# allentran/golds-rl-gym

Measured on AMD Instinct MI355X. Metric: env-steps/sec (whole node), 32k parallel Swarm-v0 envs, 20-step PAAC rollout, higher is better.
Workload: dtype f32; 1 GPU; Swarm-v0 84x84, 32768 envs per GPU, T=20 PAAC update, conv policy of train_paac_conv.py (BASELINE configs[2]); envs_per_gpu=32768, envs_total=32768, rollout_steps=20, policy=conv, train=True, swarm_math=exact, env_state_dtype=f64, streams=4, gradient_exchange=none

## Files before the change

### golds-rl-gym_amd/csrc/net_conv.hip

```cpp
#include <rccl/rccl.h>
#include <stdlib.h>
#include <string.h>

#include <chrono>
#include <cmath>
#include <string>
#include <vector>

#include "../../include/goldsrl_net.h"
#include "common.h"
#include "net_gemm.h"
#include "net_reduce.inc"
#include "rng.h"

namespace grl {

enum : uint32_t { RS_ACTION = 16 };

struct ConvOffsets {
    static constexpr long c1w = 0, c1b = c1w + 8 * 8 * 3 * 32, c2w = c1b + 32, c2b = c2w + 4 * 4 * 32 * 64, c3w = c2b + 64,
                          c3b = c3w + 3 * 3 * 64 * 64, d1w = c3b + 64, d1b = d1w + 3136 * 512, d2w = d1b + 512,
                          d2b = d2w + 512 * 256, p1w = d2b + 256, p1b = p1w + 256 * 512, heads = p1b + 512;
};
constexpr int GRL_MAX_ACTIONS = 4;
// ... 17 lines not shown
using GatherT2 = ConvGather<10, 10, 1, 1, -1, -1, 2, 2, 64, 9, 9, true>;

}

constexpr int GRL_MAX_LANES = 8;
constexpr int kLossScaleAt = 8, kLossBoundAt = 10;
constexpr int kRangeLatchAt = 12;
struct NetLane {
    float *grads;
    float *a1, *a2, *a3, *d1, *d2, *p1, *v1, *v2;
    float *ga1, *ga2, *ga3, *gd1, *gd2, *gp1, *gv1, *gv2;
    float *sraw, *z2sh, *dz2, *gt;
    float *a2sh, *d2s, *gsl, *dza, *dz3sh, *tmpw3;
    unsigned long long *m2s;
    float *dl2, *tt2, *tmpw2;
    int2 *t2desc;
    float *z3sh;
    float *a3sh, *d3, *ysh;
    unsigned long long *m3;
    float *gd1sh, *gsh3, *g3p, *dz3p;
    int *perm, *goffp, *blkcnt, *blkoff, *sbeg, *send, *sgrp, *binbase;
    unsigned short *pkey, *prank;
    unsigned *smask, *tmask, *zmask, *wmask;
    int *slot_of;
    int2 *rowdesc;
    unsigned char *skey;
    unsigned short *srank, *stap;
    int *sblkcnt, *sblkoff, *sbinbase, *sperm;
    unsigned *tamask, *tbmask, *tcmask, *tnmask;
    int *trowlist, *tblklist, *tc3list, *trows_n, *twgcnt, *twgoff;
    unsigned *tumask;
    unsigned *obsrec;
    unsigned *tneed2;
    float *tubias;
    float *tug, *tuspix;
    float *tslab, *tsums;
    unsigned *stmask, *szmask;
    int *sbase, *rowagent, *sblk;
    signed char *tilegroup, *org;
    signed char *ulist;
    float *slab;
    float *slab1h;
    float *slabb;
    float *slab1b;
    float *cfold;
    float *carow;
    int *cperm, *cblkcnt, *cblkoff, *cgoff, *cslot, *cinv;
    signed char *ctilegroup;
    double *slab64;
    float *ro_mu;
    float *ws_a3, *ws_d1, *ws_d2, *ws_p1, *ws_v1, *ws_v2, *ws_a3sh, *ws_d3;
    unsigned long long *ws_m3;
    unsigned long long *mb_d2, *mb_v1, *ws_mb;
    float *ws_sraw, *ws_a2sh, *ws_d2s;
    unsigned long long *ws_m2s;
    signed char *ws_ulist;
    void *ws_idx[24];
    bool train_ready;
};

struct grl_net : NetLane {
    grl_handle *h;
    grl_net_config cfg;
    std::string err;
    int chunk;
    float *params, *adam_m, *adam_v;
    float *paramsT;
    long adam_t;
    float *w3t, *w2t;
    float *w3f;
    float *wpvT;
    int shared_trunk;
    double sfrac;
    double pfrac[3];
    float *tbgimg, *tbgz, *tbgimg3, *tbgz3, *tybg;
    int *tbglist;
    int obs_index;
    int trunk_skip;
    int patch_skip;
    int gemm_f32, range_fallback_on, range_fallbacks, range_bits_last, update_skipped_last;
    int f32_by_fallback, f32_clean_passes, range_return_k, range_returns;
    float absmax_last;
    int loss_scale_on;
    int acc1;
    int expand3_gather;
    int expand2_gemm, ctiles;
    float *w2corr;
    grl::HeadOff ho;
    int npad, ptiles, pslices, pslice_rows, pwgrad_xcd, pdgrad_xcd, pwgrad_pair, pdgrad_pair, swgrad_pair, swgrad_chunks, slots_xcd;
    int tn_wgs, tn_wgs_dense;
    size_t slab_floats, slab_used, slabb_floats, slabb_used;
    std::vector<grl::RJob> rq;
    std::vector<int> rq_dst;
    float *stats;
    int T, B;
    uint8_t *ro_lb, *ro_ab, *ro_pos, *ro_done;
    float *ro_act, *ro_envact, *ro_val, *ro_rew, *ro_y, *ro_adv, *ro_boot, *ro_pmu, *ro_psg;
    float *mu, *sigma, *vs;
    uint8_t *tmp_lb, *tmp_ab, *tmp_pos;
    int tmp_envs;
    unsigned long act_counter;
    std::vector<void *> allocs;
    bool prof_on;
    std::vector<hipEvent_t> prof_ev;
    std::vector<unsigned char> prof_tag;
    std::vector<double> prof_launch_flops;
    int prof_tag_cur;
    size_t prof_used;
    double prof_flops;
    int last_n;
    void *comm;
    int comm_world, comm_rank;
    hipEvent_t ar_ev0, ar_ev1;
    int ar_pending;
    long ar_calls;
    long ht_rollouts, ht_updates;
    double ht_rollout_ms, ht_train_enq_ms, ht_train_wait_ms;
    double ht_train_t0;
    double ar_ms_total;
    float ar_ms_last;
    int keep_level;
    float *keep;
    size_t keep_slots;
    long param_version, keep_version;
    int keep_max_level;
    bool keep_free_capped;
    size_t keep_free_cap, keep_headroom, keep_free_seen;
    int resident_last;
    float last_inv_total;
    NetLane lanes[GRL_MAX_LANES];
    hipStream_t lane_stream[GRL_MAX_LANES];
    hipEvent_t ev_fork, ev_join[GRL_MAX_LANES];
    hipStream_t side_stream[GRL_MAX_LANES];
    hipEvent_t ev_side0[GRL_MAX_LANES], ev_side1[GRL_MAX_LANES], ev_side2[GRL_MAX_LANES];
    int idx_side, side_now, pitem_on_side;
    int nlanes, cur_lane, last_lane;
};

namespace grl {

static int nfail(grl_net *n, int code, const std::string &msg) {
    if (n) n->err = msg;
    return code;
}
#define NET_HIP(n, call)                                                                                   \
    do {                                                                                                   \
        hipError_t _e = (call);                                                                            \
        if (_e != hipSuccess) return nfail(n, GRL_E_HIP, std::string(#call) + ": " + hipGetErrorString(_e)); \
    } while (0)

template <typename T>
static int nalloc(grl_net *n, T **p, size_t count) {
    NET_HIP(n, hipMalloc((void **)p, count * sizeof(T)));
    n->allocs.push_back(*p);
    NET_HIP(n, hipMemsetAsync(*p, 0, count * sizeof(T), n->h->stream));
    NET_HIP(n, hipStreamSynchronize(n->h->stream));
    return GRL_OK;
}

static void use_lane(grl_net *net, int k) {
    if (k == net->cur_lane) return;
    net->lanes[net->cur_lane] = static_cast<NetLane &>(*net);
    static_cast<NetLane &>(*net) = net->lanes[k];
    net->h->stream = net->lane_stream[k];
    net->cur_lane = k;
}
static int lanes_active(const grl_net *net) { return net->prof_on ? 1 : net->nlanes; }
static int lanes_fork(grl_net *net) {
    if (lanes_active(net) < 2) return GRL_OK;
    use_lane(net, 0);
    NET_HIP(net, hipEventRecord(net->ev_fork, net->lane_stream[0]));
    for (int k = 1; k < net->nlanes; ++k) NET_HIP(net, hipStreamWaitEvent(net->lane_stream[k], net->ev_fork, 0));
    return GRL_OK;
}
static int lanes_join(grl_net *net) {
    use_lane(net, 0);
    if (lanes_active(net) < 2) return GRL_OK;
    for (int k = 1; k < net->nlanes; ++k) {
        NET_HIP(net, hipEventRecord(net->ev_join[k], net->lane_stream[k]));
        NET_HIP(net, hipStreamWaitEvent(net->lane_stream[0], net->ev_join[k], 0));
    }
    return GRL_OK;
}

static double slot_rows_for_flops(grl_net *net, int n) {
    if (!net->prof_on) return 9.0 * n;
    int live = 9 * n;
    if (hipStreamSynchronize(net->h->stream) == hipSuccess) (void)hipMemcpy(&live, net->sbase + n, sizeof(int), hipMemcpyDeviceToHost);
    return (double)live;
}

enum {
    PT_OTHER = 0, PT_DENSE_FWD, PT_DENSE_DGRAD, PT_DENSE_WGRAD, PT_PATCH_FWD, PT_PATCH_DGRAD, PT_PATCH_WGRAD, PT_ENV_FWD, PT_ENV_DGRAD,
    PT_ENV_WGRAD, PT_SLOT_FWD, PT_SLOT_DGRAD, PT_SLOT_WGRAD, PT_CLASS_CORR, PT_PER_AGENT, PT_COUNT
};

template <int BM, int BN, int WGM, int WGN, class AG, class Epi, int XCD = 1, bool FENCE = true, int NBUF = 1, bool ACC1 = false>
static void launch_rowk(grl_net *net, dim3 grid, hipStream_t st, AG ag, const float *Bt, int ldb, int N, Epi epi) {
    constexpr bool kAcc1 = ACC1 && ((WGM * WGN == 8 && BM == 128 && BN == 128) || (WGM * WGN == 4 && BM * BN <= 128 * 64));
    if (net->gemm_f32)
        hipLaunchKernelGGL((gemm_rowk<BM, BN, WGM, WGN, AG, Epi, XCD, FENCE, true, NBUF, false>), grid, dim3(64 * WGM * WGN), 0, st, ag, Bt, ldb, N, epi);
    else if (kAcc1 && net->acc1)
        hipLaunchKernelGGL((gemm_rowk<BM, BN, WGM, WGN, AG, Epi, XCD, FENCE, false, NBUF, kAcc1>), grid, dim3(64 * WGM * WGN), 0, st, ag, Bt, ldb, N, epi);
    else
        hipLaunchKernelGGL((gemm_rowk<BM, BN, WGM, WGN, AG, Epi, XCD, FENCE, false, NBUF, false>), grid, dim3(64 * WGM * WGN), 0, st, ag, Bt, ldb, N, epi);
}
template <int BM, int BN, int WGM, int WGN, class AG, int XCD = 1>
static void launch_tn(grl_net *net, dim3 grid, hipStream_t st, AG ag, const float *dY, int J, int mc, float *slab) {
    if (net->gemm_f32) hipLaunchKernelGGL((gemm_tn<BM, BN, WGM, WGN, AG, XCD, true>), grid, dim3(64 * WGM * WGN), 0, st, ag, dY, J, mc, slab);
    else hipLaunchKernelGGL((gemm_tn<BM, BN, WGM, WGN, AG, XCD, false>), grid, dim3(64 * WGM * WGN), 0, st, ag, dY, J, mc, slab);
}

__global__ void evict_kernel(float4 *__restrict__ buf, size_t n4) {
    const size_t stride = (size_t)gridDim.x * blockDim.x;
    for (size_t i = (size_t)blockIdx.x * blockDim.x + threadIdx.x; i < n4; i += stride) buf[i] = make_float4(0.f, 0.f, 0.f, 0.f);
}
static void maybe_evict(grl_net *n) {
    static const bool on = getenv("GRL_NET_EVICT") && atoi(getenv("GRL_NET_EVICT")) != 0;
    if (!on) return;
    static float4 *buf = nullptr;
    constexpr size_t bytes = (size_t)512 << 20;
    if (!buf && hipMalloc((void **)&buf, bytes) != hipSuccess) { buf = nullptr; return; }
    hipLaunchKernelGGL(evict_kernel, dim3(2048), dim3(256), 0, n->h->stream, buf, bytes / 16);
}

struct GemmTimer {
    grl_net *n;
    GemmTimer(grl_net *net, double flops) : n(net) {
        maybe_evict(n);
        if (n->prof_on && n->prof_used + 2 <= n->prof_ev.size()) {
            (void)hipEventRecord(n->prof_ev[n->prof_used], n->h->stream);
            n->prof_flops += flops;
            n->prof_tag[n->prof_used / 2] = (unsigned char)n->prof_tag_cur;
            n->prof_launch_flops[n->prof_used / 2] = flops;
        }
    }
    ~GemmTimer() {
        if (n->prof_on && n->prof_used + 2 <= n->prof_ev.size()) {
            (void)hipEventRecord(n->prof_ev[n->prof_used + 1], n->h->stream);
            n->prof_used += 2;
        }
    }
};

__global__ void transpose_kernel(const float *__restrict__ src, int K, int N, float *__restrict__ dst) {
    __shared__ float tile[32][33];
    int k0 = blockIdx.y * 32, n0 = blockIdx.x * 32;
    for (int r = threadIdx.y; r < 32; r += blockDim.y)
        if (k0 + r < K && n0 + (int)threadIdx.x < N) tile[r][threadIdx.x] = src[(long)(k0 + r) * N + n0 + threadIdx.x];
    __syncthreads();
    for (int r = threadIdx.y; r < 32; r += blockDim.y)
        if (n0 + r < N && k0 + (int)threadIdx.x < K) dst[(long)(n0 + r) * K + k0 + threadIdx.x] = tile[threadIdx.x][r];
}

__global__ void conv2_corr_weights_kernel(const float *__restrict__ w2, float *__restrict__ bt);
static int trunk_background(grl_net *net);
static void refresh_transposes(grl_net *net) {
    const struct { long off; int K, N; } L[] = {
        {ConvOffsets::c2w, 512, 64}, {ConvOffsets::c3w, 576, 64}, {ConvOffsets::d1w, 3136, 512}, {ConvOffsets::d2w, 512, 256},
        {ConvOffsets::p1w, 256, 512}, {net->ho.v1w, 256, 512}, {net->ho.v2w, 512, 256}};
    for (const auto &l : L) {
        float *dst = l.off == ConvOffsets::p1w ? net->wpvT : l.off == net->ho.v1w ? net->wpvT + (size_t)512 * 256 : net->paramsT + l.off;
        hipLaunchKernelGGL(transpose_kernel, dim3((l.N + 31) / 32, (l.K + 31) / 32), dim3(32, 8), 0, net->h->stream, net->params + l.off,
                           l.K, l.N, dst);
    }
    hipLaunchKernelGGL(conv2_corr_weights_kernel, dim3((4 * 576 * 128 + 255) / 256), dim3(256), 0, net->h->stream, net->params + ConvOffsets::c2w,
                       net->w2corr);
    for (int tap = 0; tap < 9; ++tap)
        hipLaunchKernelGGL(transpose_kernel, dim3(2, 2), dim3(32, 8), 0, net->h->stream, net->params + ConvOffsets::c3w + tap * 4096, 64, 64,
                           net->w3f + tap * 4096);
    (void)trunk_background(net);
}

__global__ __launch_bounds__(256) void conv1_sparse_kernel(const uint8_t *__restrict__ lbins, const uint8_t *__restrict__ abins,
                                                           const uint8_t *__restrict__ pos, const float *__restrict__ w1,
                                                           const float *__restrict__ b1, float *__restrict__ a1, int G,
                                                           float *__restrict__ sraw) {
    __shared__ unsigned int cnt[2][7056 / 4 + 4];
    __shared__ float S[400 * 32];
    const int env = blockIdx.x, tid = threadIdx.x;
    for (int i = tid; i < 2 * (7056 / 4 + 4); i += 256) (&cnt[0][0])[i] = 0;
    __syncthreads();
    if (tid < 80) {
        int bx = lbins[((size_t)env * 80 + tid) * 2], by = lbins[((size_t)env * 80 + tid) * 2 + 1];
        if (bx != 255) { int idx = bx * G + by; atomicAdd(&cnt[0][idx >> 2], 1u << (8 * (idx & 3))); }
    } else if (tid < 90) {
        int a = tid - 80;
        int bx = abins[((size_t)env * 10 + a) * 2], by = abins[((size_t)env * 10 + a) * 2 + 1];
        if (bx != 255) { int idx = bx * G + by; atomicAdd(&cnt[1][idx >> 2], 1u << (8 * (idx & 3))); }
    }
    __syncthreads();
// ... 550 lines not shown
}

extern "C" {

int grl_net_config_default(int32_t kind, grl_net_config *cfg) {
    if (!cfg || kind != GRL_NET_CONV_SINGLE_AGENT) return GRL_E_INVALID;
    memset(cfg, 0, sizeof(*cfg));
    cfg->struct_size = (int32_t)sizeof(grl_net_config);
    cfg->kind = kind;
    cfg->max_chunk_samples = 40960;
    cfg->scale = 1000.f;
    cfg->entropy_beta = 0.02f;
    cfg->clip_norm = 40.f;
    cfg->gamma = 0.99f;
    cfg->num_actions = 2;
    return GRL_OK;
}

static int range_flag_init(grl_net *n);

int grl_net_create(grl_handle *h, const grl_net_config *cfg, grl_net **out) {
    if (!h || !cfg || !out) return GRL_E_INVALID;
    *out = nullptr;
    if (cfg->struct_size != (int32_t)sizeof(grl_net_config)) return fail(h, GRL_E_INVALID, "grl_net_create: grl_net_config size mismatch");
    if (cfg->kind != GRL_NET_CONV_SINGLE_AGENT) return fail(h, GRL_E_INVALID, "grl_net_create: unknown kind");
    if (h->cfg.env_kind != GRL_ENV_SWARM || h->cfg.grid_size != 84)
        return fail(h, GRL_E_INVALID, "grl_net_create: the conv net needs a Swarm handle with grid_size 84 (84x84x3 input)");
    if (cfg->max_chunk_samples < 10 || cfg->max_chunk_samples % 10 || cfg->max_chunk_samples > 131072)
        return fail(h, GRL_E_INVALID, "grl_net_create: max_chunk_samples must be a multiple of 10 in 10..131072");
    if (cfg->num_actions < 1 || cfg->num_actions > GRL_MAX_ACTIONS)
        return fail(h, GRL_E_INVALID, "grl_net_create: num_actions must be in 1..4");
    bool free_capped = false;
    unsigned long long free_mb = 0;
    if (const char *e = getenv("GRL_NET_KEEP_FREE_MB")) {
        char *end = nullptr;
        free_mb = strtoull(e, &end, 10);
        if (*e < '0' || *e > '9' || *end != 0 || free_mb >= (1ull << 44))
            return fail(h, GRL_E_INVALID, "grl_net_create: GRL_NET_KEEP_FREE_MB must be a number of MB (decimal digits)");
        free_capped = true;
    }
    hipSetDevice(h->cfg.device_id);
    grl_net *n = new grl_net();
    n->h = h; n->cfg = *cfg; n->chunk = cfg->max_chunk_samples; n->adam_t = 0;
    n->ho = head_offsets(cfg->num_actions);
    n->T = 0; n->B = 0; n->tmp_envs = 0; n->act_counter = 0; n->prof_on = false; n->prof_used = 0; n->prof_flops = 0; n->last_n = 0; n->prof_tag_cur = 0;
    n->ro_lb = nullptr; n->slab_floats = 0; n->slab_used = 0; n->slabb_floats = 0; n->slabb_used = 0; n->w3t = n->w2t = nullptr;
    n->mu = n->sigma = n->vs = nullptr;
    n->keep_level = 0;
    n->ar_ev0 = n->ar_ev1 = nullptr; n->ar_pending = 0; n->ar_calls = 0; n->ht_rollouts = n->ht_updates = 0; n->ht_rollout_ms = n->ht_train_enq_ms = n->ht_train_wait_ms = 0.0; n->ht_train_t0 = 0.0; n->ar_ms_total = 0.0; n->ar_ms_last = 0.f;
    n->keep = nullptr; n->keep_slots = 0; n->param_version = 0; n->keep_version = -1;
    n->keep_max_level = 3; n->keep_free_capped = false; n->keep_free_cap = 0; n->keep_headroom = 0; n->keep_free_seen = 0;
    n->resident_last = 0;
    if (const char *e = getenv("GRL_NET_KEEP_LEVEL")) n->keep_max_level = atoi(e);
    n->keep_free_capped = free_capped; n->keep_free_cap = (size_t)free_mb << 20;
    n->shared_trunk = (cfg->reserved & GRL_NET_F_PER_AGENT_TRUNK) ? 0 : 1;
    n->cur_lane = 0; n->last_lane = 0;
    for (int k = 0; k < GRL_MAX_LANES; ++k) { n->lane_stream[k] = nullptr; n->ev_join[k] = nullptr; n->side_stream[k] = nullptr; n->ev_side0[k] = n->ev_side1[k] = n->ev_side2[k] = nullptr; }
    n->idx_side = 0; n->side_now = 0; n->pitem_on_side = 0;
    n->lane_stream[0] = h->stream; n->ev_fork = nullptr; n->nlanes = 1;
    const size_t c = n->chunk;
    n->ptiles = (int)((c + 255) / 256) + 9;
    n->ctiles = (int)((c + 255) / 256) + 4;
    {
        const char *lsk = getenv("GRL_NET_LOSS_SCALE");
        n->loss_scale_on = (lsk && strcmp(lsk, "off") == 0) ? 0 : 1;
        const char *gm = getenv("GRL_NET_GEMM"), *rf = getenv("GRL_NET_RANGE_FALLBACK");
        n->gemm_f32 = (gm && strcmp(gm, "f32") == 0) ? 1 : 0;
        n->range_fallback_on = (rf && strcmp(rf, "off") == 0) ? 0 : 1;
        n->range_fallbacks = 0; n->range_bits_last = 0; n->update_skipped_last = 0;
        n->f32_by_fallback = 0; n->f32_clean_passes = 0; n->range_returns = 0; n->absmax_last = 0.f;
        n->range_return_k = 4;
        if (const char *rr = getenv("GRL_NET_RANGE_RETURN")) n->range_return_k = strcmp(rr, "off") == 0 ? 0 : std::max(0, atoi(rr));
        const char *psk = getenv("GRL_PATCH_SKIP");
        n->patch_skip = (psk && strcmp(psk, "off") == 0) ? 0 : 1;
        const char *oix = getenv("GRL_OBS_INDEX");
        n->obs_index = (oix && strcmp(oix, "off") == 0) ? 0 : 1;
        const char *tsk = getenv("GRL_TRUNK_SKIP");
        n->trunk_skip = (tsk && strcmp(tsk, "off") == 0) ? 0 : 1;
        n->pfrac[0] = n->pfrac[1] = n->pfrac[2] = 1.0; n->sfrac = 1.0;
        const char *e2 = getenv("GRL_NET_EXPAND2");
        n->expand2_gemm = (e2 && strcmp(e2, "lds") == 0) ? 0 : 1;
        { const char *e3 = getenv("GRL_NET_EXPAND3"); n->expand3_gather = (e3 && strcmp(e3, "prod") == 0) ? 0 : 1;
          const char *a1 = getenv("GRL_NET_ACC1"); n->acc1 = (a1 && strcmp(a1, "off") == 0) ? 0 : 1; }
    }
    n->pslice_rows = PATCH_SLICE_ROWS; n->pwgrad_xcd = 1;
    if (const char *e = getenv("GRL_PATCH_SLICE")) { const int v = atoi(e); if (v == 256 || v == 512 || v == 1024 || v == 2048 || v == 4096 || v == 8192) n->pslice_rows = v; }
    if (const char *e = getenv("GRL_PATCH_WGRAD_XCD")) n->pwgrad_xcd = atoi(e);
    n->pwgrad_pair = 1;
    if (const char *e = getenv("GRL_PATCH_WGRAD_PAIR")) n->pwgrad_pair = strcmp(e, "off") != 0 && strcmp(e, "0") != 0;
    n->pdgrad_pair = 1;
    if (const char *e = getenv("GRL_PATCH_DGRAD_PAIR")) n->pdgrad_pair = strcmp(e, "off") != 0 && strcmp(e, "0") != 0;
    n->swgrad_pair = 1;
    if (const char *e = getenv("GRL_SLOT_WGRAD_PAIR")) n->swgrad_pair = strcmp(e, "off") != 0 && strcmp(e, "0") != 0;
    n->slots_xcd = 1;
    if (const char *e = getenv("GRL_SLOTS_XCD")) n->slots_xcd = strcmp(e, "off") != 0 && strcmp(e, "0") != 0;
    n->swgrad_chunks = 0;
    if (const char *e = getenv("GRL_SLOT_WGRAD_CHUNKS")) n->swgrad_chunks = std::max(0, atoi(e));
    n->pdgrad_xcd = 1;
    n->tn_wgs = 1024; n->tn_wgs_dense = 512;
    if (const char *e = getenv("GRL_TN_WGS")) { const int v = atoi(e); if (v >= 256 && v <= 4096) n->tn_wgs = v; }
    if (const char *e = getenv("GRL_TN_WGS_DENSE")) { const int v = atoi(e); if (v >= 128 && v <= 4096) n->tn_wgs_dense = v; }
    if (const char *e = getenv("GRL_PATCH_DGRAD_XCD")) n->pdgrad_xcd = atoi(e) != 0;
    n->pslices = (int)((c + n->pslice_rows - 1) / n->pslice_rows) + 9;
    n->npad = (int)((c + 255) / 256 * 256);
    int rc = GRL_OK;
    auto A = [&](float **p, size_t cnt) { if (rc == GRL_OK) rc = nalloc(n, p, cnt); };
    A(&n->params, n->ho.total); A(&n->paramsT, n->ho.total); A(&n->adam_m, n->ho.total); A(&n->adam_v, n->ho.total);
    A(&n->w3f, 576 * 64); A(&n->stats, 16); A(&n->wpvT, (size_t)1024 * 256); A(&n->w2corr, 4 * 576 * 128);
    A(&n->tbgimg, 12800); A(&n->tbgz, 128); A(&n->tbgimg3, 5184); A(&n->tbgz3, 128); A(&n->tybg, 49 * 512);
    if (rc == GRL_OK) rc = nalloc(n, &n->tbglist, 4);
    int nlanes = (cfg->reserved & GRL_NET_F_SINGLE_STREAM) ? 1 : 4;
    if (const char *env = getenv("GRL_NET_LANES")) { int v = atoi(env); if (v >= 1 && v <= GRL_MAX_LANES) nlanes = v; }
    for (int k = 0; k < nlanes && rc == GRL_OK; ++k) {
        static_cast<NetLane &>(*n) = NetLane{};
        rc = alloc_lane_forward(n);
        n->lanes[k] = static_cast<NetLane &>(*n);
    }
    static_cast<NetLane &>(*n) = n->lanes[0];
    if (rc == GRL_OK && nlanes > 1) {
        bool ok = hipEventCreateWithFlags(&n->ev_fork, hipEventDisableTiming) == hipSuccess;
        for (int k = 1; k < nlanes && ok; ++k)
            ok = hipStreamCreateWithFlags(&n->lane_stream[k], hipStreamNonBlocking) == hipSuccess &&
                 hipEventCreateWithFlags(&n->ev_join[k], hipEventDisableTiming) == hipSuccess;
        if (!ok) rc = nfail(n, GRL_E_HIP, "creating the lane streams/events failed");
    }
    if (rc == GRL_OK) n->nlanes = nlanes;
    {
        const char *e = getenv("GRL_NET_IDX_SIDE");
        const bool want = !(cfg->reserved & GRL_NET_F_SINGLE_STREAM) && !(e && (!strcmp(e, "off") || !strcmp(e, "0"))) && rc == GRL_OK;
        if (want && side_stream_pick(n) == GRL_OK && n->side_stream[0]) {
            const bool ok = hipEventCreateWithFlags(&n->ev_side0[0], hipEventDisableTiming) == hipSuccess &&
                            hipEventCreateWithFlags(&n->ev_side1[0], hipEventDisableTiming) == hipSuccess &&
                            hipEventCreateWithFlags(&n->ev_side2[0], hipEventDisableTiming) == hipSuccess;
            n->idx_side = ok ? 1 : 0;
        }
        (void)hipGetLastError();
    }
    if (rc == GRL_OK && hipFuncSetAttribute((const void *)expand_conv2_kernel, hipFuncAttributeMaxDynamicSharedMemorySize,
                                            (int)EXP2_LDS_BYTES) != hipSuccess)
        rc = nfail(n, GRL_E_HIP, "hipFuncSetAttribute(expand_conv2_kernel)");
    if (rc == GRL_OK) rc = ensure_tmp_obs(n, h->E);
    if (rc == GRL_OK) rc = range_flag_init(n);
    if (rc != GRL_OK) {
        fail(h, rc, "grl_net_create: " + n->err);
        grl_net_destroy(n);
        return rc;
    }
    hipStreamSynchronize(h->stream);
    *out = n;
    return GRL_OK;
}

int grl_net_destroy(grl_net *n) {
    if (!n) return GRL_OK;
    const bool alive = grl_handle_alive(n->h);
    grl_sync_for_destroy(n->h);
    if (n->comm) {
        ncclCommDestroy((ncclComm_t)n->comm);
        (void)hipGetLastError();
    }
    if (alive) use_lane(n, 0);
    for (int k = 1; k < GRL_MAX_LANES; ++k) {
        if (n->lane_stream[k]) { hipStreamSynchronize(n->lane_stream[k]); hipStreamDestroy(n->lane_stream[k]); }
        if (n->ev_join[k]) hipEventDestroy(n->ev_join[k]);
    }
    for (int k = 0; k < GRL_MAX_LANES; ++k) {
// ... 357 lines not shown
```

### golds-rl-gym_amd/csrc/net_gemm.h

```cpp
#pragma once
#include <hip/hip_runtime.h>
#include <stdint.h>

#include <type_traits>
#include <utility>

namespace grl {

template <class E, class = void>
struct epi_row_bits : std::false_type {};
template <class E>
struct epi_row_bits<E, std::void_t<decltype(E::kRowBits)>> : std::bool_constant<E::kRowBits> {};

template <class E, class = void>
struct epi_row_auxn : std::false_type {};
template <class E>
struct epi_row_auxn<E, std::void_t<decltype(E::kRowAuxN)>> : std::bool_constant<E::kRowAuxN> {};
template <class E, class = void>
struct epi_add_aux : std::false_type {};
template <class E>
struct epi_add_aux<E, std::void_t<decltype(E::kAddAux)>> : std::bool_constant<E::kAddAux> {};

typedef float f32x16 __attribute__((ext_vector_type(16)));
typedef float f32x4 __attribute__((ext_vector_type(4)));
// ... 839 lines not shown
        s += (row[0] + row[32]) + (row[64] + row[96]);
    }
    red[threadIdx.x] = s;
    __syncthreads();
    if (threadIdx.x < 32) {
        float t = 0.f;
#pragma unroll
        for (int j = 0; j < 8; ++j) t += red[j * 32 + threadIdx.x];
        partial[blockIdx.x * 32 + threadIdx.x] = t;
    }
}

constexpr float kLowScale = 2048.f;
__device__ __forceinline__ void split2(float x, float y, unsigned &h, unsigned &l) {
    const f32x2 xy = {x, y};
    const f16x2 hv = __builtin_convertvector(xy, f16x2);
    const f32x2 r = {(x - (float)hv[0]) * kLowScale, (y - (float)hv[1]) * kLowScale};
    const f16x2 lv = __builtin_convertvector(r, f16x2);
    h = __builtin_bit_cast(unsigned, hv);
    l = __builtin_bit_cast(unsigned, lv);
}
__device__ __forceinline__ void split4(float x0, float x1, float x2, float x3, uint2 &h, uint2 &l) {
    split2(x0, x1, h.x, l.x);
    split2(x2, x3, h.y, l.y);
}
__device__ __forceinline__ void mfma_x3(f32x4 &acc, f32x4 &acl, const f16x8 (&a)[2], const f16x8 (&b)[2]) {
    acl = __builtin_amdgcn_mfma_f32_16x16x32_f16(a[1], b[0], acl, 0, 0, 0);
    acl = __builtin_amdgcn_mfma_f32_16x16x32_f16(a[0], b[1], acl, 0, 0, 0);
    acc = __builtin_amdgcn_mfma_f32_16x16x32_f16(a[0], b[0], acc, 0, 0, 0);
}
constexpr int kLdh = 32;
__device__ int *g_gemm_range_flag;
__device__ unsigned *g_gemm_absmax;
constexpr float kF16Max = 65504.f;
constexpr int kW128M = 4, kW128N = 2, kW256M = 8, kW256N = 1;
__device__ __forceinline__ int swz(int row) { return (0x78 >> (((row >> 2) & 3) * 2)) & 3; }

__device__ __forceinline__ int f32_off(int row, int k) { return row * 32 + ((((k >> 2) ^ (row & 7)) << 2) | (k & 3)); }
template <int TM, int TN>
__device__ __forceinline__ void mfma_f32_step(const float *__restrict__ Af, const float *__restrict__ Bf, int arow, int brow, int kg,
                                              f32x4 (&acc)[TM][TN]) {
    float4 a0[TM], a1[TM], b0[TN], b1[TN];
#pragma unroll
    for (int a = 0; a < TM; ++a) {
        a0[a] = *reinterpret_cast<const float4 *>(Af + f32_off(arow + a * 16, 8 * kg));
        a1[a] = *reinterpret_cast<const float4 *>(Af + f32_off(arow + a * 16, 8 * kg + 4));
    }
#pragma unroll
    for (int b = 0; b < TN; ++b) {
        b0[b] = *reinterpret_cast<const float4 *>(Bf + f32_off(brow + b * 16, 8 * kg));
        b1[b] = *reinterpret_cast<const float4 *>(Bf + f32_off(brow + b * 16, 8 * kg + 4));
    }
#define GRL_F32_STEP(AV, BV)                                                                                          \
    _Pragma("unroll") for (int a = 0; a < TM; ++a)                                                                    \
        _Pragma("unroll") for (int b = 0; b < TN; ++b) acc[a][b] = __builtin_amdgcn_mfma_f32_16x16x4f32(AV, BV, acc[a][b], 0, 0, 0);
    GRL_F32_STEP(a0[a].x, b0[b].x) GRL_F32_STEP(a0[a].y, b0[b].y) GRL_F32_STEP(a0[a].z, b0[b].z) GRL_F32_STEP(a0[a].w, b0[b].w)
    GRL_F32_STEP(a1[a].x, b1[b].x) GRL_F32_STEP(a1[a].y, b1[b].y) GRL_F32_STEP(a1[a].z, b1[b].z) GRL_F32_STEP(a1[a].w, b1[b].w)
#undef GRL_F32_STEP
}

template <class T, class = void> struct ag_has_ctx : std::false_type {};
template <class T> struct ag_has_ctx<T, std::void_t<decltype(std::declval<const T &>().wg_ctx(0))>> : std::true_type {};
template <class AG> __device__ __forceinline__ auto ag_ctx(const AG &ag, int m0) {
    if constexpr (ag_has_ctx<AG>::value) return ag.wg_ctx(m0);
    else return m0;
}
template <class AG, class C> __device__ __forceinline__ bool ag_tile_ok(const AG &ag, const C &c, int m0, int k0) {
    if constexpr (ag_has_ctx<AG>::value) return ag.tile_ok_c(c, k0);
    else return ag.tile_ok(m0, k0);
}
template <class AG, class C> __device__ __forceinline__ int ag_bk(const AG &ag, const C &c, int m0, int k0) {
    if constexpr (ag_has_ctx<AG>::value) return ag.bk_c(c, k0);
    else return ag.bk(k0, m0);
}
template <class T, class = void> struct ag_has_n_ok : std::false_type {};
template <class T> struct ag_has_n_ok<T, std::void_t<decltype(std::declval<const T &>().n_ok(0, 0))>> : std::true_type {};
template <class T, class = void> struct ag_has_i_ok : std::false_type {};
template <class T> struct ag_has_i_ok<T, std::void_t<decltype(std::declval<const T &>().i_ok(0, 0))>> : std::true_type {};
template <class T, class = void> struct ag_pair_n : std::false_type {};
template <class T> struct ag_pair_n<T, std::void_t<decltype(T::kPairN)>> : std::bool_constant<T::kPairN> {};
template <class T, class = void> struct ag_pair_i : std::false_type {};
template <class T> struct ag_pair_i<T, std::void_t<decltype(T::kPairI)>> : std::bool_constant<T::kPairI> {};

template <int BM, int BN, int WGM, int WGN, class AG, class Epi, int XCD_ORDER = 1, bool FENCE = true, bool F32 = false, int NBUF = 1, bool ACC1 = false>
__global__ __launch_bounds__(64 * WGM * WGN, ACC1 ? (WGM * WGN == 8 ? 6 : 4) : WGM * WGN / 2) void gemm_rowk(AG ag, const float *__restrict__ Bt, int ldb, int N, Epi epi) {
    constexpr int BK = 32, LDH = kLdh, NT = 64 * WGM * WGN, RPP = NT / 8;
    constexpr int WM = BM / WGM, WN = BN / WGN, TM = WM / 16, TN = WN / 16;
    constexpr int NA = BM / RPP;
    constexpr int NB = BN / RPP;
    static_assert((WGM * WGN == 4 || WGM * WGN == 8) && TM >= 1 && TN >= 1 && NA >= 1 && BN % RPP == 0, "4 or 8 waves");
    static_assert(NBUF == 1 || NBUF == 2, "one or two LDS buffers");
    __shared__ __attribute__((aligned(16))) unsigned short As[NBUF][2][BM * LDH];
    static_assert(!(ACC1 && F32), "the fp32 form has one accumulator set anyway");
    __shared__ __attribute__((aligned(16))) unsigned short Bs[NBUF][ACC1 ? 3 : 2][BN * LDH];

    const int tid = threadIdx.x, lane = tid & 63, wave = tid >> 6;
    const int wm = wave / WGN, wn = wave - wm * WGN;
    int bx = blockIdx.x, by = blockIdx.y;
    if constexpr (XCD_ORDER == 2) {
        const int nt = (ag.live_rows() + BM - 1) / BM, tpx = (nt + 7) >> 3, w = blockIdx.y;
        if ((w >> 3) >= tpx) return;
        by = (w & 7) * tpx + (w >> 3);
        if (by >= nt) return;
    }
    if (XCD_ORDER == 1) {
        const int nx = gridDim.x, L = by * nx + bx, g = L / (8 * nx);
        if ((g + 1) * 8 <= (int)gridDim.y) {
            const int l = L - g * 8 * nx;
            by = g * 8 + (l & 7);
            bx = l >> 3;
        }
    }
    const int m0 = by * BM, n0 = bx * BN;
    if (!ag.tile_active(m0)) return;
    constexpr bool PAIRN = ag_pair_n<AG>::value;
    int2 pp = make_int2(0, 0);
    if constexpr (PAIRN) {
        static_assert(!PAIRN || (BM == 128 && BN == 128 && WGN == 2 && 64 * WGM * WGN == 512), "128 x 128 on eight waves: a wave column per pixel");
        pp = ag.npair(m0, bx);
        if (pp.x < 0) return;
    } else if constexpr (ag_has_n_ok<AG>::value) {
        if (!ag.n_ok(m0, n0)) return;
    }
    const int M = ag.rows, K = ag.K();
    const auto wctx = ag_ctx(ag, m0);
    const int trow = tid >> 3, tk4 = (tid & 7) * 4;
    const int wo = (((tk4 >> 3) ^ swz(trow)) << 3) + (tk4 & 4);

    long aoff[NA];
    int ayx[NA];
    bool arow_ok[NA];
#pragma unroll
    for (int i = 0; i < NA; ++i) {
        int r = m0 + trow + RPP * i;
        arow_ok[i] = r < M;
        int iy0, ix0;
        ag.row(arow_ok[i] ? r : 0, aoff[i], iy0, ix0);
        ayx[i] = (iy0 << 16) | (ix0 & 0xFFFF);
    }
    static_assert(NB == 1 || NB == 2 || NB == 4, "B tile of 1, 2 or 4 passes");
    const float *brow0 = Bt + (long)(ag.bn(PAIRN ? pp.x * 64 : n0, m0) + trow) * ldb + tk4;
    const float *brow1 = PAIRN ? Bt + (long)(ag.bn(max(pp.y, pp.x) * 64, m0) + trow) * ldb + tk4 : brow0 + (long)RPP * ldb;

    float4 ra[NA];
    float4 rb0 = make_float4(0.f, 0.f, 0.f, 0.f), rb1 = rb0, rb2 = rb0, rb3 = rb0;
    unsigned vmask = 0;
#define GRL_LOAD_TILE(kt_)                                                                                 \
    {                                                                                                      \
        int toff, ty, tx;                                                                                  \
        ag.tap((kt_) * BK, toff, ty, tx);                                                                  \
        _Pragma("unroll") for (int i = 0; i < NA; ++i) {                                                   \
            int iy0 = ayx[i] >> 16, ix0 = (int)(int16_t)(ayx[i] & 0xFFFF);                                 \
            bool v = arow_ok[i] && ag.ok(iy0, ix0, ty, tx);                                                \
             \
              \
            ra[i] = *reinterpret_cast<const float4 *>(ag.base + (v ? aoff[i] + toff : 0L) + tk4);          \
            vmask = v ? (vmask | (1u << i)) : (vmask & ~(1u << i));    \
        }                                                                                                  \
                     \
        const int bko = ag_bk(ag, wctx, m0, (kt_) * BK);                                                             \
        rb0 = *reinterpret_cast<const float4 *>(brow0 + bko);                                              \
        if (NB > 1) rb1 = *reinterpret_cast<const float4 *>(brow1 + bko);                                  \
        if (NB > 2) rb2 = *reinterpret_cast<const float4 *>(brow0 + (long)2 * RPP * ldb + bko);            \
        if (NB > 2) rb3 = *reinterpret_cast<const float4 *>(brow0 + (long)3 * RPP * ldb + bko);            \
    }
#define GRL_STORE_PLANES(S_, row_, v4_)                                                                    \
    {                                                                                                      \
        if constexpr (F32) {                                                                               \
            *reinterpret_cast<float4 *>(reinterpret_cast<float *>(&S_[0][0]) + f32_off(row_, tk4)) = (v4_); \
        } else {                                                                                           \
            uint2 h_, l_;                                                                                  \
            split4((v4_).x, (v4_).y, (v4_).z, (v4_).w, h_, l_);                                            \
            *reinterpret_cast<uint2 *>(&S_[0][(row_) * LDH + wo]) = h_;                                    \
            *reinterpret_cast<uint2 *>(&S_[1][(row_) * LDH + wo]) = l_;                                    \
        }                                                                                                  \
    }
#define GRL_STORE_PLANES_B(S_, row_, v4_)                                                                  \
    {                                                                                                      \
        GRL_STORE_PLANES(S_, row_, v4_)                                                                    \
        if constexpr (ACC1) {                                                                              \
            uint2 h_, l_;                                                                                  \
            split4((v4_).x, (v4_).y, (v4_).z, (v4_).w, h_, l_);       \
            const f16x2 k_ = {(_Float16)kLowScale, (_Float16)kLowScale};                                   \
            const f16x2 s0_ = __builtin_bit_cast(f16x2, h_.x) * k_, s1_ = __builtin_bit_cast(f16x2, h_.y) * k_; \
            *reinterpret_cast<uint2 *>(&S_[2][(row_) * LDH + wo]) = make_uint2(__builtin_bit_cast(unsigned, s0_), __builtin_bit_cast(unsigned, s1_)); \
        }                                                                                                  \
    }
#define GRL_STORE_TILE(buf_)                                                                               \
    {                                                                                                      \
        _Pragma("unroll") for (int i = 0; i < NA; ++i) {                                                   \
            const bool v = (vmask >> i) & 1u;                                                              \
            float4 t4 = ra[i];                                                                             \
            t4.x = v ? t4.x : 0.f; t4.y = v ? t4.y : 0.f; t4.z = v ? t4.z : 0.f; t4.w = v ? t4.w : 0.f;    \
            if (AG::kRelu) { t4.x = fmaxf(t4.x, 0.f); t4.y = fmaxf(t4.y, 0.f); t4.z = fmaxf(t4.z, 0.f); t4.w = fmaxf(t4.w, 0.f); } \
            GRL_STORE_PLANES(As[buf_], trow + RPP * i, t4)                                                 \
        }                                                                                                  \
        GRL_STORE_PLANES_B(Bs[buf_], trow, rb0)                                                            \
        if (NB > 1) GRL_STORE_PLANES_B(Bs[buf_], trow + RPP, rb1)                                          \
        if (NB > 2) GRL_STORE_PLANES_B(Bs[buf_], trow + 2 * RPP, rb2)                                      \
        if (NB > 2) GRL_STORE_PLANES_B(Bs[buf_], trow + 3 * RPP, rb3)                                      \
    }

    f32x4 acc[TM][TN], acl[ACC1 ? 1 : TM][ACC1 ? 1 : TN];
#pragma unroll
    for (int a = 0; a < TM; ++a)
#pragma unroll
        for (int b = 0; b < TN; ++b)
#pragma unroll
            for (int r = 0; r < 4; ++r) {
                acc[a][b][r] = 0.f;
                if constexpr (!ACC1) acl[a][b][r] = 0.f;
            }

    const int nk = K / BK;
    int kt = 0;
    while (kt < nk && !ag_tile_ok(ag, wctx, m0, kt * BK)) ++kt;
    GRL_LOAD_TILE(kt < nk ? kt : 0)
    const int l16 = lane & 15, kg = lane >> 4;
    const int ro = (kg ^ swz(l16)) << 3;
    const int aro = (wm * WM + l16) * LDH + ro;
    const int bro = (wn * WN + l16) * LDH + ro;
#define GRL_MFMA_TILE(cb_)                                                                                                             \
    {                                                                                                                                  \
        if constexpr (F32) {                                                                                                           \
            mfma_f32_step<TM, TN>(reinterpret_cast<const float *>(&As[cb_][0][0]), reinterpret_cast<const float *>(&Bs[cb_][0][0]),    \
                                  wm * WM + l16, wn * WN + l16, kg, acc);                                                              \
        } else if constexpr (ACC1) {                                                                                                   \
            f16x8 af[TM][2];                                                                                                           \
            _Pragma("unroll") for (int a = 0; a < TM; ++a)                                                                             \
                _Pragma("unroll") for (int p = 0; p < 2; ++p) af[a][p] = *reinterpret_cast<const f16x8 *>(&As[cb_][p][aro + a * 16 * LDH]); \
            _Pragma("unroll") for (int b = 0; b < TN; ++b) {                                                                           \
                f16x8 bf[3];                                                                                                           \
                _Pragma("unroll") for (int p = 0; p < 3; ++p) bf[p] = *reinterpret_cast<const f16x8 *>(&Bs[cb_][p][bro + b * 16 * LDH]); \
                _Pragma("unroll") for (int a = 0; a < TM; ++a) {                                                                       \
                    acc[a][b] = __builtin_amdgcn_mfma_f32_16x16x32_f16(af[a][1], bf[0], acc[a][b], 0, 0, 0);                           \
                    acc[a][b] = __builtin_amdgcn_mfma_f32_16x16x32_f16(af[a][0], bf[1], acc[a][b], 0, 0, 0);                           \
                    acc[a][b] = __builtin_amdgcn_mfma_f32_16x16x32_f16(af[a][0], bf[2], acc[a][b], 0, 0, 0);                           \
                }                                                                                                                      \
            }                                                                                                                          \
        } else if constexpr (TM < TN) {         \
            f16x8 af[TM][2];                                                                                                           \
            _Pragma("unroll") for (int a = 0; a < TM; ++a)                                                                             \
                _Pragma("unroll") for (int p = 0; p < 2; ++p) af[a][p] = *reinterpret_cast<const f16x8 *>(&As[cb_][p][aro + a * 16 * LDH]); \
            _Pragma("unroll") for (int b = 0; b < TN; ++b) {                                                                           \
                f16x8 bf[2];                                                                                                           \
                _Pragma("unroll") for (int p = 0; p < 2; ++p) bf[p] = *reinterpret_cast<const f16x8 *>(&Bs[cb_][p][bro + b * 16 * LDH]); \
                _Pragma("unroll") for (int a = 0; a < TM; ++a) mfma_x3(acc[a][b], acl[a][b], af[a], bf);                               \
            }                                                                                                                          \
        } else {                                                                                                                       \
            f16x8 bf[TN][2];                                                                                                           \
            _Pragma("unroll") for (int b = 0; b < TN; ++b)                                                                             \
                _Pragma("unroll") for (int p = 0; p < 2; ++p) bf[b][p] = *reinterpret_cast<const f16x8 *>(&Bs[cb_][p][bro + b * 16 * LDH]); \
            _Pragma("unroll") for (int a = 0; a < TM; ++a) {                                                                           \
                f16x8 af[2];                                                                                                           \
                _Pragma("unroll") for (int p = 0; p < 2; ++p) af[p] = *reinterpret_cast<const f16x8 *>(&As[cb_][p][aro + a * 16 * LDH]); \
                _Pragma("unroll") for (int b = 0; b < TN; ++b) mfma_x3(acc[a][b], acl[a][b], af, bf[b]);                               \
            }                                                                                                                          \
        }                                                                                                                              \
    }
    if constexpr (NBUF == 1) {
        while (kt < nk) {
            GRL_STORE_TILE(0)
            __syncthreads();
            int ktn = kt + 1;
            while (ktn < nk && !ag_tile_ok(ag, wctx, m0, ktn * BK)) ++ktn;
            {
                const int ktl = ktn < nk ? ktn : kt;
                GRL_LOAD_TILE(ktl)
            }
            if constexpr (FENCE) { GRL_SCHED_FENCE }
            GRL_MFMA_TILE(0)
            if constexpr (FENCE) { GRL_SCHED_FENCE }
            __syncthreads();
            kt = ktn;
        }
    } else {
        int ktn = nk;
        if (kt < nk) {
            GRL_STORE_TILE(0)
            ktn = kt + 1;
            while (ktn < nk && !ag_tile_ok(ag, wctx, m0, ktn * BK)) ++ktn;
            GRL_LOAD_TILE(ktn < nk ? ktn : kt)
            __syncthreads();
        }
        int cb = 0;
        while (kt < nk) {
            int ktnn = ktn;
            if (ktn < nk) {
                GRL_STORE_TILE(cb ^ 1)
                ktnn = ktn + 1;
                while (ktnn < nk && !ag_tile_ok(ag, wctx, m0, ktnn * BK)) ++ktnn;
                GRL_LOAD_TILE(ktnn < nk ? ktnn : ktn)
            }
            if constexpr (FENCE) { GRL_SCHED_FENCE }
            GRL_MFMA_TILE(cb)
            if constexpr (FENCE) { GRL_SCHED_FENCE }
            __syncthreads();
            kt = ktn;
            ktn = ktnn;
            cb ^= 1;
        }
    }
#undef GRL_MFMA_TILE
    if constexpr (!F32) {
#pragma unroll
        for (int a = 0; a < TM; ++a)
#pragma unroll
            for (int b = 0; b < TN; ++b)
#pragma unroll
                for (int r = 0; r < 4; ++r) {
                    if constexpr (ACC1) acc[a][b][r] *= 1.0f / kLowScale;
                    else acc[a][b][r] = __builtin_fmaf(acl[a][b][r], 1.0f / kLowScale, acc[a][b][r]);
                }
    }
    const int ecolbase = PAIRN ? ((wn == 0 ? pp.x : pp.y) < 0 ? N : (wn == 0 ? pp.x : pp.y) * 64) : n0 + wn * WN;
    const int erow = m0 + wm * WM + 4 * kg, ecol = ecolbase + l16;
    int rax[TM][4];
    float eax[TM][TN][4];
    bool out_of_range = false;
    float amax = 0.f;
#pragma unroll
    for (int a = 0; a < TM; ++a)
#pragma unroll
        for (int r = 0; r < 4; ++r) {
            if constexpr (epi_row_bits<Epi>::value || epi_row_auxn<Epi>::value) rax[a][r] = epi.row_aux_n(min(erow + a * 16 + r, M - 1), ecolbase);
            else rax[a][r] = epi.row_aux(min(erow + a * 16 + r, M - 1));
        }
#pragma unroll
    for (int a = 0; a < TM; ++a)
#pragma unroll
        for (int b = 0; b < TN; ++b)
#pragma unroll
            for (int r = 0; r < 4; ++r)
                eax[a][b][r] = epi.elem_aux(min(erow + a * 16 + r, M - 1), min(ecol + b * 16, N - 1), rax[a][r]);
#pragma unroll
    for (int a = 0; a < TM; ++a)
#pragma unroll
        for (int b = 0; b < TN; ++b)
#pragma unroll
            for (int r = 0; r < 4; ++r) {
                const int row = erow + a * 16 + r, col = ecol + b * 16;
                if (row < M && col < N) epi.store(row, col, acc[a][b][r], rax[a][r], eax[a][b][r]);
                const float gv = epi_add_aux<Epi>::value ? acc[a][b][r] + eax[a][b][r] : acc[a][b][r];
                out_of_range |= !(fabsf(gv) <= kF16Max);
                if constexpr (F32) amax = fmaxf(amax, fabsf(gv));
            }
    if (!F32 && out_of_range) atomicOr(g_gemm_range_flag, 1);
    if constexpr (F32) {
#pragma unroll
        for (int o = 32; o > 0; o >>= 1) amax = fmaxf(amax, __shfl_xor(amax, o, 64));
        if (lane == 0) atomicMax(g_gemm_absmax, __float_as_uint(amax));
    }
    if constexpr (Epi::kColSum) {
#pragma unroll
        for (int b = 0; b < TN; ++b) {
            float sum = 0.f;
#pragma unroll
            for (int a = 0; a < TM; ++a)
#pragma unroll
                for (int r = 0; r < 4; ++r)
                    if (erow + a * 16 + r < M) sum += epi.value(acc[a][b][r], eax[a][b][r]);
            sum += __shfl_xor(sum, 16);
            sum += __shfl_xor(sum, 32);
            const int col = ecol + b * 16;
            if (kg == 0 && col < N) epi.csum[(long)(by * WGM + wm) * N + col] = sum;
        }
    }
    if constexpr (epi_row_bits<Epi>::value) {
        static_assert(WN == 64, "a wave covers exactly one 64-column block");
#pragma unroll
        for (int a = 0; a < TM; ++a)
#pragma unroll
            for (int r = 0; r < 4; ++r) {
                unsigned long long w = 0ull;
#pragma unroll
                for (int b = 0; b < TN; ++b) {
                    const unsigned long long bal = __ballot(epi.bit(acc[a][b][r], eax[a][b][r]));
                    w |= ((bal >> (16 * kg)) & 0xFFFFull) << (16 * b);
                }
                const int row = erow + a * 16 + r;
                if (l16 == 0 && row < M) epi.store_bits(row, ecolbase, w, rax[a][r]);
            }
    }
#undef GRL_LOAD_TILE
#undef GRL_STORE_TILE
#undef GRL_STORE_PLANES
#undef GRL_STORE_PLANES_B
}

template <int BM, int BN, int WGM, int WGN, class AG, int XCD_ORDER = 1, bool F32 = false>
__global__ __launch_bounds__(64 * WGM * WGN, WGM * WGN / 2) void gemm_tn(AG ag, const float *__restrict__ dY, int J, int mc, float *__restrict__ slab) {
    constexpr int BK = 32, LDH = kLdh, NT = 64 * WGM * WGN;
    constexpr int WM = BM / WGM, WN = BN / WGN, TM = WM / 16, TN = WN / 16;
    constexpr int A4 = BM / 4, B4 = BN / 4;
    constexpr int NA = BK * A4 / NT, NB = BK * B4 / NT;
    static_assert((WGM * WGN == 4 || WGM * WGN == 8) && NA >= 1 && NB >= 1 && NA <= 4 && NB <= 4 && (NA != 3) && (NB != 3), "tile size");
    __shared__ __attribute__((aligned(16))) unsigned short As[2][BM * LDH];
    __shared__ __attribute__((aligned(16))) unsigned short Bs[2][BN * LDH];
    const int tid = threadIdx.x, lane = tid & 63, wave = tid >> 6;
    const int wm = wave / WGN, wn = wave - wm * WGN;
    int bx = blockIdx.x, by = blockIdx.y, bz = blockIdx.z;
    if (XCD_ORDER == 2) {
        const int nx = gridDim.x, ny = gridDim.y, l = by * nx + bx, g = l / (8 * ny);
        if ((g + 1) * 8 <= nx) {
            const int r = l - g * 8 * ny;
            bx = g * 8 + (r & 7);
            by = r >> 3;
        } else {
            const int r = l - g * 8 * ny, w = nx - g * 8;
            by = r / w;
            bx = g * 8 + (r - by * w);
        }
    }
    if (XCD_ORDER == 1) {
        const int nx = gridDim.x, T = nx * gridDim.y, L = bz * T + by * nx + bx, g = L / (8 * T);
        if ((g + 1) * 8 <= (int)gridDim.z) {
            const int l = L - g * 8 * T, t = l >> 3;
            bz = g * 8 + (l & 7);
            by = t / nx;
            bx = t - by * nx;
        }
    }
    constexpr bool PAIR = ag_pair_i<AG>::value;
    const int i0 = bx * BM, j0 = by * BN;
    const int I = ag.K();
    int mbeg, mend;
    ag.mrange(bz, mc, mbeg, mend);
    int2 pp = make_int2(0, 0);
    if constexpr (PAIR) {
        static_assert(!PAIR || BM == 128, "two 64-column halves");
        pp = ag.pair(bz, bx);
        if (pp.x < 0) return;
    } else if constexpr (ag_has_i_ok<AG>::value) {
        if (!ag.i_ok(bz, i0)) return;
    }

    int toff, ty, tx;
    ag.tap(PAIR ? (((int)(threadIdx.x % (BM / 4)) < 16 ? pp.x : max(pp.y, 0)) * 64) : i0, toff, ty, tx);

    const int ca = tid % A4, cb = tid % B4;
    int ga = tid / A4, gb = tid / B4;
    if (NA == 4) ga ^= (ca >> 1) & 1;
    if (NA == 2) ga ^= ((ca >> 1) & 1) << 1;
    if (NB == 4) gb ^= (cb >> 1) & 1;
    if (NB == 2) gb ^= ((cb >> 1) & 1) << 1;
    if (NB == 1) gb ^= ((cb >> 1) & 1) << 2;
    const int ma = NA * ga, mb = NB * gb;
    const int acol = PAIR ? toff + (ca & 15) * 4 : toff + ca * 4;
    const bool ahalf_ok = !PAIR || ca < 16 || pp.y >= 0;
    float4 ra[NA], rb[NB];
    unsigned vma = 0, vmb = 0;
    int2 ia[NA];
    int ib[NB];
    unsigned iva = 0;
#define GRL_LOAD_IDX(mt_)                                                                                          \
    {                                                                                                              \
        _Pragma("unroll") for (int i = 0; i < NA; ++i) {                                                           \
            const int m = (mt_) + ma + i;                                                                          \
            ia[i] = ag.ahandle(m < mend ? m : mbeg);                                                               \
            iva = (m < mend && ag.hvalid(ia[i])) ? (iva | (1u << i)) : (iva & ~(1u << i));                         \
        }                                                                                                          \
        _Pragma("unroll") for (int i = 0; i < NB; ++i) {                                                           \
            const int m = (mt_) + mb + i;                                                                          \
            ib[i] = ag.bhandle(m < mend ? m : mbeg);                                                               \
            if (m >= mend) ib[i] = -1;                                                                             \
        }                                                                                                          \
    }
#define GRL_LOAD_TILE()                                                                                            \
    {                                                                                                              \
        _Pragma("unroll") for (int i = 0; i < NA; ++i) {                                                           \
            const bool inr = (iva >> i) & 1u;                                                                      \
            long off; int iy0, ix0;                                                                                \
            ag.rowh(ia[i], off, iy0, ix0);                                                                         \
            const bool v = inr && ahalf_ok && ag.ok(iy0, ix0, ty, tx);                                             \
            ra[i] = *reinterpret_cast<const float4 *>(ag.base + (v ? off + acol : (long)(ca * 4)));                \
            vma = v ? (vma | (1u << i)) : (vma & ~(1u << i));                                                      \
        }                                                                                                          \
        _Pragma("unroll") for (int i = 0; i < NB; ++i) {                                                           \
            const bool v = ib[i] >= 0;                                                                             \
            rb[i] = *reinterpret_cast<const float4 *>(dY + (long)(v ? ib[i] : 0) * J + j0 + cb * 4);               \
            vmb = v ? (vmb | (1u << i)) : (vmb & ~(1u << i));                                                      \
        }                                                                                                          \
    }
#define GRL_TN_OFF(rho_, m_) ((rho_) * LDH + ((((m_) >> 3) ^ swz(rho_)) << 3) + ((m_) & 7))
#define GRL_STORE_RUN(S_, NV_, rho_, m_, r_, comp_)                                                                \
    {                                                                                                              \
        if constexpr (F32) {                                                                                       \
            float *f_ = reinterpret_cast<float *>(&S_[0][0]) + f32_off(rho_, m_);                                  \
            if (NV_ == 4) *reinterpret_cast<float4 *>(f_) = make_float4(r_[0].comp_, r_[1 % NV_].comp_, r_[2 % NV_].comp_, r_[3 % NV_].comp_); \
            else if (NV_ == 2) *reinterpret_cast<float2 *>(f_) = make_float2(r_[0].comp_, r_[1 % NV_].comp_);      \
            else *f_ = r_[0].comp_;                                                                                \
        } else {                                                                                                   \
        const int o_ = GRL_TN_OFF(rho_, m_);                                                                       \
        if (NV_ == 4) {                                                                                            \
            uint2 h_, l_;                                                                                          \
            split4(r_[0].comp_, r_[1 % NV_].comp_, r_[2 % NV_].comp_, r_[3 % NV_].comp_, h_, l_);                  \
            *reinterpret_cast<uint2 *>(&S_[0][o_]) = h_;                                                           \
            *reinterpret_cast<uint2 *>(&S_[1][o_]) = l_;                                                           \
        } else {                                                                                                   \
            unsigned h_, l_;                                                                                       \
            split2(r_[0].comp_, r_[1 % NV_].comp_, h_, l_);                                                        \
            if (NV_ == 2) {                                                                                        \
                *reinterpret_cast<unsigned *>(&S_[0][o_]) = h_;                                                    \
                *reinterpret_cast<unsigned *>(&S_[1][o_]) = l_;                                                    \
            } else {                                                                                               \
                S_[0][o_] = (unsigned short)(h_ & 0xFFFFu);                                                        \
                S_[1][o_] = (unsigned short)(l_ & 0xFFFFu);                                                        \
            }                                                                                                      \
        }                                                                                                          \
        }                                                                                                          \
    }
#define GRL_STORE_TILE()                                                                                           \
    {                                                                                                              \
        _Pragma("unroll") for (int i = 0; i < NA; ++i) {                                                           \
            const bool v = (vma >> i) & 1u;                                                                        \
            float4 t4 = ra[i];                                                                                     \
            t4.x = v ? t4.x : 0.f; t4.y = v ? t4.y : 0.f; t4.z = v ? t4.z : 0.f; t4.w = v ? t4.w : 0.f;            \
            if (AG::kRelu) { t4.x = fmaxf(t4.x, 0.f); t4.y = fmaxf(t4.y, 0.f); t4.z = fmaxf(t4.z, 0.f); t4.w = fmaxf(t4.w, 0.f); } \
            ra[i] = t4;                                                                                            \
        }                                                                                                          \
        GRL_STORE_RUN(As, NA, 0 * A4 + ca, ma, ra, x)                                                  \
        GRL_STORE_RUN(As, NA, 1 * A4 + ca, ma, ra, y)                                                  \
        GRL_STORE_RUN(As, NA, 2 * A4 + ca, ma, ra, z)                                                  \
        GRL_STORE_RUN(As, NA, 3 * A4 + ca, ma, ra, w)                                                  \
        _Pragma("unroll") for (int i = 0; i < NB; ++i) {                                                           \
            const bool v = (vmb >> i) & 1u;                                                                        \
            float4 t4 = rb[i];                                                                                     \
            t4.x = v ? t4.x : 0.f; t4.y = v ? t4.y : 0.f; t4.z = v ? t4.z : 0.f; t4.w = v ? t4.w : 0.f;            \
            rb[i] = t4;                                                                                            \
        }                                                                                                          \
        if (NB == 1 && !F32) {       \
            const bool odd = gb & 1;                                                                               \
            const float4 t4 = rb[0];                                                                               \
            const float o0 = __shfl_xor(odd ? t4.x : t4.z, B4), o1 = __shfl_xor(odd ? t4.y : t4.w, B4);            \
            unsigned h0, l0, h1, l1;                                                                               \
            split2(odd ? o1 : t4.x, odd ? t4.w : o0, h0, l0);       \
            split2(odd ? o0 : t4.y, odd ? t4.z : o1, h1, l1);                  \
            const int q0 = GRL_TN_OFF((odd ? 3 : 0) * B4 + cb, mb & ~1), q1 = GRL_TN_OFF((odd ? 2 : 1) * B4 + cb, mb & ~1); \
            *reinterpret_cast<unsigned *>(&Bs[0][q0]) = h0;                                                        \
            *reinterpret_cast<unsigned *>(&Bs[1][q0]) = l0;                                                        \
            *reinterpret_cast<unsigned *>(&Bs[0][q1]) = h1;                                                        \
            *reinterpret_cast<unsigned *>(&Bs[1][q1]) = l1;                                                        \
        } else {                                                                                                   \
        GRL_STORE_RUN(Bs, NB, 0 * B4 + cb, mb, rb, x)                                                  \
        GRL_STORE_RUN(Bs, NB, 1 * B4 + cb, mb, rb, y)                                                  \
        GRL_STORE_RUN(Bs, NB, 2 * B4 + cb, mb, rb, z)                                                  \
        GRL_STORE_RUN(Bs, NB, 3 * B4 + cb, mb, rb, w)                                                  \
        }                                                                                                          \
    }
    f32x4 acc[TM][TN], acl[TM][TN];
#pragma unroll
    for (int a = 0; a < TM; ++a)
#pragma unroll
        for (int b = 0; b < TN; ++b)
#pragma unroll
            for (int r = 0; r < 4; ++r) acc[a][b][r] = acl[a][b][r] = 0.f;
    const int l16 = lane & 15, kg = lane >> 4;
    const int ro = (kg ^ swz(l16)) << 3;
    const int aro = (wm * WM + l16) * LDH + ro;
    const int bro = (wn * WN + l16) * LDH + ro;
    if (mbeg < mend) {
        GRL_LOAD_IDX(mbeg)
        GRL_LOAD_TILE()
        GRL_LOAD_IDX(mbeg + BK)
        for (int mt = mbeg; mt < mend; mt += BK) {
            GRL_STORE_TILE()
            __syncthreads();
            GRL_LOAD_TILE()
            GRL_LOAD_IDX(mt + 2 * BK)
            {
                if constexpr (F32) {
                    mfma_f32_step<TM, TN>(reinterpret_cast<const float *>(&As[0][0]), reinterpret_cast<const float *>(&Bs[0][0]),
                                          wm * WM + l16, wn * WN + l16, kg, acc);
                } else if constexpr (TM < TN) {
                    f16x8 af[TM][2];
#pragma unroll
                    for (int a = 0; a < TM; ++a)
#pragma unroll
                        for (int p = 0; p < 2; ++p) af[a][p] = *reinterpret_cast<const f16x8 *>(&As[p][aro + a * 16 * LDH]);
#pragma unroll
                    for (int b = 0; b < TN; ++b) {
                        f16x8 bf[2];
#pragma unroll
                        for (int p = 0; p < 2; ++p) bf[p] = *reinterpret_cast<const f16x8 *>(&Bs[p][bro + b * 16 * LDH]);
#pragma unroll
                        for (int a = 0; a < TM; ++a) mfma_x3(acc[a][b], acl[a][b], af[a], bf);
                    }
                } else {
                    f16x8 bf[TN][2];
#pragma unroll
                    for (int b = 0; b < TN; ++b)
#pragma unroll
                        for (int p = 0; p < 2; ++p) bf[b][p] = *reinterpret_cast<const f16x8 *>(&Bs[p][bro + b * 16 * LDH]);
#pragma unroll
                    for (int a = 0; a < TM; ++a) {
                        f16x8 af[2];
#pragma unroll
                        for (int p = 0; p < 2; ++p) af[p] = *reinterpret_cast<const f16x8 *>(&As[p][aro + a * 16 * LDH]);
#pragma unroll
                        for (int b = 0; b < TN; ++b) mfma_x3(acc[a][b], acl[a][b], af, bf[b]);
                    }
                }
            }
            __syncthreads();
        }
    }
    if constexpr (!F32) {
#pragma unroll
        for (int a = 0; a < TM; ++a)
#pragma unroll
            for (int b = 0; b < TN; ++b)
#pragma unroll
                for (int r = 0; r < 4; ++r) acc[a][b][r] = __builtin_fmaf(acl[a][b][r], 1.0f / kLowScale, acc[a][b][r]);
    }
    float *out = slab + (long)bz * I * J;
#pragma unroll
    for (int a = 0; a < TM; ++a)
#pragma unroll
        for (int b = 0; b < TN; ++b)
#pragma unroll
            for (int r = 0; r < 4; ++r) {
                const int pa = wm * WM + a * 16 + 4 * kg + r;
                const int pb = wn * WN + b * 16 + l16;
                int row = i0 + 4 * (pa % A4) + pa / A4;
                const int col = j0 + 4 * (pb % B4) + pb / B4;
                if constexpr (PAIR) {
                    const int c = row - i0, px = c < 64 ? pp.x : pp.y;
                    row = px < 0 ? I : px * 64 + (c & 63);
                }
                if (row < I && col < J) out[(long)row * J + col] = acc[a][b][r];
            }
#undef GRL_LOAD_TILE
#undef GRL_LOAD_IDX
#undef GRL_STORE_TILE
#undef GRL_STORE_RUN
#undef GRL_TN_OFF
}



constexpr int kNarrowCols = 4;
__global__ __launch_bounds__(256) void slab_reduce_narrow_kernel(const float *__restrict__ slab, int chunks, int n, float *__restrict__ dst,
                                                                 int accumulate) {
    const int lane = threadIdx.x & 63, i = blockIdx.x * kNarrowCols + (threadIdx.x >> 6);
    float s0 = 0.f, s1 = 0.f, s2 = 0.f, s3 = 0.f;
    if (i < n) {
        int c = lane;
        for (; c + 192 < chunks; c += 256) {
            s0 += slab[(long)c * n + i];
            s1 += slab[(long)(c + 64) * n + i];
            s2 += slab[(long)(c + 128) * n + i];
            s3 += slab[(long)(c + 192) * n + i];
        }
        for (; c < chunks; c += 64) s0 += slab[(long)c * n + i];
    }
    float s = (s0 + s1) + (s2 + s3);
#pragma unroll
    for (int o = 32; o > 0; o >>= 1) s += __shfl_xor(s, o, 64);
    if (lane == 0 && i < n) dst[i] = accumulate ? dst[i] + s : s;
}

__global__ __launch_bounds__(256) void colsum_kernel(const float *__restrict__ dY, int M, int J, int mc, float *__restrict__ slab) {
    __shared__ float4 red[256];
    const int jv = J >> 2;
    const int rl = 256 / jv;
    const int jl = threadIdx.x % jv, rsub = threadIdx.x / jv;
    const int mbeg = blockIdx.y * mc, mend = min(M, mbeg + mc);
    const float4 *__restrict__ p = reinterpret_cast<const float4 *>(dY) + jl;
    float4 s0 = make_float4(0.f, 0.f, 0.f, 0.f), s1 = s0, s2 = s0, s3 = s0;
    int m = mbeg + rsub;
    for (; m + 3 * rl < mend; m += 4 * rl) {
        const float4 v0 = p[(long)m * jv], v1 = p[(long)(m + rl) * jv], v2 = p[(long)(m + 2 * rl) * jv], v3 = p[(long)(m + 3 * rl) * jv];
        s0.x += v0.x; s0.y += v0.y; s0.z += v0.z; s0.w += v0.w;
        s1.x += v1.x; s1.y += v1.y; s1.z += v1.z; s1.w += v1.w;
        s2.x += v2.x; s2.y += v2.y; s2.z += v2.z; s2.w += v2.w;
        s3.x += v3.x; s3.y += v3.y; s3.z += v3.z; s3.w += v3.w;
    }
    for (; m < mend; m += rl) {
        const float4 v0 = p[(long)m * jv];
        s0.x += v0.x; s0.y += v0.y; s0.z += v0.z; s0.w += v0.w;
    }
    float4 s = make_float4((s0.x + s1.x) + (s2.x + s3.x), (s0.y + s1.y) + (s2.y + s3.y), (s0.z + s1.z) + (s2.z + s3.z),
                           (s0.w + s1.w) + (s2.w + s3.w));
    red[threadIdx.x] = s;
    __syncthreads();
    if (rsub == 0) {
        for (int r = 1; r < rl; ++r) {
            const float4 v = red[r * jv + jl];
            s.x += v.x; s.y += v.y; s.z += v.z; s.w += v.w;
// ... 7 lines not shown
```

### golds-rl-gym_amd/csrc/net_patch.inc

```

struct PatchShape { int g, ry0, ry1, rx0, rx1; };
__device__ __forceinline__ PatchShape patch_shape(const signed char *__restrict__ ul, int cnt) {
    int uy0 = 9, ux0 = 9, uy1 = -1, ux1 = -1;
    for (int j = 0; j < cnt; ++j) {
        const int u = ul[j], y = u / 9, x = u - y * 9;
        uy0 = min(uy0, y); ux0 = min(ux0, x); uy1 = max(uy1, y); ux1 = max(ux1, x);
    }
    if (uy0 > 8) return PatchShape{0, 0, 4, 0, 4};
    const int oy = min(max(uy0 - 2, 0), 2), ox = min(max(ux0 - 2, 0), 2);
    PatchShape p{oy * 3 + ox, max(uy0 - 2, 0) - oy, min(uy1, 6) - oy, max(ux0 - 2, 0) - ox, min(ux1, 6) - ox};
    if (p.ry0 < 0 || p.ry1 > 4 || p.ry0 > p.ry1) { p.ry0 = 0; p.ry1 = 4; }
    if (p.rx0 < 0 || p.rx1 > 4 || p.rx0 > p.rx1) { p.rx0 = 0; p.rx1 = 4; }
    return p;
}
__device__ __forceinline__ int span_code(int &r0, int &r1) {
    if (r0 == 0) return r1;
    if (r1 == 4) return 4 + r0;
    r0 = 0;
    return r1;
}

constexpr int PATCH_KEYS = 9 * 81;
constexpr int PATCH_SORT_BLOCK = 1024;
__global__ __launch_bounds__(PATCH_SORT_BLOCK) void patch_group_kernel(const signed char *__restrict__ ulist, const int *__restrict__ sbase, int n,
// ... 473 lines not shown
    __syncthreads();
    if (threadIdx.x == 0) tmask[blockIdx.x] = (unsigned short)(part[0] | part[1]);
}

struct PItemBufs { float *d2c; int4 *desc; unsigned short *tapm, *tmask9; int *icnt, *ioff, *irows; };
static PItemBufs pitem_bufs(grl_net *net) {
    const size_t c = net->chunk, nbmax = (c + 255) / 256;
    PItemBufs b;
    b.d2c = net->a2;
    b.desc = reinterpret_cast<int4 *>(net->a2 + (size_t)net->ctiles * 256 * 576);
    b.tapm = reinterpret_cast<unsigned short *>(b.desc + c * 25 + 256);
    b.tmask9 = b.tapm + c * 25 + 256;
    b.icnt = reinterpret_cast<int *>(b.tmask9 + ((c * 25 + 127) / 128 + 8) / 2 * 2 + 2);
    b.ioff = b.icnt + nbmax * PITEM_KEYS;
    b.irows = b.ioff + nbmax * PITEM_KEYS;
    return b;
}
static bool pitem_gather_on(const grl_net *net) { return net->expand3_gather && net->expand2_gemm && net->chunk <= (1u << 17); }
static int pitem_index(grl_net *net, int n, const uint8_t *pos) {
    hipStream_t st = net->h->stream;
    const PItemBufs b = pitem_bufs(net);
    const bool trunk3f = net->trunk_skip && net->expand2_gemm;
    const unsigned *wm = net->patch_skip ? net->wmask : nullptr, *smk = net->patch_skip ? net->smask : nullptr;
    const int nb = (n + 255) / 256;
    if ((nb + PITEM_SB - 1) / PITEM_SB > 256) return nfail(net, GRL_E_INVALID, "pitem_index: chunk too large for the item scan");
    hipLaunchKernelGGL(pitem_count_kernel, dim3(nb), dim3(256), 0, st, wm, smk, n, (const signed char *)net->org, pos, (const int *)net->cslot, b.icnt);
    hipLaunchKernelGGL(pitem_scan_kernel, dim3(1), dim3(1024), 0, st, (const int *)b.icnt, nb, b.ioff, b.irows);
    hipLaunchKernelGGL(pitem_place_kernel, dim3(nb), dim3(256), 0, st, wm, smk, n, (const signed char *)net->org, pos, (const int *)net->cslot,
                       (const int *)net->cinv, trunk3f ? (const unsigned *)net->tcmask : (const unsigned *)nullptr, (const int *)b.ioff, b.desc, b.tapm);
    const int tiles = (n * 25 + 127) / 128;
    hipLaunchKernelGGL(pitem_masks_kernel, dim3(tiles), dim3(128), 0, st, b.desc, (const unsigned short *)b.tapm, (const int *)b.irows, b.tmask9);
    NET_HIP(net, hipGetLastError());
    return GRL_OK;
}

static int forward_conv3_dense1_shared(grl_net *net, int nenv, const uint8_t *pos) {
    hipStream_t st = net->h->stream;
    const float *P = net->params, *PT = net->paramsT;
    const int n = nenv * 10;
    const bool trunk3f = net->trunk_skip && net->expand2_gemm;
    if (trunk3f) {
        GatherConv3Rows g{net->a2sh, net->tc3list, net->trows_n + 2, net->tbgimg3, nenv * 49, 1};
        EpiBiasDualRows e{net->z3sh, nullptr, 64, P + ConvOffsets::c3b, net->tc3list, net->trows_n + 2, nullptr, nullptr};
        net->prof_tag_cur = PT_ENV_FWD;
        {
            GemmTimer t(net, 2.0 * trunk_live(net, 2, (double)nenv * 49) * 576 * 64);
            launch_rowk<256, 64, kW256M, kW256N, GatherConv3Rows, EpiBiasDualRows>(net, dim3(1, (nenv * 49 + 255) / 256), st, g, PT + ConvOffsets::c3w, 576, 64, e);
        }
    } else {
        GatherConv3 g{net->a2sh, nenv * 49};
        EpiBiasAct e{net->z3sh, 64, P + ConvOffsets::c3b, ACT_NONE};
        net->prof_tag_cur = PT_ENV_FWD;
        GemmTimer t(net, 2.0 * nenv * 49 * 576 * 64);
        launch_rowk<256, 64, kW256M, kW256N, GatherConv3, EpiBiasAct>(net, dim3(1, (nenv * 49 + 255) / 256), st, g, PT + ConvOffsets::c3w, 576, 64, e);
    }
    if (pitem_gather_on(net)) {
        const PItemBufs pb = pitem_bufs(net);
        float *d2c = pb.d2c;
        int4 *desc = pb.desc;
        unsigned short *tmask9 = pb.tmask9;
        int *irows = pb.irows;
        hipLaunchKernelGGL(a3sh_relu_kernel, dim3(nenv), dim3(256), 0, st, (const float *)net->z3sh,
                           trunk3f ? (const unsigned *)net->tcmask : (const unsigned *)nullptr, (const float *)net->tbgz3,
                           trunk3f ? (const unsigned *)net->tumask : (const unsigned *)nullptr, net->a3sh);
        if (net->pitem_on_side) net->pitem_on_side = 0;
        else if (int rc = pitem_index(net, n, pos)) return rc;
        const int maxrows = n * 25, tiles = (maxrows + 127) / 128;
        double live_pairs = (double)maxrows * 9;
        if (net->prof_on) {
            int nlive = 0;
            NET_HIP(net, hipStreamSynchronize(st));
            NET_HIP(net, hipMemcpy(&nlive, irows, sizeof(int), hipMemcpyDeviceToHost));
            const int nt = (nlive + 127) / 128;
            std::vector<unsigned short> tm(nt > 0 ? nt : 1);
            if (nt > 0) NET_HIP(net, hipMemcpy(tm.data(), tmask9, (size_t)nt * 2, hipMemcpyDeviceToHost));
            live_pairs = 0;
            for (int t = 0; t < nt; ++t) live_pairs += 128.0 * __builtin_popcount(tm[t] & 0x1FFu);
        }
        SlotsToPatch g{d2c, desc, maxrows, irows, tmask9};
        EpiPatchExpand e{desc, net->z3sh, (const float *)net->tbgz3, net->d3, net->m3};
        net->prof_tag_cur = PT_SLOT_FWD;
        GemmTimer t(net, 2.0 * live_pairs * 64 * 64);
        if (net->slots_xcd)
            launch_rowk<128, 64, 4, 1, SlotsToPatch, EpiPatchExpand, 2, true, 1, true>(net, dim3(1, tiles + 8), st, g, PT + ConvOffsets::c3w, 576, 64, e);
        else
            launch_rowk<128, 64, 4, 1, SlotsToPatch, EpiPatchExpand, 1, true, 1, true>(net, dim3(1, tiles), st, g, PT + ConvOffsets::c3w, 576, 64, e);
    } else {
    {
        SlotRowsP g{net->d2s, net->sperm, n * 9, 64, 64, net->sbase + n, net->patch_skip ? net->stmask : nullptr};
        EpiPermStore e{net->a2, net->sperm, 576};
        net->prof_tag_cur = PT_SLOT_FWD;
        GemmTimer t(net, 2.0 * slot_rows_for_flops(net, n) * 64 * 576 * net->sfrac);
        launch_rowk<256, 64, kW256M, kW256N, SlotRowsP, EpiPermStore>(net, dim3(576 / 64, (n * 9 + 255) / 256), st, g, net->w3f, 64, 576, e);
    }
    maybe_evict(net);
    hipLaunchKernelGGL(expand_conv3_patch_kernel, dim3(nenv), dim3(256), 0, st, net->z3sh, net->a2, net->ulist, net->sbase, net->org,
                       net->patch_skip ? net->smask : nullptr, net->patch_skip ? net->wmask : nullptr, net->a3sh, net->d3, net->m3,
                       trunk3f ? (const unsigned *)net->tcmask : (const unsigned *)nullptr, (const float *)net->tbgz3,
                       trunk3f ? (const unsigned *)net->tumask : (const unsigned *)nullptr);
    }
    if (trunk3f) {
        static_assert(3136 <= DenseRowsKU::kMaxK, "the union mask's 64 bits cover K");
        DenseRowsKU g{{net->a3sh, nenv, 3136, 3136}, net->tumask};
        EpiBiasAct e{net->ysh, 512, net->tubias, ACT_NONE};
        net->prof_tag_cur = PT_ENV_FWD;
        GemmTimer t(net, 2.0 * nenv * 64.0 * trunk_union_pixels(net) * 512);
        launch_rowk<128, 64, 4, 1, DenseRowsKU, EpiBiasAct, true, true, 2>(net, dim3(512 / 64, (nenv + 127) / 128), st, g, PT + ConvOffsets::d1w, 3136, 512, e);
    } else {
        DenseRows g{net->a3sh, nenv, 3136, 3136};
        EpiBiasAct e{net->ysh, 512, P + ConvOffsets::d1b, ACT_NONE};
        net->prof_tag_cur = PT_ENV_FWD;
        GemmTimer t(net, 2.0 * nenv * 3136 * 512);
        launch_rowk<128, 64, 4, 1, DenseRows, EpiBiasAct>(net, dim3(512 / 64, (nenv + 127) / 128), st, g, PT + ConvOffsets::d1w, 3136, 512, e);
    }
    {
        static_assert(1600 <= PatchRows::kMaxK0, "the support word's 32 bits cover the patch");
        PatchRows g{net->d3, net->perm, net->tilegroup, net->ptiles * 256, 1600, 1600, 0, nullptr, nullptr, net->patch_skip ? net->tmask : nullptr, nullptr};
        EpiPatchFwd e{net->d1, net->ysh, net->perm, 512};
        net->prof_tag_cur = PT_PATCH_FWD;
        GemmTimer t(net, 2.0 * n * 1600 * 512 * net->pfrac[0]);
        launch_rowk<128, 128, kW128M, kW128N, PatchRows, EpiPatchFwd, true, false, 2>(net, dim3(512 / 128, net->ptiles * 2), st, g, PT + ConvOffsets::d1w, 3136, 512, e);
    }
    NET_HIP(net, hipGetLastError());
    return GRL_OK;
}

__global__ __launch_bounds__(256, 6) void agent_dz3_kernel(const float *__restrict__ gsh3, const float *__restrict__ g3p,
                                                        const float *__restrict__ a3sh, const unsigned long long *__restrict__ m3,
                                                        const signed char *__restrict__ org, const unsigned *__restrict__ smask, int nenv,
                                                        float *__restrict__ dz3sh, float *__restrict__ dz3p, float *__restrict__ bsum,
                                                        const unsigned *__restrict__ cmask, float *__restrict__ bgsum,
                                                        const float *__restrict__ a3bg, const unsigned *__restrict__ umask) {
    __shared__ __attribute__((aligned(16))) float acc[49 * 64];
    __shared__ unsigned cm[2];
    const unsigned um0 = umask ? umask[0] : 0xFFFFFFFFu, um1 = umask ? umask[1] : 0xFFFFFFFFu;
    const float4 zero4 = make_float4(0.f, 0.f, 0.f, 0.f);
    float4 cs = zero4;
    float4 cb = zero4;
    __shared__ unsigned char mskn[49 * 16];
    __shared__ int og[10], pcnt[10];
    __shared__ unsigned char plist[10][28];
    const int tid = threadIdx.x, l16 = tid & 15, c4 = l16 * 4;
    float4 bg4 = zero4;
    if (a3bg) bg4 = *reinterpret_cast<const float4 *>(a3bg + c4);
    for (int env = blockIdx.x; env < nenv; env += gridDim.x) {
        __syncthreads();
        if (tid >= 64 && tid < 66) cm[tid - 64] = cmask ? cmask[(size_t)env * 2 + tid - 64] : 0xFFFFFFFFu;
        if (tid < 10) {
            og[tid] = org[(size_t)env * 10 + tid];
            const unsigned sm = smask ? smask[(size_t)env * 10 + tid] : 0x1FFFFFFu;
            int c = 0;
            for (int q = 0; q < 25; ++q)
                if ((sm >> q) & 1u) plist[tid][c++] = (unsigned char)q;
            pcnt[tid] = c;
        }
        __syncthreads();
        {
            float4 sv[4], gv[4];
#pragma unroll
            for (int k = 0; k < 4; ++k) {
                const int i = tid + 256 * k, p = i >> 4;
                sv[k] = bg4;
                gv[k] = zero4;
                if (i < 49 * 16 && ((p < 32 ? um0 >> p : um1 >> (p - 32)) & 1u)) {
                    if (!a3bg || ((cm[p >> 5] >> (p & 31)) & 1u)) sv[k] = reinterpret_cast<const float4 *>(a3sh + (size_t)env * 3136)[i];
                    gv[k] = reinterpret_cast<const float4 *>(gsh3 + (size_t)env * 3136)[i];
                }
            }
#pragma unroll
            for (int k = 0; k < 4; ++k) {
                const int i = tid + 256 * k;
                if (i < 49 * 16) {
                    const float4 s = sv[k], g = gv[k];
                    mskn[i] = (unsigned char)((s.x > 0.f ? 1 : 0) | (s.y > 0.f ? 2 : 0) | (s.z > 0.f ? 4 : 0) | (s.w > 0.f ? 8 : 0));
                    reinterpret_cast<float4 *>(acc)[i] = make_float4(s.x > 0.f ? g.x : 0.f, s.y > 0.f ? g.y : 0.f, s.z > 0.f ? g.z : 0.f, s.w > 0.f ? g.w : 0.f);
                }
            }
        }
        int qn = -1;
        float4 gn = zero4;
        unsigned bn = 0;
#define GRL_DZ3_FETCH(a_, r_)                                                                                             \
        {                                                                                                                  \
            const int e_ = tid + 256 * (r_);                                                                               \
            qn = e_ < pcnt[a_] * 16 ? (int)plist[a_][e_ >> 4] : -1;                                                        \
            if (qn >= 0) {                                                                                                 \
                const size_t m_ = (size_t)env * 10 + (a_);                                                                \
                gn = *reinterpret_cast<const float4 *>(g3p + m_ * 1600 + qn * 64 + c4);                                    \
                bn = reinterpret_cast<const unsigned *>(m3)[(m_ * 25 + qn) * 2 + (c4 >> 5)];                               \
            }                                                                                                              \
// ... 55 lines not shown
```

### golds-rl-gym_amd/csrc/net_shared.inc

```

__device__ __forceinline__ bool conv1_cover(int ph, int pw, int c, int &oy1, int &ox1, int &tap1) {
    oy1 = (ph >> 2) - (c >> 1);
    ox1 = (pw >> 2) - (c & 1);
    const int ky = ph - 4 * oy1, kx = pw - 4 * ox1;
    tap1 = ky * 8 + kx;
    return oy1 >= 0 && oy1 < 20 && ox1 >= 0 && ox1 < 20;
}
__device__ __forceinline__ bool conv2_cover(int oy1, int ox1, int q, int &o2, int &tap2) {
    const int oy2 = (oy1 >> 1) - (q >> 1), ox2 = (ox1 >> 1) - (q & 1);
    tap2 = (oy1 - 2 * oy2) * 4 + (ox1 - 2 * ox2);
    o2 = oy2 * 9 + ox2;
    return oy2 >= 0 && oy2 < 9 && ox2 >= 0 && ox2 < 9;
}

__device__ __forceinline__ void agent_setup(const float *__restrict__ sraw_env, const float *__restrict__ w1, int ph, int pw, int tid,
                                            float *dlt, int *pairs, int *pix) {
    if (tid < 128) {
        const int c = tid >> 5, ci = tid & 31;
        int oy1, ox1, tap1;
        float d = 0.f;
        if (conv1_cover(ph, pw, c, oy1, ox1, tap1)) {
            const float s = sraw_env[(oy1 * 20 + ox1) * 32 + ci];
            d = fmaxf(s + w1[(tap1 * 3 + 2) * 32 + ci], 0.f) - fmaxf(s, 0.f);
        }
// ... 956 lines not shown
    hipLaunchKernelGGL(trunk_scan_kernel, dim3(1), dim3(1024), 0, st, net->twgcnt, nwg, net->twgoff, net->trows_n, net->tumask);
    hipLaunchKernelGGL(trunk_emit_kernel, dim3(nwg), dim3(256), 0, st, net->tamask, net->tbmask, net->tcmask, net->twgoff, nenv, net->trowlist,
                       net->tblklist, net->tc3list, net->tumask);
    hipLaunchKernelGGL(trunk_ubias_kernel, dim3(2), dim3(256), 0, st, net->params + ConvOffsets::d1b, (const float *)net->tybg, (const unsigned *)net->tumask,
                       net->tubias, net->tneed2);
    NET_HIP(net, hipGetLastError());
    return GRL_OK;
}
static double trunk_live(grl_net *net, int which, double upper) {
    if (!net->prof_on) return upper;
    int cnt = 0;
    if (hipStreamSynchronize(net->h->stream) != hipSuccess || hipMemcpy(&cnt, net->trows_n + which, sizeof(int), hipMemcpyDeviceToHost) != hipSuccess)
        return upper;
    return (double)cnt;
}

static int trunk_background(grl_net *net) {
    if (!net->shared_trunk || !net->tbgimg) return GRL_OK;
    hipStream_t st = net->h->stream;
    const float *P = net->params, *PT = net->paramsT;
    hipLaunchKernelGGL(trunk_bg_kernel, dim3(12800 / 256), dim3(256), 0, st, P + ConvOffsets::c1b, net->tbgimg, net->tbglist);
    {
        GatherConv2ReluRows g{net->tbgimg, net->tbglist, net->tbglist + 1, net->tbgimg, 1, 1};
        EpiBiasDualRows e{nullptr, nullptr, 64, P + ConvOffsets::c2b, net->tbglist, net->tbglist + 1, net->tbgz, net->tbgz + 64};
        launch_rowk<128, 64, 4, 1, GatherConv2ReluRows, EpiBiasDualRows>(net, dim3(1, 1), st, g, PT + ConvOffsets::c2w, 512, 64, e);
    }
    hipLaunchKernelGGL(trunk_fill_kernel, dim3((81 * 16 + 255) / 256), dim3(256), 0, st, (const unsigned *)nullptr, 0, 1, (const float *)nullptr, 0,
                       (float *)nullptr, (const float *)(net->tbgz + 64), net->tbgimg3, 81, (const unsigned *)nullptr);
    {
        GatherConv3Rows g{net->tbgimg3, net->tbglist, net->tbglist + 1, net->tbgimg3, 1, 1};
        EpiBiasDualRows e{nullptr, nullptr, 64, P + ConvOffsets::c3b, net->tbglist, net->tbglist + 1, net->tbgz3, net->tbgz3 + 64};
        launch_rowk<256, 64, kW256M, kW256N, GatherConv3Rows, EpiBiasDualRows>(net, dim3(1, 1), st, g, PT + ConvOffsets::c3w, 576, 64, e);
    }
    hipLaunchKernelGGL(trunk_ybg_kernel, dim3(98), dim3(256), 0, st, (const float *)(net->tbgz3 + 64), P + ConvOffsets::d1w, net->tybg);
    NET_HIP(net, hipGetLastError());
    return GRL_OK;
}

static int conv1_sparse_grid() {
    int per_cu = 0, dev = 0;
    hipDeviceProp_t prop;
    if (hipOccupancyMaxActiveBlocksPerMultiprocessor(&per_cu, (const void *)conv1_sparse_shared_kernel, 256, 0) != hipSuccess || hipGetDevice(&dev) != hipSuccess ||
        hipGetDeviceProperties(&prop, dev) != hipSuccess || per_cu < 1) {
        (void)hipGetLastError();
        return 1024;
    }
    return per_cu * prop.multiProcessorCount;
}
static double trunk_union_pixels(grl_net *net) {
    if (!net->prof_on) return 49.0;
    unsigned u[2] = {0xFFFFFFFFu, 0x1FFFFu};
    if (hipStreamSynchronize(net->h->stream) == hipSuccess) (void)hipMemcpy(u, net->tumask, sizeof(u), hipMemcpyDeviceToHost);
    return (double)(__builtin_popcount(u[0]) + __builtin_popcount(u[1] & 0x1FFFFu));
}
static int patch_sort(grl_net *net, int n);
static bool pitem_gather_on(const grl_net *net);
static int pitem_index(grl_net *net, int n, const uint8_t *pos);
static int forward_conv12_shared(grl_net *net, const uint8_t *lb, const uint8_t *ab, const uint8_t *pos, int nenv, bool tail) {
    hipStream_t st = net->h->stream;
    net->pitem_on_side = 0;
    const float *P = net->params, *PT = net->paramsT;
    const int n = nenv * 10;
    const bool trunk = net->expand2_gemm && net->trunk_skip;
    const bool side = net->idx_side && net->side_now && net->cur_lane == 0 && net->expand2_gemm && !net->prof_on && net->side_stream[0];
    if (side) NET_HIP(net, hipEventRecord(net->ev_side0[net->cur_lane], st));
    if (trunk)
        if (int rc = trunk_index(net, lb, ab, pos, nenv)) return rc;
    if (side) NET_HIP(net, hipEventRecord(net->ev_side2[net->cur_lane], st));
    static const int hgc1 = conv1_sparse_grid();
    if (net->obs_index) {
        static const int hgc1i = conv1_sparse_indexed_grid();
        if (int rc = obs_index(net, lb, ab, pos, nenv, net->obsrec, st, 1)) return rc;
        hipLaunchKernelGGL(conv1_sparse_indexed_kernel, dim3(nenv < hgc1i ? nenv : hgc1i), dim3(256), 0, st, (const unsigned *)net->obsrec, P + ConvOffsets::c1w,
                           P + ConvOffsets::c1b, net->sraw, trunk ? (const unsigned *)net->tnmask : (const unsigned *)nullptr, nenv);
    } else
    hipLaunchKernelGGL(conv1_sparse_shared_kernel, dim3(nenv < hgc1 ? nenv : hgc1), dim3(256), 0, st, lb, ab, P + ConvOffsets::c1w, P + ConvOffsets::c1b,
                       net->h->cfg.grid_size, net->sraw, trunk ? (const unsigned *)net->tnmask : (const unsigned *)nullptr, nenv);
    if (trunk) {
        GatherConv2ReluRows gr{net->sraw, net->trowlist, net->trows_n, net->tbgimg, nenv * 81, 1};
        EpiBiasDualRows e{net->z2sh, net->a2sh, 64, P + ConvOffsets::c2b, net->trowlist, net->trows_n, nullptr, nullptr};
        net->prof_tag_cur = PT_ENV_FWD;
        {
            GemmTimer t(net, 2.0 * trunk_live(net, 0, (double)nenv * 81) * 512 * 64);
            launch_rowk<128, 64, 4, 1, GatherConv2ReluRows, EpiBiasDualRows>(net, dim3(1, (nenv * 81 + 127) / 128), st, gr,
                                                                                      PT + ConvOffsets::c2w, 512, 64, e);
        }
        hipLaunchKernelGGL(trunk_fill_kernel, dim3((nenv * 81 * 16 + 255) / 256), dim3(256), 0, st, (const unsigned *)net->tamask, 3, 81,
                           (const float *)(net->tbgz + 64), nenv * 81, net->a2sh, (const float *)nullptr, (float *)nullptr, 0,
                           (const unsigned *)net->tneed2);
    } else {
        GatherConv2Relu g{net->sraw, nenv * 81};
        net->prof_tag_cur = PT_ENV_FWD;
        GemmTimer t(net, 2.0 * nenv * 81 * 512 * 64);
        if (net->expand2_gemm) {
            EpiBiasDual e{net->z2sh, net->a2sh, 64, P + ConvOffsets::c2b};
            launch_rowk<256, 64, kW256M, kW256N, GatherConv2Relu, EpiBiasDual>(net, dim3(1, (nenv * 81 + 255) / 256), st, g, PT + ConvOffsets::c2w, 512, 64, e);
        } else {
            EpiBiasAct e{net->z2sh, 64, P + ConvOffsets::c2b, ACT_NONE};
            launch_rowk<256, 64, kW256M, kW256N, GatherConv2Relu, EpiBiasAct>(net, dim3(1, (nenv * 81 + 255) / 256), st, g, PT + ConvOffsets::c2w, 512, 64, e);
        }
    }
    if (side) {
        hipStream_t ss = net->side_stream[net->cur_lane];
        NET_HIP(net, hipStreamWaitEvent(ss, net->ev_side0[net->cur_lane], 0));
        net->h->stream = ss;
        int rc = slot_index(net, pos, n);
        if (rc == GRL_OK) {
            const int nb = (n + 255) / 256;
            hipLaunchKernelGGL(conv2_prep_kernel, dim3((n + 3) / 4), dim3(256), 0, ss, net->sraw, pos, P + ConvOffsets::c1w, net->sbase, n, net->z2sh,
                               net->carow, net->ulist, net->cslot, net->d2s, 1);
            hipLaunchKernelGGL(corr_count_kernel, dim3(nb), dim3(256), 0, ss, pos, n, net->cblkcnt);
            hipLaunchKernelGGL(corr_offsets_kernel, dim3(1), dim3(256), 0, ss, net->cblkcnt, nb, net->ctiles, net->cblkoff, net->cgoff, net->ctilegroup,
                               net->cperm);
            hipLaunchKernelGGL(corr_place_kernel, dim3(nb), dim3(256), 0, ss, pos, n, net->cblkoff, net->cgoff, net->cperm, net->cinv);
            rc = patch_sort(net, n);
            if (rc == GRL_OK && tail && pitem_gather_on(net)) {
                NET_HIP(net, hipStreamWaitEvent(ss, net->ev_side2[net->cur_lane], 0));
                rc = pitem_index(net, n, pos);
                net->pitem_on_side = rc == GRL_OK;
            }
        }
        net->h->stream = st;
        if (rc) return rc;
    }
    if (side) {
        NET_HIP(net, hipEventRecord(net->ev_side1[net->cur_lane], net->side_stream[net->cur_lane]));
        NET_HIP(net, hipStreamWaitEvent(st, net->ev_side1[net->cur_lane], 0));
    } else if (int rc = slot_index(net, pos, n)) return rc;
    if (net->expand2_gemm) {
        const int nb = (n + 255) / 256;
        hipLaunchKernelGGL(conv2_prep_kernel, dim3((n + 3) / 4), dim3(256), 0, st, net->sraw, pos, P + ConvOffsets::c1w, net->sbase, n, net->z2sh,
                           net->carow, net->ulist, net->cslot, net->d2s, side ? 2 : 3);
        if (!side) {
        hipLaunchKernelGGL(corr_count_kernel, dim3(nb), dim3(256), 0, st, pos, n, net->cblkcnt);
        hipLaunchKernelGGL(corr_offsets_kernel, dim3(1), dim3(256), 0, st, net->cblkcnt, nb, net->ctiles, net->cblkoff, net->cgoff, net->ctilegroup,
                           net->cperm);
        hipLaunchKernelGGL(corr_place_kernel, dim3(nb), dim3(256), 0, st, pos, n, net->cblkoff, net->cgoff, net->cperm, net->cinv);
        }
        CorrRows g{net->carow, net->cperm, net->ctilegroup, net->ctiles * 256};
        EpiConv2Corr e{net->d2s, net->m2s, net->cperm, net->cslot, net->expand3_gather && net->chunk <= (1u << 17) ? net->a2 : nullptr};
        net->prof_tag_cur = PT_CLASS_CORR;
        GemmTimer t(net, 2.0 * n * 128 * 576 * (6.25 / 9.0));
        launch_rowk<128, 64, 4, 1, CorrRows, EpiConv2Corr, true, true, 1, true>(net, dim3(576 / 64, net->ctiles * 2), st, g, net->w2corr, 128, 576, e);
    } else {
        hipLaunchKernelGGL(expand_conv2_kernel, dim3(nenv < 256 ? nenv : 256), dim3(1024), EXP2_LDS_BYTES, st, net->sraw, net->z2sh, pos,
                           P + ConvOffsets::c1w, P + ConvOffsets::c2w, nenv, net->a2sh, net->d2s, net->m2s, net->ulist, net->sbase);
    }
    NET_HIP(net, hipGetLastError());
    return side ? GRL_OK : patch_sort(net, n);
}

__global__ void reduce_agents_kernel(const float *__restrict__ src, int nenv, int per4, float *__restrict__ dst) {
    const size_t i = (size_t)blockIdx.x * blockDim.x + threadIdx.x;
    if (i >= (size_t)nenv * per4) return;
    const size_t e = i / per4, r = i - e * per4;
    float4 v[10];
#pragma unroll
    for (int a = 0; a < 10; ++a) v[a] = reinterpret_cast<const float4 *>(src)[(e * 10 + a) * per4 + r];
    float4 s = v[0];
#pragma unroll
    for (int a = 1; a < 10; ++a) { s.x += v[a].x; s.y += v[a].y; s.z += v[a].z; s.w += v[a].w; }
    reinterpret_cast<float4 *>(dst)[i] = s;
}

__global__ __launch_bounds__(256) void agent_dz2_kernel(const float *__restrict__ gsl, const unsigned long long *__restrict__ m2,
                                                        const float *__restrict__ a2sh, const signed char *__restrict__ ulist,
                                                        const int *__restrict__ sbase, int nenv, float *__restrict__ dz2, float *__restrict__ dza,
                                                        float *__restrict__ bsum, const unsigned *__restrict__ amask, int bgsum) {
    __shared__ __attribute__((aligned(16))) float corr[81 * 64];
    float4 cs = make_float4(0.f, 0.f, 0.f, 0.f);
    __shared__ int ul[90], sb[11], u0[10];
    __shared__ unsigned long long mw[90];
    __shared__ unsigned am[3];
    const int tid = threadIdx.x, sl = tid >> 4, c4 = (tid & 15) * 4;
    const float4 zero4 = make_float4(0.f, 0.f, 0.f, 0.f);
    for (int env = blockIdx.x; env < nenv; env += gridDim.x) {
        __syncthreads();
        for (int i = tid; i < 81 * 16; i += 256) reinterpret_cast<float4 *>(corr)[i] = zero4;
        if (tid < 11) sb[tid] = sbase[(size_t)env * 10 + tid];
        if (tid >= 64 && tid < 67) am[tid - 64] = amask ? amask[(size_t)env * 3 + tid - 64] : 0xFFFFFFFFu;
        __syncthreads();
        if (tid < 90) {
            const int a = tid / 9, j = tid - a * 9;
            const bool has = j < sb[a + 1] - sb[a];
            ul[tid] = has ? ulist[sb[a] + j] : -1;
            mw[tid] = has ? m2[(size_t)sb[a] + j] : 0ull;
        }
        float *dz = dz2 + (size_t)env * 5184;
        float4 dzv[6];
        unsigned okm = 0;
#pragma unroll
        for (int k = 0; k < 6; ++k) {
            const int i = tid + 256 * k, o = i >> 4;
            const bool ok = i < 81 * 16 && (!bgsum || ((am[o >> 5] >> (o & 31)) & 1u));
            dzv[k] = zero4;
            if (ok) dzv[k] = reinterpret_cast<const float4 *>(dz)[i];
            okm |= ok ? 1u << k : 0u;
        }
        __syncthreads();
        if (tid < 10) {
            int y0 = 99, x0 = 99;
            for (int j = 0; j < 9; ++j) {
                const int u = ul[tid * 9 + j];
                if (u < 0) continue;
                y0 = min(y0, u / 9); x0 = min(x0, u % 9);
            }
            u0[tid] = y0 > 8 ? 0 : y0 * 9 + x0;
        }
        const float *ash = a2sh + (size_t)env * 5184;
        int u = sl < sb[1] - sb[0] ? ul[sl] : -1;
        float4 g = zero4, sv = zero4;
        if (u >= 0) {
            g = *reinterpret_cast<const float4 *>(gsl + ((size_t)sb[0] + sl) * 64 + c4);
            sv = *reinterpret_cast<const float4 *>(ash + u * 64 + c4);
        }
        __syncthreads();
#pragma unroll
        for (int a = 0; a < 10; ++a) {
            int un = -1;
            float4 gn = zero4, svn = zero4;
            if (a < 9) {
                un = sl < sb[a + 2] - sb[a + 1] ? ul[(a + 1) * 9 + sl] : -1;
                if (un >= 0) {
                    gn = *reinterpret_cast<const float4 *>(gsl + ((size_t)sb[a + 1] + sl) * 64 + c4);
                    svn = *reinterpret_cast<const float4 *>(ash + un * 64 + c4);
                }
// ... 284 lines not shown
```

### golds-rl-gym_amd/csrc/net_train.inc

```

namespace grl {

static inline double host_now_ms() {
    return std::chrono::duration<double, std::milli>(std::chrono::steady_clock::now().time_since_epoch()).count();
}

static int rq_flush(grl_net *net) {
    const int nj = (int)net->rq.size();
    if (!nj) { net->slab_used = 0; net->slabb_used = 0; return GRL_OK; }
    std::vector<int> phase(nj, 0);
    int maxph = 0;
    for (int k = 0; k < nj; ++k) {
        for (int i = 0; i < k; ++i) phase[k] += net->rq_dst[i] == net->rq_dst[k];
        maxph = std::max(maxph, phase[k]);
    }
    for (int ph = 0; ph <= maxph; ++ph) {
        int k = 0;
        while (k < nj) {
            RBatch B;
            B.njobs = 0;
            int blocks = 0;
            for (; k < nj && B.njobs < kRJobs; ++k) {
                if (phase[k] != ph) continue;
                B.bstart[B.njobs] = blocks;
// ... 599 lines not shown
    if (rc == GRL_OK) rc = nalloc(net, &net->t2desc, (size_t)4 * net->npad);
    A(&net->dl2, (size_t)4 * net->npad * 32); A(&net->tt2, (size_t)4 * net->npad * 32);
    A(&net->tmpw2, 4 * 256 * 32);
    A(&net->gd1sh, (c / 10) * 512); A(&net->gsh3, (c / 10) * 3136); A(&net->g3p, c * 1600); A(&net->dz3p, c * 1600);
    net->slab_floats = ((size_t)112 << 20) + (size_t)net->pslices * 1600 * 512;
    A(&net->slab, net->slab_floats);
    net->slab_used = 0;
    A(&net->slab1h, (size_t)2048 * 2048);
    {
        size_t sb = ((size_t)c / 128 + 2) * kW128M * 512;
        sb = std::max(sb, ((size_t)(c / 10) * 100 / 128 + 2) * kW128M * 128);
        sb = std::max(sb, ((size_t)(c / 10) * 81 / 128 + 2) * 4 * 64);
        net->slabb_floats = 5 * sb + 4096;
        A(&net->slabb, net->slabb_floats);
        net->slabb_used = 0;
    }
    A(&net->slab1b, (size_t)3 * 2048 * 64);
    A(&net->cfold, (size_t)kFoldParts * 32);
    if (rc == GRL_OK) rc = nalloc(net, &net->slab64, kSlab64Doubles + 4096);
    A(&net->ro_mu, c * (3 * (size_t)net->ho.A + net->ho.dz + 3));
    if (rc == GRL_OK) net->train_ready = true;
    return rc;
}

template <int BM, int BN, int WGM, int WGN, class AG>
static int tn_launch(grl_net *net, int rd, AG ag, int I, const float *dY, int J, float *gdst, int accumulate = 1, double flop_rows = 0.0,
                     int min_chunks = 0, int wgs = 0) {
    const int M = ag.rows;
    const int tiles = (I / BM) * (J / BN);
    int chunks = ((wgs > 0 ? wgs : net->tn_wgs) + tiles - 1) / tiles;
    if (min_chunks > chunks) chunks = min_chunks;
    if (chunks > 1024) chunks = 1024;
    if ((size_t)chunks * I * J > slab_left(net)) chunks = (int)(slab_left(net) / ((size_t)I * J));
    if (chunks < 1) return nfail(net, GRL_E_INVALID, "tn_launch: slab too small");
    int mc = ((M + chunks - 1) / chunks + 31) / 32 * 32;
    chunks = (M + mc - 1) / mc;
    const long n = (long)I * J;
    float *slab = slab_take(net, (size_t)chunks * n);
    if (!slab) return nfail(net, GRL_E_INVALID, "tn_launch: slab too small");
    {
        GemmTimer t(net, 2.0 * (flop_rows > 0.0 ? flop_rows : (double)M) * (double)I * J);
        launch_tn<BM, BN, WGM, WGN, AG>(net, dim3(I / BM, J / BN, chunks), net->h->stream, ag, dY, J, mc, slab);
    }
    RJob j{};
    j.kind = RJ_SLAB; j.blocks = (int)((n + 255) / 256); j.i0 = chunks; j.i1 = accumulate; j.n = n; j.p0 = slab; j.d0 = gdst;
    rq_push(net, rd, j);
    NET_HIP(net, hipGetLastError());
    return GRL_OK;
}

__global__ __launch_bounds__(256) void slot_range_masks_kernel(const int *__restrict__ sperm, const unsigned short *__restrict__ stap,
                                                               const int *__restrict__ live, int mc, unsigned *__restrict__ zmask) {
    __shared__ unsigned part[4];
    const int beg = blockIdx.x * mc, end = min(*live, beg + mc);
    unsigned v = 0;
    for (int s = beg + threadIdx.x; s < end; s += 256) v |= stap[sperm[s]];
#pragma unroll
    for (int o = 32; o > 0; o >>= 1) v |= __shfl_xor(v, o, 64);
    if ((threadIdx.x & 63) == 0) part[threadIdx.x >> 6] = v;
    __syncthreads();
    if (threadIdx.x == 0) zmask[blockIdx.x] = part[0] | part[1] | part[2] | part[3];
}
static int slot_wgrad_launch(grl_net *net, int n, float *gw3, double flop_rows, int min_chunks) {
    constexpr int BM = 64, BN = 64, I = 576, J = 64;
    const int M = n * 9, tiles = (I / BM) * (J / BN);
    int chunks = (net->tn_wgs + tiles - 1) / tiles;
    if (net->swgrad_chunks > 0) min_chunks = net->swgrad_chunks;
    if (min_chunks > chunks) chunks = min_chunks;
    if (chunks > 1024) chunks = 1024;
    if ((size_t)chunks * I * J > slab_left(net)) chunks = (int)(slab_left(net) / ((size_t)I * J));
    if (chunks < 1) return nfail(net, GRL_E_INVALID, "slot_wgrad_launch: slab too small");
    const int mc = ((M + chunks - 1) / chunks + 31) / 32 * 32;
    chunks = (M + mc - 1) / mc;
    float *slab = slab_take(net, (size_t)chunks * I * J);
    if (!slab) return nfail(net, GRL_E_INVALID, "slot_wgrad_launch: slab too small");
    hipStream_t st = net->h->stream;
    const bool skip = net->patch_skip != 0;
    if (skip) hipLaunchKernelGGL(slot_range_masks_kernel, dim3(chunks), dim3(256), 0, st, net->sperm, net->stap, net->sbase + n, mc, net->szmask);
    SlotGatherT3P ag{net->dz3p, net->rowdesc, M, net->sbase + n, net->sperm, nullptr, skip ? net->szmask : nullptr};
    {
        GemmTimer t(net, 2.0 * flop_rows * (double)I * J * net->sfrac);
        if (net->swgrad_pair) {
            SlotGatherT3PPair gp{ag};
            launch_tn<128, BN, 2, 2, SlotGatherT3PPair>(net, dim3(5, J / BN, chunks), st, gp, net->d2s, J, mc, slab);
        } else
            launch_tn<BM, BN, 2, 2, SlotGatherT3P>(net, dim3(I / BM, J / BN, chunks), st, ag, net->d2s, J, mc, slab);
    }
    RJob j{};
    j.kind = RJ_TAPS_C3; j.blocks = I * J / 32; j.i0 = chunks; j.p0 = slab; j.p1 = skip ? net->szmask : nullptr; j.d0 = gw3;
    rq_push(net, RD_C3W, j);
    NET_HIP(net, hipGetLastError());
    return GRL_OK;
}

static int colsum_launch(grl_net *net, int rd, const float *dY, int M, int J, float *gdst) {
    if (J < 32 || J > 1024 || (J & (J - 1))) return nfail(net, GRL_E_INVALID, "colsum_launch: J must be a power of two in 32..1024");
    int chunks = (M + 31) / 32;
    if (chunks > 2048) chunks = 2048;
    int mc = (M + chunks - 1) / chunks;
    chunks = (M + mc - 1) / mc;
    float *slab = slab_take(net, (size_t)chunks * J);
    if (!slab) return nfail(net, GRL_E_INVALID, "colsum_launch: slab too small");
    hipLaunchKernelGGL(colsum_kernel, dim3(1, chunks), dim3(256), 0, net->h->stream, dY, M, J, mc, slab);
    RJob j{};
    j.kind = RJ_NARROW; j.blocks = (J + kNarrowCols - 1) / kNarrowCols; j.i0 = chunks; j.i1 = 1; j.n = J; j.p0 = slab; j.d0 = gdst;
    rq_push(net, rd, j);
    NET_HIP(net, hipGetLastError());
    return GRL_OK;
}

static void csum_reduce(grl_net *net, int rd, const float *csum, int rows, int J, float *bias_dst) {
    const int parts = (rows + 127) / 128 * kW128M;
    RJob j{};
    j.kind = RJ_NARROW; j.blocks = (J + kNarrowCols - 1) / kNarrowCols; j.i0 = parts; j.i1 = 1; j.n = J; j.p0 = csum; j.d0 = bias_dst;
    rq_push(net, rd, j);
}

template <int BM, int BN, int WGM, int WGN, bool FENCE = true, int NBUF = 1, bool ACC1 = false, class AG, class Epi>
static void rowk_launch(grl_net *net, AG ag, const float *W, int ldb, int N, Epi epi, double flops) {
    GemmTimer t(net, flops);
    launch_rowk<BM, BN, WGM, WGN, AG, Epi, true, FENCE, NBUF, ACC1>(net, dim3(N / BN, (ag.rows + BM - 1) / BM), net->h->stream, ag, W, ldb, N, epi);
}

static int resident_grid(const void *kernel, int cap) {
    int per_cu = 0, dev = 0;
    hipDeviceProp_t prop;
    if (hipOccupancyMaxActiveBlocksPerMultiprocessor(&per_cu, kernel, 256, 0) != hipSuccess || hipGetDevice(&dev) != hipSuccess ||
        hipGetDeviceProperties(&prop, dev) != hipSuccess || per_cu < 1) {
        (void)hipGetLastError();
        return cap;
    }
    const long g = (long)per_cu * prop.multiProcessorCount;
    return g < cap ? (int)g : cap;
}

static int backward_chunk_body(grl_net *net, const TrainBufs &tb, const uint8_t *lb, const uint8_t *ab, const uint8_t *pos, int nenv,
                               const float *actions, const float *adv, const float *y, float inv_total, long slot,
                               const float *pmu, const float *psg, const float *pval);
static void rq_reset(grl_net *net) {
    net->rq.clear(); net->rq_dst.clear();
    net->slab_used = 0; net->slabb_used = 0;
}
static int backward_chunk(grl_net *net, const TrainBufs &tb, const uint8_t *lb, const uint8_t *ab, const uint8_t *pos, int nenv,
                          const float *actions, const float *adv, const float *y, float inv_total, long slot = -1,
                          const float *pmu = nullptr, const float *psg = nullptr, const float *pval = nullptr) {
    if (!net->rq.empty() || net->slab_used || net->slabb_used) {
        rq_reset(net);
        return nfail(net, GRL_E_INVALID, "backward_chunk: reductions of an earlier chunk were still queued");
    }
    const int rc = backward_chunk_body(net, tb, lb, ab, pos, nenv, actions, adv, y, inv_total, slot, pmu, psg, pval);
    if (rc != GRL_OK) rq_reset(net);
    return rc;
}
static int backward_chunk_body(grl_net *net, const TrainBufs &tb, const uint8_t *lb, const uint8_t *ab, const uint8_t *pos, int nenv,
                               const float *actions, const float *adv, const float *y, float inv_total, long slot,
                               const float *pmu, const float *psg, const float *pval) {
    hipStream_t st = net->h->stream;
    const float *P = net->params;
    float *Gr = net->grads;
    const int n = nenv * 10;
    bind_activations(net, slot);
    const bool have_heads = slot >= 0 && pmu && psg && pval;
    int rc = forward_chunk(net, lb, ab, pos, nenv, tb.cmu, tb.csigma, tb.cvs, slot >= 0, have_heads);
    if (rc) return rc;
    if (net->shared_trunk && net->obs_index && (rc = obs_index(net, lb, ab, pos, nenv, net->obsrec, st, 2))) return rc;
    const float *hmu = have_heads ? pmu : tb.cmu, *hsg = have_heads ? psg : tb.csigma, *hvs = have_heads ? pval : tb.cvs;
    const HeadOff &ho = net->ho;
    const int HS = heads_slab(ho.A), NW = 1024 * ho.A + 2 * ho.A;
    int chunks = (n + 4 * kHeadRows - 1) / (4 * kHeadRows);
    if (chunks > 1024) chunks = 1024;
    const int HS2 = HS + 768;
    float *hslab = slab_take(net, (size_t)chunks * HS2);
    if (!hslab) return nfail(net, GRL_E_INVALID, "backward_chunk: slab too small for the heads");
    GRL_HEADS_DISPATCH(ho.A, hipLaunchKernelGGL(heads_backward_kernel<kA>, dim3(chunks), dim3(256), 0, st, net->p1, net->v2,
                                                hmu, hsg, hvs, actions, adv, y, P, ho, n, net->cfg.scale, net->cfg.entropy_beta, inv_total,
                                                (const float *)(net->stats + kLossScaleAt), net->gp1, net->gv2, tb.dzh, tb.stats64, hslab));
    {
        RJob j{};
        j.kind = RJ_HEADS; j.blocks = (HS2 + kNarrowCols - 1) / kNarrowCols; j.i0 = chunks; j.i1 = NW; j.i2 = HS; j.i3 = HS2; j.p0 = hslab;
        j.d0 = Gr + ho.muw; j.p1 = Gr + ho.v3w; j.p2 = Gr + ConvOffsets::p1b; j.p3 = Gr + net->ho.v2b; j.d1 = tb.stats64;
        rq_push(net, RD_HEADS, j);
    }
    net->prof_tag_cur = net->shared_trunk ? PT_DENSE_DGRAD : PT_PER_AGENT;
    const size_t csum_floats = ((size_t)n / 128 + 2) * kW128M * 512;
    float *cs1 = slabb_take(net, csum_floats), *cs2 = slabb_take(net, csum_floats), *cs3 = slabb_take(net, csum_floats);
    if (!cs1 || !cs2 || !cs3) return nfail(net, GRL_E_INVALID, "backward_chunk: column-sum buffer too small");
    rowk_launch<128, 128, kW128M, kW128N>(net, DenseRows{net->gv2, n, 256, 256}, P + ho.v2w, 256, 512,
                                      EpiGradSumBits{net->gv1, 512, net->mb_v1, cs1}, 2.0 * n * 256 * 512);
    csum_reduce(net, RD_V1B, cs1, n, 512, Gr + ho.v1b);
    rowk_launch<128, 128, kW128M, kW128N, true, 2>(net, DenseRowsPair{net->gp1, n, 512, 512, (int)(net->gv1 - net->gp1), (int)(ho.v1w - ConvOffsets::p1w)},
                                P + ConvOffsets::p1w, 512, 256, EpiGradSumBits{net->gd2, 256, net->mb_d2, cs2}, 2.0 * n * 1024 * 256);
    csum_reduce(net, RD_D2B, cs2, n, 256, Gr + ConvOffsets::d2b);
    rowk_launch<128, 128, kW128M, kW128N>(net, DenseRows{net->gd2, n, 256, 256}, P + ConvOffsets::d2w, 256, 512,
                                      EpiGradSum{net->gd1, 512, net->d1, cs3}, 2.0 * n * 256 * 512);
    csum_reduce(net, RD_D1B, cs3, n, 512, Gr + ConvOffsets::d1b);
    if (!net->shared_trunk)
        rowk_launch<256, 64, kW256M, kW256N>(net, DenseRows{net->gd1, n, 512, 512}, P + ConvOffsets::d1w, 512, 3136,
                                   EpiGrad{net->ga3, 3136, net->a3}, 2.0 * n * 512 * 3136);
    if (net->shared_trunk) {
        hipLaunchKernelGGL(reduce_agents_kernel, dim3((unsigned)(((size_t)nenv * 128 + 255) / 256)), dim3(256), 0, st, net->gd1, nenv, 128,
                           net->gd1sh);
        net->prof_tag_cur = PT_ENV_DGRAD;
        const bool trunk3 = net->trunk_skip && net->expand2_gemm;
        if (trunk3) {
            int cch = (nenv + 31) / 32;
            if (cch > 2048) cch = 2048;
            const int cmc = (nenv + cch - 1) / cch;
            cch = (nenv + cmc - 1) / cmc;
            float *gslab = slab_take(net, (size_t)cch * 512);
            if (!gslab) return nfail(net, GRL_E_INVALID, "backward_chunk: slab too small");
            hipLaunchKernelGGL(colsum_kernel, dim3(1, cch), dim3(256), 0, st, (const float *)net->gd1sh, nenv, 512, cmc, gslab);
            hipLaunchKernelGGL(slab_reduce_narrow_kernel, dim3((512 + kNarrowCols - 1) / kNarrowCols), dim3(256), 0, st, gslab, cch, 512, net->tug, 0);
            rowk_launch<256, 64, kW256M, kW256N>(net, DenseRowsNU{{net->gd1sh, nenv, 512, 512}, net->tumask}, P + ConvOffsets::d1w, 512, 3136,
                                       EpiStore{net->gsh3, 3136}, 2.0 * nenv * 512 * 64.0 * trunk_union_pixels(net));
        } else {
            rowk_launch<256, 64, kW256M, kW256N>(net, DenseRows{net->gd1sh, nenv, 512, 512}, P + ConvOffsets::d1w, 512, 3136,
                                       EpiStore{net->gsh3, 3136}, 2.0 * nenv * 512 * 3136);
        }
        {
            PatchRows g{net->gd1, net->perm, net->tilegroup, net->ptiles * 256, 512, 512, 1, nullptr, nullptr, net->patch_skip ? net->tmask : nullptr, nullptr};
            net->prof_tag_cur = PT_PATCH_DGRAD;
            GemmTimer t(net, 2.0 * n * 512 * 1600 * net->pfrac[1]);
            if (net->pdgrad_pair) {
                PatchRowsPairN gp{g};
                launch_rowk<128, 128, kW128M, kW128N, PatchRowsPairN, EpiPermStore, true>(net, dim3(13, net->ptiles * 2), st, gp, P + ConvOffsets::d1w, 512, 1600,
                                                                                          EpiPermStore{net->g3p, net->perm, 1600});
            } else if (net->pdgrad_xcd)
                launch_rowk<256, 64, kW256M, kW256N, PatchRows, EpiPermStore, true>(net, dim3(1600 / 64, net->ptiles), st, g, P + ConvOffsets::d1w, 512, 1600, EpiPermStore{net->g3p, net->perm, 1600});
            else
                launch_rowk<256, 64, kW256M, kW256N, PatchRows, EpiPermStore, false>(net, dim3(1600 / 64, net->ptiles), st, g, P + ConvOffsets::d1w, 512, 1600, EpiPermStore{net->g3p, net->perm, 1600});
        }
        static const int hg3 = resident_grid((const void *)agent_dz3_kernel, 2048);
        maybe_evict(net);
        hipLaunchKernelGGL(agent_dz3_kernel, dim3(nenv < hg3 ? nenv : hg3), dim3(256), 0, st, net->gsh3, net->g3p, net->a3sh, net->m3,
                           net->org, net->patch_skip ? net->smask : nullptr, nenv, net->dz3sh, net->dz3p, net->slab1b,
                           trunk3 ? (const unsigned *)net->tcmask : (const unsigned *)nullptr, trunk3 ? net->tslab + 2048 * 64 : (float *)nullptr,
                           trunk3 ? (const float *)(net->tbgz3 + 64) : (const float *)nullptr,
                           trunk3 ? (const unsigned *)net->tumask : (const unsigned *)nullptr);
        if (trunk3) {
            RJob two[2] = {};
            two[0].kind = RJ_NARROW; two[0].blocks = (64 + kNarrowCols - 1) / kNarrowCols; two[0].i0 = nenv < hg3 ? nenv : hg3; two[0].i1 = 0; two[0].n = 64;
            two[0].p0 = net->tslab + 2048 * 64; two[0].d0 = net->tsums + 128;
            two[1] = two[0]; two[1].p0 = net->slab1b; two[1].d0 = net->tsums + 192;
            rb_launch(net, two, 2);
            hipLaunchKernelGGL(trunk_upix_kernel, dim3(49), dim3(256), 0, st, P + ConvOffsets::d1w, (const float *)net->tug, (const unsigned *)net->tumask,
                               net->tuspix);
            hipLaunchKernelGGL(trunk_uadd_kernel, dim3(1), dim3(64), 0, st, (const float *)net->tuspix, (const float *)(net->tbgz3 + 64), net->tsums);
        } else {
            RJob j{};
            j.kind = RJ_NARROW; j.blocks = (64 + kNarrowCols - 1) / kNarrowCols; j.i0 = nenv < hg3 ? nenv : hg3; j.i1 = 1; j.n = 64; j.p0 = net->slab1b; j.d0 = Gr + ConvOffsets::c3b;
            rq_push(net, RD_C3B, j);
        }
        net->prof_tag_cur = PT_ENV_DGRAD;
        if (trunk3) {
            float *cs4 = slabb_take(net, ((size_t)nenv * 81 / 128 + 2) * 4 * 64);
            if (!cs4) return nfail(net, GRL_E_INVALID, "backward_chunk: column-sum buffer too small");
            rowk_launch<128, 64, 4, 1, false, 1, true>(net, GatherT3Rows{net->dz3sh, net->trowlist, net->trows_n, nenv * 81}, net->w3t, 576, 64,
                                       EpiGradRowsSum{net->dz2, 64, net->a2sh, cs4, net->trowlist, net->trows_n},
                                       2.0 * trunk_live(net, 0, (double)nenv * 81) * 576 * 64);
            hipLaunchKernelGGL(colsum_live_kernel, dim3(kLiveParts), dim3(256), 0, st, (const float *)cs4, (const int *)net->trows_n, 128, 4, 64,
                               net->cfold);
        } else if (nenv % 256 == 0)
            rowk_launch<256, 64, 4, 1, false>(net, GatherT3PM{net->dz3sh, nenv * 81, nenv}, net->w3t, 576, 64,
                                       EpiGradPM{net->dz2, net->a2sh, nenv, 81, 64}, 2.0 * nenv * 441 * 64 * 64);
        else
            rowk_launch<256, 64, 4, 1, false>(net, GatherT3{net->dz3sh, nenv * 81}, net->w3t, 576, 64, EpiGrad{net->dz2, 64, net->a2sh},
                                       2.0 * nenv * 81 * 576 * 64);
        net->prof_tag_cur = PT_SLOT_DGRAD;
        hipLaunchKernelGGL(slot_rowdesc_kernel, dim3((n * 9 + 255) / 256), dim3(256), 0, st, net->rowagent, net->ulist, net->org, net->sbase + n,
                           net->sperm, n * 9, net->rowdesc);
        {
            SlotGatherT3P g3{net->dz3p, net->rowdesc, n * 9, net->sbase + n, net->sperm, net->patch_skip ? net->stmask : nullptr, nullptr};
            GemmTimer t(net, 2.0 * slot_rows_for_flops(net, n) * 576 * 64 * net->sfrac);
            launch_rowk<128, 64, 4, 1, SlotGatherT3P, EpiPermStore, true, true, 1, true>(net, dim3(1, (n * 9 + 127) / 128), st, g3, net->w3t, 576, 64,
                                                                                         EpiPermStore{net->gsl, net->sperm, 64});
        }
        static const int hg2 = resident_grid((const void *)agent_dz2_kernel, 2048);
        maybe_evict(net);
        const bool trunk = net->trunk_skip && net->expand2_gemm;
        float *slab1b_dz2 = net->slab1b + (size_t)2048 * 64;
        hipLaunchKernelGGL(agent_dz2_kernel, dim3(nenv < hg2 ? nenv : hg2), dim3(256), 0, st, net->gsl, net->m2s, net->a2sh, net->ulist,
                           net->sbase, nenv, net->dz2, net->dza, slab1b_dz2, trunk ? (const unsigned *)net->tamask : (const unsigned *)nullptr,
                           trunk ? 1 : 0);
        if (trunk) {
            hipLaunchKernelGGL(slab_reduce_narrow_kernel, dim3((64 + kNarrowCols - 1) / kNarrowCols), dim3(256), 0, st, slab1b_dz2, nenv < hg2 ? nenv : hg2, 64, net->tsums, 0);
            hipLaunchKernelGGL(trunk_closed3_kernel, dim3(1), dim3(256), 0, st, P + ConvOffsets::c3w, (const float *)(net->tbgz + 64),
                               (const float *)net->cfold, net->tsums, Gr + ConvOffsets::c3b);
        } else {
            RJob j{};
            j.kind = RJ_NARROW; j.blocks = (64 + kNarrowCols - 1) / kNarrowCols; j.i0 = nenv < hg2 ? nenv : hg2; j.i1 = 1; j.n = 64; j.p0 = slab1b_dz2; j.d0 = Gr + ConvOffsets::c2b;
            rq_push(net, RD_C2B, j);
        }
        net->prof_tag_cur = PT_ENV_DGRAD;
        float *cs5 = slabb_take(net, ((size_t)nenv * 100 / 128 + 2) * kW128M * 128);
        if (!cs5) return nfail(net, GRL_E_INVALID, "backward_chunk: column-sum buffer too small");
        if (trunk) {
            rowk_launch<128, 128, 2, 2, false>(net, GatherT2Rows{net->dz2, net->tblklist, net->trows_n + 1, nenv * 100}, net->w2t, 256, 128,
                                        EpiGradStride2Rows{net->gt, net->sraw, cs5, P + ConvOffsets::c1b, net->tblklist, net->trows_n + 1},
                                        2.0 * trunk_live(net, 1, (double)nenv * 100) * 256 * 128);
            hipLaunchKernelGGL(fold_class_sums_kernel, dim3(kFoldParts), dim3(256), 0, st, cs5, (nenv * 100 + 127) / 128 * 2, net->cfold,
                               (const int *)(net->trows_n + 1));
        } else {
            rowk_launch<128, 128, 2, 2, false>(net, GatherT2{net->dz2, nenv * 100}, net->w2t, 256, 128,
                                        EpiGradStride2<true, true>{net->gt, net->sraw, cs5}, 2.0 * nenv * 100 * 256 * 128);
            hipLaunchKernelGGL(fold_class_sums_kernel, dim3(kFoldParts), dim3(256), 0, st, cs5, (nenv * 100 + 127) / 128 * 2, net->cfold,
                               (const int *)nullptr);
        }
        {
            RJob j{};
            j.kind = RJ_FOLDFINAL; j.blocks = 1; j.p0 = net->cfold; j.d0 = Gr + ConvOffsets::c1b;
            rq_push(net, RD_C1B, j);
        }
    } else {
    if (n % 256 == 0)
        rowk_launch<256, 64, 4, 1, false>(net, GatherT3PM{net->ga3, n * 81, n}, net->w3t, 576, 64, EpiGradPM{net->ga2, net->a2, n, 81, 64},
                                   2.0 * n * 441 * 64 * 64);
    else
        rowk_launch<256, 64, 4, 1, false>(net, GatherT3{net->ga3, n * 81}, net->w3t, 576, 64, EpiGrad{net->ga2, 64, net->a2},
                                   2.0 * n * 81 * 576 * 64);
    rowk_launch<128, 128, 2, 2, false>(net, GatherT2{net->ga2, n * 100}, net->w2t, 256, 128, EpiGradStride2<true>{net->ga1, net->a1, nullptr},
                                2.0 * n * 100 * 256 * 128);
    }
    NET_HIP(net, hipGetLastError());
    net->prof_tag_cur = net->shared_trunk ? PT_DENSE_WGRAD : PT_PER_AGENT;
    if ((rc = tn_launch<128, 128, 2, 2>(net, RD_V2W, DenseRows{net->v1, n, 512, 512}, 512, net->gv2, 256, Gr + net->ho.v2w, 1, 0.0, 0, net->tn_wgs_dense))) return rc;
    if ((rc = tn_launch<128, 128, 2, 2>(net, RD_V1W, DenseRows{net->d2, n, 256, 256}, 256, net->gv1, 512, Gr + net->ho.v1w, 1, 0.0, 0, net->tn_wgs_dense))) return rc;
    if ((rc = tn_launch<128, 128, 2, 2>(net, RD_P1W, DenseRows{net->d2, n, 256, 256}, 256, net->gp1, 512, Gr + ConvOffsets::p1w, 1, 0.0, 0, net->tn_wgs_dense))) return rc;
    if ((rc = tn_launch<128, 128, 2, 2>(net, RD_D2W, DenseRows{net->d1, n, 512, 512}, 512, net->gd2, 256, Gr + ConvOffsets::d2w, 1, 0.0, 0, net->tn_wgs_dense))) return rc;
    if (net->shared_trunk) {
        net->prof_tag_cur = PT_ENV_WGRAD;
        if (net->trunk_skip && net->expand2_gemm) {
            constexpr int I = 3136, J = 512, tiles = (I / 64) * (J / 128);
            int chunks = (net->tn_wgs + tiles - 1) / tiles;
            if ((size_t)chunks * I * J > slab_left(net)) chunks = (int)(slab_left(net) / ((size_t)I * J));
            if (chunks < 1) return nfail(net, GRL_E_INVALID, "dense1 per-env weight gradient: slab too small");
            const int mc = ((nenv + chunks - 1) / chunks + 31) / 32 * 32;
            chunks = (nenv + mc - 1) / mc;
            float *slab = slab_take(net, (size_t)chunks * I * J);
            if (!slab) return nfail(net, GRL_E_INVALID, "dense1 per-env weight gradient: slab too small");
            {
                GemmTimer t(net, 2.0 * nenv * 64.0 * trunk_union_pixels(net) * J);
                launch_tn<64, 128, 2, 2, DenseRowsIU>(net, dim3(I / 64, J / 128, chunks), st, DenseRowsIU{{net->a3sh, nenv, 3136, 3136}, net->tumask},
                                                      net->gd1sh, J, mc, slab);
            }
            RJob j{};
            j.kind = RJ_UMASK; j.blocks = (int)(((long)I * J + 255) / 256); j.i0 = chunks; j.n = (long)I * J; j.p0 = slab; j.p1 = net->tumask;
            j.p2 = net->tbgz3 + 64; j.p3 = net->tug; j.d0 = Gr + ConvOffsets::d1w;
            rq_push(net, RD_D1W, j);
        } else if ((rc = tn_launch<64, 128, 2, 2>(net, RD_D1W, DenseRows{net->a3sh, nenv, 3136, 3136}, 3136, net->gd1sh, 512, Gr + ConvOffsets::d1w))) return rc;
        {
            float *pslab = slab_take(net, (size_t)net->pslices * 1600 * 512);
            if (!pslab) return nfail(net, GRL_E_INVALID, "backward_chunk: slab too small for the patch slices");
            PatchRows g{net->d3, net->perm, net->tilegroup, net->ptiles * 256, 1600, 1600, 0, net->sbeg, net->send, net->patch_skip ? net->tmask : nullptr,
                        net->patch_skip ? net->zmask : nullptr};
            {
                net->prof_tag_cur = PT_PATCH_WGRAD;
                GemmTimer t(net, 2.0 * n * 1600 * 512 * net->pfrac[2]);
                if (net->pwgrad_pair) {
                    PatchRowsPair gp{g};
                    if (net->pwgrad_xcd == 1)
                        launch_tn<128, 128, 2, 2, PatchRowsPair, 1>(net, dim3(13, 512 / 128, net->pslices), st, gp, net->gd1, 512, 0, pslab);
                    else
                        launch_tn<128, 128, 2, 2, PatchRowsPair, 0>(net, dim3(13, 512 / 128, net->pslices), st, gp, net->gd1, 512, 0, pslab);
                } else if (net->pwgrad_xcd == 1)
                    launch_tn<64, 128, 2, 2, PatchRows, 1>(net, dim3(1600 / 64, 512 / 128, net->pslices), st, g, net->gd1, 512, 0, pslab);
                else if (net->pwgrad_xcd == 2)
                    launch_tn<64, 128, 2, 2, PatchRows, 2>(net, dim3(1600 / 64, 512 / 128, net->pslices), st, g, net->gd1, 512, 0, pslab);
                else
                    launch_tn<64, 128, 2, 2, PatchRows, 0>(net, dim3(1600 / 64, 512 / 128, net->pslices), st, g, net->gd1, 512, 0, pslab);
            }
            RJob j{};
            j.kind = RJ_PATCH; j.blocks = 3136 * 128 / 256; j.i0 = net->pslices; j.p0 = pslab; j.p1 = net->sgrp; j.p2 = net->patch_skip ? net->zmask : nullptr;
            j.d0 = Gr + ConvOffsets::d1w;
            rq_push(net, RD_D1W, j);
        }
    } else {
        if ((rc = tn_launch<64, 128, 2, 2>(net, RD_D1W, DenseRows{net->a3, n, 3136, 3136}, 3136, net->gd1, 512, Gr + ConvOffsets::d1w))) return rc;
    }
    if (net->shared_trunk) {
        net->prof_tag_cur = PT_ENV_WGRAD;
        if (net->trunk_skip && net->expand2_gemm) {
            constexpr int I = 576, J = 64, tiles = (I / 64) * (J / 64);
            int chunks = (net->tn_wgs + tiles - 1) / tiles;
            if ((size_t)chunks * I * J > slab_left(net)) chunks = (int)(slab_left(net) / ((size_t)I * J));
            if (chunks < 1) return nfail(net, GRL_E_INVALID, "conv3 weight gradient: slab too small");
            float *slab = slab_take(net, (size_t)chunks * I * J);
            if (!slab) return nfail(net, GRL_E_INVALID, "conv3 weight gradient: slab too small");
            GatherConv3Rows ag{net->a2sh, net->tc3list, net->trows_n + 2, net->tbgimg3, nenv * 49, chunks};
            {
                GemmTimer t(net, 2.0 * trunk_live(net, 2, (double)nenv * 49) * I * J);
                launch_tn<64, 64, 2, 2, GatherConv3Rows>(net, dim3(I / 64, J / 64, chunks), st, ag, net->dz3sh, J, 0, slab);
            }
            RJob j{};
            j.kind = RJ_SLAB; j.blocks = (I * J + 255) / 256; j.i0 = chunks; j.i1 = 1; j.n = (long)I * J; j.p0 = slab; j.d0 = Gr + ConvOffsets::c3w;
            rq_push(net, RD_C3W, j);
            RJob r{};
            r.kind = RJ_RANK1; r.blocks = I * J / 256; r.i0 = 63; r.p0 = net->tbgz + 64; r.p1 = net->tsums + 128; r.d0 = Gr + ConvOffsets::c3w;
            rq_push(net, RD_C3W, r);
        } else if ((rc = tn_launch<64, 64, 2, 2>(net, RD_C3W, GatherConv3{net->a2sh, nenv * 49}, 576, net->dz3sh, 64, Gr + ConvOffsets::c3w))) return rc;
        net->prof_tag_cur = PT_SLOT_WGRAD;
        if ((rc = slot_wgrad_launch(net, n, Gr + ConvOffsets::c3w, slot_rows_for_flops(net, n), 684))) return rc;
        net->prof_tag_cur = PT_ENV_WGRAD;
        if (net->trunk_skip && net->expand2_gemm) {
            constexpr int I = 512, J = 64, tiles = (I / 128) * (J / 64);
            int chunks = (net->tn_wgs + tiles - 1) / tiles;
            if ((size_t)chunks * I * J > slab_left(net)) chunks = (int)(slab_left(net) / ((size_t)I * J));
            if (chunks < 1) return nfail(net, GRL_E_INVALID, "conv2 weight gradient: slab too small");
            float *slab = slab_take(net, (size_t)chunks * I * J);
            if (!slab) return nfail(net, GRL_E_INVALID, "conv2 weight gradient: slab too small");
            GatherConv2ReluRows ag{net->sraw, net->trowlist, net->trows_n, net->tbgimg, nenv * 81, chunks};
            {
                GemmTimer t(net, 2.0 * trunk_live(net, 0, (double)nenv * 81) * I * J);
                launch_tn<128, 64, 2, 2, GatherConv2ReluRows>(net, dim3(I / 128, J / 64, chunks), st, ag, net->dz2, J, 0, slab);
            }
            RJob j{};
            j.kind = RJ_SLAB; j.blocks = (I * J + 255) / 256; j.i0 = chunks; j.i1 = 1; j.n = (long)I * J; j.p0 = slab; j.d0 = Gr + ConvOffsets::c2w;
            rq_push(net, RD_C2W, j);
            RJob w{};
            w.kind = RJ_CLOSED_W; w.blocks = 128; w.p0 = P + ConvOffsets::c1b; w.p1 = net->tsums + 64; w.d0 = Gr + ConvOffsets::c2w;
            rq_push(net, RD_C2W, w);
            RJob b1{};
            b1.kind = RJ_CLOSED_B1; b1.blocks = 1; b1.p0 = P + ConvOffsets::c1b; b1.p1 = P + ConvOffsets::c2w; b1.p2 = net->tsums; b1.d0 = Gr + ConvOffsets::c1b;
            rq_push(net, RD_C1B, b1);
            RJob b2{};
            b2.kind = RJ_CLOSED_B2; b2.blocks = 1; b2.p0 = net->tsums; b2.d0 = Gr + ConvOffsets::c2b;
            rq_push(net, RD_C2B, b2);
        } else if ((rc = tn_launch<128, 64, 2, 2>(net, RD_C2W, GatherConv2Relu{net->sraw, nenv * 81}, 512, net->dz2, 64, Gr + ConvOffsets::c2w))) return rc;
    } else {
        if ((rc = tn_launch<64, 64, 2, 2>(net, RD_C3W, GatherConv3{net->a2, n * 49}, 576, net->ga3, 64, Gr + ConvOffsets::c3w))) return rc;
        if ((rc = tn_launch<128, 64, 2, 2>(net, RD_C2W, GatherConv2{net->a1, n * 81}, 512, net->ga2, 64, Gr + ConvOffsets::c2w))) return rc;
    }
    if (!net->shared_trunk && (rc = colsum_launch(net, RD_C3B, net->ga3, n * 49, 64, Gr + ConvOffsets::c3b))) return rc;
    int blocks = nenv < 512 ? nenv : 512;
    if (net->shared_trunk) {
        static const int hgs = resident_grid((const void *)agent_ds_kernel, 2048);
        const int dblocks = nenv < hgs ? nenv : hgs, npad = net->npad;
        maybe_evict(net);
        const int t2rows = (n + 127) / 128 * 128;
        hipLaunchKernelGGL(gather_t2_kernel, dim3((t2rows + kT2Agents - 1) / kT2Agents), dim3(256), 0, st, net->sraw, pos, net->ulist, net->sbase,
                           P + ConvOffsets::c1w, n, npad, t2rows, net->t2desc, net->dl2);
        net->prof_tag_cur = PT_CLASS_CORR;
        {
            const int cpc = 64;
            const int mc = ((n + cpc - 1) / cpc + 31) / 32 * 32;
            T2SlotGather g{net->dza, net->t2desc, 4 * npad, npad, n, 32, cpc};
            {
                GemmTimer t(net, 4 * 2.0 * n * 256 * 32);
                launch_rowk<128, 32, 4, 1, T2SlotGather, EpiStore>(net, dim3(1, 4 * npad / 128), st, g, net->w2t, 256, 32, EpiStore{net->tt2, 32});
            }
            float *cslab = slab_take(net, (size_t)4 * cpc * 8192);
            if (!cslab) return nfail(net, GRL_E_INVALID, "class corrections: slab too small");
            {
                GemmTimer t(net, 4 * 2.0 * n * 256 * 32);
                launch_tn<64, 32, 4, 1, T2SlotGather>(net, dim3(256 / 64, 1, 4 * cpc), st, g, net->dl2, 32, mc, cslab);
            }
            RJob j{};
            j.kind = RJ_GROUPS_C2; j.blocks = 4 * 8192 / 256; j.i0 = cpc; j.p0 = cslab; j.d0 = Gr + ConvOffsets::c2w;
            rq_push(net, RD_C2W, j);
        }
        float *slab1h = net->slab1h, *slab1b_ds = net->slab1b + (size_t)2 * 2048 * 64;
        if (net->obs_index)
            hipLaunchKernelGGL(agent_ds_indexed_kernel, dim3(dblocks), dim3(256), 0, st, net->sraw, (const unsigned *)net->obsrec, net->tt2, npad, net->gt,
                               P + ConvOffsets::c1w, nenv, slab1h, slab1b_ds);
        else
            hipLaunchKernelGGL(agent_ds_kernel, dim3(dblocks), dim3(256), 0, st, net->sraw, pos, net->tt2, npad, net->gt, P + ConvOffsets::c1w,
                               nenv, slab1h, slab1b_ds);
        {
            RJob j{};
            j.kind = RJ_ONEHOT; j.blocks = 2048 / 16; j.i0 = dblocks; j.p0 = slab1h; j.d0 = Gr + ConvOffsets::c1w;
            rq_push(net, RD_C1W_HOT, j);
            RJob b{};
            b.kind = RJ_NARROW; b.blocks = (32 + kNarrowCols - 1) / kNarrowCols; b.i0 = dblocks; b.i1 = 1; b.n = 32; b.p0 = slab1b_ds; b.d0 = Gr + ConvOffsets::c1b;
            rq_push(net, RD_C1B, b);
        }
        static const int hgw = resident_grid((const void *)conv1_wgrad_shared_kernel, 1536);
        const int wblocks = nenv < hgw ? nenv : hgw;
        if (net->obs_index)
            hipLaunchKernelGGL(conv1_wgrad_indexed_kernel, dim3(wblocks), dim3(256), 0, st, (const unsigned *)net->obsrec, (const float *)net->gt, nenv,
                               net->slab64);
        else
            hipLaunchKernelGGL(conv1_wgrad_shared_kernel, dim3(wblocks), dim3(256), 0, st, lb, ab, (const float *)net->gt, nenv,
                               net->h->cfg.grid_size, net->slab64);
        RJob j{};
        j.kind = RJ_SLAB64; j.blocks = 4096 / 16; j.i0 = wblocks; j.p0 = net->slab64; j.d0 = Gr + ConvOffsets::c1w;
        rq_push(net, RD_C1W_CNT, j);
    } else {
        if ((rc = colsum_launch(net, RD_C2B, net->ga2, n * 81, 64, Gr + ConvOffsets::c2b))) return rc;
        if ((rc = colsum_launch(net, RD_C1B, net->ga1, n * 400, 32, Gr + ConvOffsets::c1b))) return rc;
        hipLaunchKernelGGL(conv1_wgrad_kernel, dim3(blocks), dim3(256), 0, st, lb, ab, pos, net->ga1, nenv, net->h->cfg.grid_size,
                           net->slab64, (const float *)nullptr);
    }
    if (!net->shared_trunk)
        hipLaunchKernelGGL(slab64_reduce_kernel, dim3(6144 / 256), dim3(256), 0, st, net->slab64, blocks, 6144, Gr + ConvOffsets::c1w);
    NET_HIP(net, hipGetLastError());
    return rq_flush(net);
}

static int train_begin(grl_net *net, TrainBufs *tb) {
    static_assert(sizeof(double) == 8, "");
    const size_t c = net->chunk;
    const int nl = lanes_active(net);
    hipStream_t main_st = net->lane_stream[0];
    rq_reset(net);
    for (int k = nl - 1; k >= 0; --k) {
        use_lane(net, k);
        int rc = ensure_train_bufs(net);
        if (rc) return rc;
        float *base = net->ro_mu;
        const size_t A = net->ho.A, dz = net->ho.dz;
        tb[k].cmu = base; tb[k].csigma = base + c * A; tb[k].cvs = base + c * 2 * A; tb[k].dzh = tb[k].cvs + c; tb[k].cact = tb[k].dzh + c * dz;
        tb[k].cadv = tb[k].cact + c * A; tb[k].cy = tb[k].cadv + c;
        tb[k].stats64 = net->slab64 + kSlab64Doubles;
        tb[k].partial = tb[k].stats64 + 8;
        NET_HIP(net, hipMemsetAsync(net->grads, 0, net->ho.total * 4, main_st));
        NET_HIP(net, hipMemsetAsync(tb[k].stats64, 0, 8 * sizeof(double), main_st));
    }
    hipLaunchKernelGGL(transpose_conv_weights_kernel, dim3((576 * 64 + 255) / 256), dim3(256), 0, main_st,
                       net->params + ConvOffsets::c2w, net->params + ConvOffsets::c3w, net->w2t, net->w3t);
    NET_HIP(net, hipMemsetAsync(net->stats + kLossBoundAt, 0, sizeof(float), main_st));
    NET_HIP(net, hipGetLastError());
    return GRL_OK;
}

static int train_bound_rows(grl_net *net, const float *mu, const float *sigma, const float *vs, const float *actions, const float *adv,
                            const float *y, long n) {
    GRL_HEADS_DISPATCH(net->ho.A, hipLaunchKernelGGL(head_bound_kernel<kA>, dim3((unsigned)std::min<long>((n + 255) / 256, 2048)), dim3(256), 0, net->lane_stream[0], mu,
                                                     sigma, vs, actions, adv, y, n, net->cfg.scale, net->cfg.entropy_beta,
                                                     reinterpret_cast<unsigned *>(net->stats + kLossBoundAt)));
    NET_HIP(net, hipGetLastError());
    return GRL_OK;
}

static int train_scale_and_fork(grl_net *net, float inv_total) {
    hipLaunchKernelGGL(loss_scale_kernel, dim3(1), dim3(64), 0, net->lane_stream[0], reinterpret_cast<const unsigned *>(net->stats + kLossBoundAt),
                       inv_total, net->loss_scale_on, net->stats + kLossScaleAt);
    NET_HIP(net, hipGetLastError());
    return lanes_fork(net);
// ... 492 lines not shown
```

Before: 2.265 million env-steps/s.

## Add depth-two register prefetch to gemm kernels, enabled for conv2 weight-grad by default

Adds a second register staging set to the row-gather and TN GEMM kernels, so global loads for tile k+2 are in flight while tile k is stored to LDS and multiplied. The goal is to hide gather-load latency in memory-bound conv GEMMs. A per-call-site bitmask picks which launches use it, and by default only the conv2 rows TN weight-gradient kernel does. The extra registers lower the occupancy bound (launch_bounds of 3 for 4-wave kernels) and may cause spills.

```diff
diff --git a/golds-rl-gym_amd/csrc/net_conv.hip b/golds-rl-gym_amd/csrc/net_conv.hip
--- a/golds-rl-gym_amd/csrc/net_conv.hip
+++ b/golds-rl-gym_amd/csrc/net_conv.hip
@@ -123,6 +123,7 @@
     int f32_by_fallback, f32_clean_passes, range_return_k, range_returns;
     float absmax_last;
     int loss_scale_on;
+    unsigned pf_mask;
     int acc1;
     int expand3_gather;
     int expand2_gemm, ctiles;
@@ -236,9 +237,30 @@
     PT_ENV_WGRAD, PT_SLOT_FWD, PT_SLOT_DGRAD, PT_SLOT_WGRAD, PT_CLASS_CORR, PT_PER_AGENT, PT_COUNT
 };
 
-template <int BM, int BN, int WGM, int WGN, class AG, class Epi, int XCD = 1, bool FENCE = true, int NBUF = 1, bool ACC1 = false>
+enum {
+    PF_NONE = 0, PF_SLOTS_TO_PATCH, PF_CORR_ROWS, PF_SLOT_T3P, PF_T3_ROWS, PF_CONV2_ROWS, PF_DENSE_KU, PF_T2_SLOT,
+    PF_TN_SLOT_T3P, PF_TN_SLOT_T3P_PAIR, PF_TN_CONV3_ROWS, PF_TN_CONV2_ROWS, PF_TN_DENSE_IU, PF_TN_T2_SLOT, PF_COUNT
+};
+constexpr unsigned kPfAuto = 1u << (PF_TN_CONV2_ROWS - 1);
+#define GRL_PF_ON(net_, pfi_) ((pfi_) > 0 && !(net_)->gemm_f32 && (((net_)->pf_mask >> ((pfi_) > 0 ? (pfi_) - 1 : 0)) & 1u))
+
+template <int BM, int BN, int WGM, int WGN, class AG, class Epi, int XCD = 1, bool FENCE = true, int NBUF = 1, bool ACC1 = false, int PFI = PF_NONE>
 static void launch_rowk(grl_net *net, dim3 grid, hipStream_t st, AG ag, const float *Bt, int ldb, int N, Epi epi) {
     constexpr bool kAcc1 = ACC1 && ((WGM * WGN == 8 && BM == 128 && BN == 128) || (WGM * WGN == 4 && BM * BN <= 128 * 64));
+    if constexpr (PFI != PF_NONE) {
+        constexpr bool kEh = PFI == PF_T3_ROWS;
+        constexpr bool kTwoAccFits = !(PFI == PF_SLOTS_TO_PATCH || PFI == PF_SLOT_T3P);
+        if (GRL_PF_ON(net, PFI)) {
+            if (kAcc1 && net->acc1) {
+                hipLaunchKernelGGL((gemm_rowk<BM, BN, WGM, WGN, AG, Epi, XCD, FENCE, false, NBUF, kAcc1, 2, kEh>), grid, dim3(64 * WGM * WGN), 0, st, ag, Bt, ldb, N, epi);
+                return;
+            }
+            if constexpr (kTwoAccFits) {
+                hipLaunchKernelGGL((gemm_rowk<BM, BN, WGM, WGN, AG, Epi, XCD, FENCE, false, NBUF, false, 2, false>), grid, dim3(64 * WGM * WGN), 0, st, ag, Bt, ldb, N, epi);
+                return;
+            }
+        }
+    }
     if (net->gemm_f32)
         hipLaunchKernelGGL((gemm_rowk<BM, BN, WGM, WGN, AG, Epi, XCD, FENCE, true, NBUF, false>), grid, dim3(64 * WGM * WGN), 0, st, ag, Bt, ldb, N, epi);
     else if (kAcc1 && net->acc1)
@@ -246,8 +268,14 @@
     else
         hipLaunchKernelGGL((gemm_rowk<BM, BN, WGM, WGN, AG, Epi, XCD, FENCE, false, NBUF, false>), grid, dim3(64 * WGM * WGN), 0, st, ag, Bt, ldb, N, epi);
 }
-template <int BM, int BN, int WGM, int WGN, class AG, int XCD = 1>
+template <int BM, int BN, int WGM, int WGN, class AG, int XCD = 1, int PFI = PF_NONE>
 static void launch_tn(grl_net *net, dim3 grid, hipStream_t st, AG ag, const float *dY, int J, int mc, float *slab) {
+    if constexpr (PFI != PF_NONE) {
+        if (GRL_PF_ON(net, PFI)) {
+            hipLaunchKernelGGL((gemm_tn<BM, BN, WGM, WGN, AG, XCD, false, 2>), grid, dim3(64 * WGM * WGN), 0, st, ag, dY, J, mc, slab);
+            return;
+        }
+    }
     if (net->gemm_f32) hipLaunchKernelGGL((gemm_tn<BM, BN, WGM, WGN, AG, XCD, true>), grid, dim3(64 * WGM * WGN), 0, st, ag, dY, J, mc, slab);
     else hipLaunchKernelGGL((gemm_tn<BM, BN, WGM, WGN, AG, XCD, false>), grid, dim3(64 * WGM * WGN), 0, st, ag, dY, J, mc, slab);
 }
@@ -964,6 +992,8 @@
         n->expand2_gemm = (e2 && strcmp(e2, "lds") == 0) ? 0 : 1;
         { const char *e3 = getenv("GRL_NET_EXPAND3"); n->expand3_gather = (e3 && strcmp(e3, "prod") == 0) ? 0 : 1;
           const char *a1 = getenv("GRL_NET_ACC1"); n->acc1 = (a1 && strcmp(a1, "off") == 0) ? 0 : 1; }
+        { const char *pf = getenv("GRL_GEMM_PF");
+          n->pf_mask = (pf && strcmp(pf, "1") == 0) ? 0u : (pf && strcmp(pf, "2") == 0) ? (1u << (PF_COUNT - 1)) - 1u : kPfAuto; }
     }
     n->pslice_rows = PATCH_SLICE_ROWS; n->pwgrad_xcd = 1;
     if (const char *e = getenv("GRL_PATCH_SLICE")) { const int v = atoi(e); if (v == 256 || v == 512 || v == 1024 || v == 2048 || v == 4096 || v == 8192) n->pslice_rows = v; }
diff --git a/golds-rl-gym_amd/csrc/net_gemm.h b/golds-rl-gym_amd/csrc/net_gemm.h
--- a/golds-rl-gym_amd/csrc/net_gemm.h
+++ b/golds-rl-gym_amd/csrc/net_gemm.h
@@ -945,8 +945,8 @@
 template <class T, class = void> struct ag_pair_i : std::false_type {};
 template <class T> struct ag_pair_i<T, std::void_t<decltype(T::kPairI)>> : std::bool_constant<T::kPairI> {};
 
-template <int BM, int BN, int WGM, int WGN, class AG, class Epi, int XCD_ORDER = 1, bool FENCE = true, bool F32 = false, int NBUF = 1, bool ACC1 = false>
-__global__ __launch_bounds__(64 * WGM * WGN, ACC1 ? (WGM * WGN == 8 ? 6 : 4) : WGM * WGN / 2) void gemm_rowk(AG ag, const float *__restrict__ Bt, int ldb, int N, Epi epi) {
+template <int BM, int BN, int WGM, int WGN, class AG, class Epi, int XCD_ORDER = 1, bool FENCE = true, bool F32 = false, int NBUF = 1, bool ACC1 = false, int PF = 1, bool EH = false>
+__global__ __launch_bounds__(64 * WGM * WGN, PF == 2 && WGM * WGN == 4 ? 3 : ACC1 ? (WGM * WGN == 8 ? 6 : 4) : WGM * WGN / 2) void gemm_rowk(AG ag, const float *__restrict__ Bt, int ldb, int N, Epi epi) {
     constexpr int BK = 32, LDH = kLdh, NT = 64 * WGM * WGN, RPP = NT / 8;
     constexpr int WM = BM / WGM, WN = BN / WGN, TM = WM / 16, TN = WN / 16;
     constexpr int NA = BM / RPP;
@@ -1005,10 +1005,13 @@
     const float *brow0 = Bt + (long)(ag.bn(PAIRN ? pp.x * 64 : n0, m0) + trow) * ldb + tk4;
     const float *brow1 = PAIRN ? Bt + (long)(ag.bn(max(pp.y, pp.x) * 64, m0) + trow) * ldb + tk4 : brow0 + (long)RPP * ldb;
 
-    float4 ra[NA];
-    float4 rb0 = make_float4(0.f, 0.f, 0.f, 0.f), rb1 = rb0, rb2 = rb0, rb3 = rb0;
-    unsigned vmask = 0;
-#define GRL_LOAD_TILE(kt_)                                                                                 \
+    static_assert(PF == 1 || (PF == 2 && !F32), "prefetch depth 1 or 2; the fp32 form keeps 1");
+    float4 ra_a[NA], ra_b[NA];
+    float4 rb0_a = make_float4(0.f, 0.f, 0.f, 0.f), rb1_a = rb0_a, rb2_a = rb0_a, rb3_a = rb0_a;
+    float4 rb0_b = rb0_a, rb1_b = rb0_a, rb2_b = rb0_a, rb3_b = rb0_a;
+    unsigned vmask_a = 0, vmask_b = 0;
+#define GRL_LOAD_TILE(kt_) GRL_LOAD_TILE_S(kt_, _a)
+#define GRL_LOAD_TILE_S(kt_, S_)                                                                              \
     {                                                                                                      \
         int toff, ty, tx;                                                                                  \
         ag.tap((kt_) * BK, toff, ty, tx);                                                                  \
@@ -1016,16 +1019,16 @@
             int iy0 = ayx[i] >> 16, ix0 = (int)(int16_t)(ayx[i] & 0xFFFF);                                 \
             bool v = arow_ok[i] && ag.ok(iy0, ix0, ty, tx);                                                \
              \
-              \
-            ra[i] = *reinterpret_cast<const float4 *>(ag.base + (v ? aoff[i] + toff : 0L) + tk4);          \
-            vmask = v ? (vmask | (1u << i)) : (vmask & ~(1u << i));    \
+                                          \
+            ra##S_[i] = *reinterpret_cast<const float4 *>(ag.base + (v ? aoff[i] + toff : 0L) + tk4);      \
+            vmask##S_ = v ? (vmask##S_ | (1u << i)) : (vmask##S_ & ~(1u << i));    \
         }                                                                                                  \
                      \
         const int bko = ag_bk(ag, wctx, m0, (kt_) * BK);                                                             \
-        rb0 = *reinterpret_cast<const float4 *>(brow0 + bko);                                              \
-        if (NB > 1) rb1 = *reinterpret_cast<const float4 *>(brow1 + bko);                                  \
-        if (NB > 2) rb2 = *reinterpret_cast<const float4 *>(brow0 + (long)2 * RPP * ldb + bko);            \
-        if (NB > 2) rb3 = *reinterpret_cast<const float4 *>(brow0 + (long)3 * RPP * ldb + bko);            \
+        rb0##S_ = *reinterpret_cast<const float4 *>(brow0 + bko);                                          \
+        if (NB > 1) rb1##S_ = *reinterpret_cast<const float4 *>(brow1 + bko);                              \
+        if (NB > 2) rb2##S_ = *reinterpret_cast<const float4 *>(brow0 + (long)2 * RPP * ldb + bko);        \
+        if (NB > 2) rb3##S_ = *reinterpret_cast<const float4 *>(brow0 + (long)3 * RPP * ldb + bko);        \
     }
 #define GRL_STORE_PLANES(S_, row_, v4_)                                                                    \
     {                                                                                                      \
@@ -1049,19 +1052,20 @@
             *reinterpret_cast<uint2 *>(&S_[2][(row_) * LDH + wo]) = make_uint2(__builtin_bit_cast(unsigned, s0_), __builtin_bit_cast(unsigned, s1_)); \
         }                                                                                                  \
     }
-#define GRL_STORE_TILE(buf_)                                                                               \
+#define GRL_STORE_TILE(buf_) GRL_STORE_TILE_S(buf_, _a)
+#define GRL_STORE_TILE_S(buf_, S_)                                                                         \
     {                                                                                                      \
         _Pragma("unroll") for (int i = 0; i < NA; ++i) {                                                   \
-            const bool v = (vmask >> i) & 1u;                                                              \
-            float4 t4 = ra[i];                                                                             \
+            const bool v = (vmask##S_ >> i) & 1u;                                                          \
+            float4 t4 = ra##S_[i];                                                                           \
             t4.x = v ? t4.x : 0.f; t4.y = v ? t4.y : 0.f; t4.z = v ? t4.z : 0.f; t4.w = v ? t4.w : 0.f;    \
             if (AG::kRelu) { t4.x = fmaxf(t4.x, 0.f); t4.y = fmaxf(t4.y, 0.f); t4.z = fmaxf(t4.z, 0.f); t4.w = fmaxf(t4.w, 0.f); } \
             GRL_STORE_PLANES(As[buf_], trow + RPP * i, t4)                                                 \
         }                                                                                                  \
-        GRL_STORE_PLANES_B(Bs[buf_], trow, rb0)                                                            \
-        if (NB > 1) GRL_STORE_PLANES_B(Bs[buf_], trow + RPP, rb1)                                          \
-        if (NB > 2) GRL_STORE_PLANES_B(Bs[buf_], trow + 2 * RPP, rb2)                                      \
-        if (NB > 2) GRL_STORE_PLANES_B(Bs[buf_], trow + 3 * RPP, rb3)                                      \
+        GRL_STORE_PLANES_B(Bs[buf_], trow, rb0##S_)                                                        \
+        if (NB > 1) GRL_STORE_PLANES_B(Bs[buf_], trow + RPP, rb1##S_)                                      \
+        if (NB > 2) GRL_STORE_PLANES_B(Bs[buf_], trow + 2 * RPP, rb2##S_)                                  \
+        if (NB > 2) GRL_STORE_PLANES_B(Bs[buf_], trow + 3 * RPP, rb3##S_)                                  \
     }
 
     f32x4 acc[TM][TN], acl[ACC1 ? 1 : TM][ACC1 ? 1 : TN];
@@ -1079,10 +1083,28 @@
     int kt = 0;
     while (kt < nk && !ag_tile_ok(ag, wctx, m0, kt * BK)) ++kt;
     GRL_LOAD_TILE(kt < nk ? kt : 0)
+    int kt1 = nk;
+    if constexpr (PF == 2) {
+        kt1 = kt < nk ? kt + 1 : nk;
+        while (kt1 < nk && !ag_tile_ok(ag, wctx, m0, kt1 * BK)) ++kt1;
+        GRL_LOAD_TILE_S(kt1 < nk ? kt1 : (kt < nk ? kt : 0), _b)
+    }
     const int l16 = lane & 15, kg = lane >> 4;
     const int ro = (kg ^ swz(l16)) << 3;
     const int aro = (wm * WM + l16) * LDH + ro;
     const int bro = (wn * WN + l16) * LDH + ro;
+    int rax_h[EH ? TM : 1][4];
+    if constexpr (EH) {
+        const int hcolbase = PAIRN ? ((wn == 0 ? pp.x : pp.y) < 0 ? N : (wn == 0 ? pp.x : pp.y) * 64) : n0 + wn * WN;
+        const int hrow = m0 + wm * WM + 4 * kg;
+#pragma unroll
+        for (int a = 0; a < TM; ++a)
+#pragma unroll
+            for (int r = 0; r < 4; ++r) {
+                if constexpr (epi_row_bits<Epi>::value || epi_row_auxn<Epi>::value) rax_h[a][r] = epi.row_aux_n(min(hrow + a * 16 + r, M - 1), hcolbase);
+                else rax_h[a][r] = epi.row_aux(min(hrow + a * 16 + r, M - 1));
+            }
+    }
 #define GRL_MFMA_TILE(cb_)                                                                                                             \
     {                                                                                                                                  \
         if constexpr (F32) {                                                                                                           \
@@ -1121,7 +1143,65 @@
             }                                                                                                                          \
         }                                                                                                                              \
     }
-    if constexpr (NBUF == 1) {
+#define GRL_NEXT_TILE(dst_, k_)                                                                            \
+    {                                                                                                      \
+        dst_ = (k_) < nk ? (k_) + 1 : nk;                                                                  \
+        while (dst_ < nk && !ag_tile_ok(ag, wctx, m0, dst_ * BK)) ++dst_;                                  \
+    }
+#define GRL_PF2_STEP(S_, kc_, kn_)                                                                         \
+    {                                                                                                      \
+        GRL_STORE_TILE_S(0, S_)                                                                            \
+        __syncthreads();                                                                                   \
+        int k2_;                                                                                           \
+        GRL_NEXT_TILE(k2_, kn_)                                                                            \
+        {                                                                                                  \
+            const int ktl = k2_ < nk ? k2_ : kc_;                                                          \
+            GRL_LOAD_TILE_S(ktl, S_)                                                                       \
+        }                                                                                                  \
+        if constexpr (FENCE) { GRL_SCHED_FENCE }                                                           \
+        GRL_MFMA_TILE(0)                                                                                   \
+        if constexpr (FENCE) { GRL_SCHED_FENCE }                                                           \
+        __syncthreads();                                                                                   \
+        kc_ = k2_;                                                                                         \
+    }
+    if constexpr (PF == 2 && NBUF == 1) {
+        while (kt < nk) {
+            GRL_PF2_STEP(_a, kt, kt1)
+            if (kt1 >= nk) break;
+            GRL_PF2_STEP(_b, kt1, kt)
+        }
+    } else if constexpr (PF == 2) {
+        int kt2 = nk;
+        if (kt < nk) {
+            GRL_STORE_TILE_S(0, _a)
+            GRL_NEXT_TILE(kt2, kt1)
+            GRL_LOAD_TILE_S(kt2 < nk ? kt2 : kt, _a)
+            __syncthreads();
+        }
+#define GRL_PF2_HALF(S_, cb_, kc_, kn_, kf_)       \
+    {                                                                                                      \
+        int k3_ = nk;                                                                                      \
+        if (kn_ < nk) {                                                                 \
+            GRL_STORE_TILE_S(cb_ ^ 1, S_)                                                                  \
+            GRL_NEXT_TILE(k3_, kf_)                                                                        \
+            GRL_LOAD_TILE_S(k3_ < nk ? k3_ : kn_, S_)                                                      \
+        }                                                                                                  \
+        if constexpr (FENCE) { GRL_SCHED_FENCE }                                                           \
+        GRL_MFMA_TILE(cb_)                                                                                 \
+        if constexpr (FENCE) { GRL_SCHED_FENCE }                                                           \
+        __syncthreads();                                                                                   \
+        kc_ = k3_;                                                                                         \
+    }
+        while (kt < nk) {
+            GRL_PF2_HALF(_b, 0, kt, kt1, kt2)
+            if (kt1 >= nk) break;
+            GRL_PF2_HALF(_a, 1, kt1, kt2, kt)
+            if (kt2 >= nk) break;
+            const int t0 = kt2, t1 = kt, t2 = kt1;
+            kt = t0; kt1 = t1; kt2 = t2;
+        }
+#undef GRL_PF2_HALF
+    } else if constexpr (NBUF == 1) {
         while (kt < nk) {
             GRL_STORE_TILE(0)
             __syncthreads();
@@ -1165,6 +1245,8 @@
         }
     }
 #undef GRL_MFMA_TILE
+#undef GRL_PF2_STEP
+#undef GRL_NEXT_TILE
     if constexpr (!F32) {
 #pragma unroll
         for (int a = 0; a < TM; ++a)
@@ -1186,7 +1268,8 @@
     for (int a = 0; a < TM; ++a)
 #pragma unroll
         for (int r = 0; r < 4; ++r) {
-            if constexpr (epi_row_bits<Epi>::value || epi_row_auxn<Epi>::value) rax[a][r] = epi.row_aux_n(min(erow + a * 16 + r, M - 1), ecolbase);
+            if constexpr (EH) rax[a][r] = rax_h[EH ? a : 0][r];
+            else if constexpr (epi_row_bits<Epi>::value || epi_row_auxn<Epi>::value) rax[a][r] = epi.row_aux_n(min(erow + a * 16 + r, M - 1), ecolbase);
             else rax[a][r] = epi.row_aux(min(erow + a * 16 + r, M - 1));
         }
 #pragma unroll
@@ -1246,13 +1329,15 @@
             }
     }
 #undef GRL_LOAD_TILE
+#undef GRL_LOAD_TILE_S
 #undef GRL_STORE_TILE
+#undef GRL_STORE_TILE_S
 #undef GRL_STORE_PLANES
 #undef GRL_STORE_PLANES_B
 }
 
-template <int BM, int BN, int WGM, int WGN, class AG, int XCD_ORDER = 1, bool F32 = false>
-__global__ __launch_bounds__(64 * WGM * WGN, WGM * WGN / 2) void gemm_tn(AG ag, const float *__restrict__ dY, int J, int mc, float *__restrict__ slab) {
+template <int BM, int BN, int WGM, int WGN, class AG, int XCD_ORDER = 1, bool F32 = false, int PF = 1>
+__global__ __launch_bounds__(64 * WGM * WGN, PF == 2 && WGM * WGN == 4 && BM * BN <= 64 * 64 ? 3 : WGM * WGN / 2) void gemm_tn(AG ag, const float *__restrict__ dY, int J, int mc, float *__restrict__ slab) {
     constexpr int BK = 32, LDH = kLdh, NT = 64 * WGM * WGN;
     constexpr int WM = BM / WGM, WN = BN / WGN, TM = WM / 16, TN = WN / 16;
     constexpr int A4 = BM / 4, B4 = BN / 4;
@@ -1311,38 +1396,39 @@
     const int ma = NA * ga, mb = NB * gb;
     const int acol = PAIR ? toff + (ca & 15) * 4 : toff + ca * 4;
     const bool ahalf_ok = !PAIR || ca < 16 || pp.y >= 0;
-    float4 ra[NA], rb[NB];
-    unsigned vma = 0, vmb = 0;
-    int2 ia[NA];
-    int ib[NB];
-    unsigned iva = 0;
-#define GRL_LOAD_IDX(mt_)                                                                                          \
+    static_assert(PF == 1 || (PF == 2 && !F32), "prefetch depth 1 or 2; the fp32 form keeps 1");
+    float4 ra_a[NA], rb_a[NB], ra_b[NA], rb_b[NB];
+    unsigned vma_a = 0, vmb_a = 0, vma_b = 0, vmb_b = 0;
+    int2 ia_a[NA], ia_b[NA];
+    int ib_a[NB], ib_b[NB];
+    unsigned iva_a = 0, iva_b = 0;
+#define GRL_LOAD_IDX(mt_, S_)                                                                                      \
     {                                                                                                              \
         _Pragma("unroll") for (int i = 0; i < NA; ++i) {                                                           \
             const int m = (mt_) + ma + i;                                                                          \
-            ia[i] = ag.ahandle(m < mend ? m : mbeg);                                                               \
-            iva = (m < mend && ag.hvalid(ia[i])) ? (iva | (1u << i)) : (iva & ~(1u << i));                         \
+            ia##S_[i] = ag.ahandle(m < mend ? m : mbeg);                                                           \
+            iva##S_ = (m < mend && ag.hvalid(ia##S_[i])) ? (iva##S_ | (1u << i)) : (iva##S_ & ~(1u << i));         \
         }                                                                                                          \
         _Pragma("unroll") for (int i = 0; i < NB; ++i) {                                                           \
             const int m = (mt_) + mb + i;                                                                          \
-            ib[i] = ag.bhandle(m < mend ? m : mbeg);                                                               \
-            if (m >= mend) ib[i] = -1;                                                                             \
+            ib##S_[i] = ag.bhandle(m < mend ? m : mbeg);                                                           \
+            if (m >= mend) ib##S_[i] = -1;                                                                         \
         }                                                                                                          \
     }
-#define GRL_LOAD_TILE()                                                                                            \
+#define GRL_LOAD_TILE(S_)                                                                                          \
     {                                                                                                              \
         _Pragma("unroll") for (int i = 0; i < NA; ++i) {                                                           \
-            const bool inr = (iva >> i) & 1u;                                                                      \
+            const bool inr = (iva##S_ >> i) & 1u;                                                                  \
             long off; int iy0, ix0;                                                                                \
-            ag.rowh(ia[i], off, iy0, ix0);                                                                         \
+            ag.rowh(ia##S_[i], off, iy0, ix0);                                                                     \
             const bool v = inr && ahalf_ok && ag.ok(iy0, ix0, ty, tx);                                             \
-            ra[i] = *reinterpret_cast<const float4 *>(ag.base + (v ? off + acol : (long)(ca * 4)));                \
-            vma = v ? (vma | (1u << i)) : (vma & ~(1u << i));                                                      \
+            ra##S_[i] = *reinterpret_cast<const float4 *>(ag.base + (v ? off + acol : (long)(ca * 4)));            \
+            vma##S_ = v ? (vma##S_ | (1u << i)) : (vma##S_ & ~(1u << i));                                          \
         }                                                                                                          \
         _Pragma("unroll") for (int i = 0; i < NB; ++i) {                                                           \
-            const bool v = ib[i] >= 0;                                                                             \
-            rb[i] = *reinterpret_cast<const float4 *>(dY + (long)(v ? ib[i] : 0) * J + j0 + cb * 4);               \
-            vmb = v ? (vmb | (1u << i)) : (vmb & ~(1u << i));                                                      \
+            const bool v = ib##S_[i] >= 0;                                                                         \
+            rb##S_[i] = *reinterpret_cast<const float4 *>(dY + (long)(v ? ib##S_[i] : 0) * J + j0 + cb * 4);       \
+            vmb##S_ = v ? (vmb##S_ | (1u << i)) : (vmb##S_ & ~(1u << i));                                          \
         }                                                                                                          \
     }
 #define GRL_TN_OFF(rho_, m_) ((rho_) * LDH + ((((m_) >> 3) ^ swz(rho_)) << 3) + ((m_) & 7))
@@ -1373,28 +1459,28 @@
         }                                                                                                          \
         }                                                                                                          \
     }
-#define GRL_STORE_TILE()                                                                                           \
+#define GRL_STORE_TILE(S_)                                                                                         \
     {                                                                                                              \
         _Pragma("unroll") for (int i = 0; i < NA; ++i) {                                                           \
-            const bool v = (vma >> i) & 1u;                                                                        \
-            float4 t4 = ra[i];                                                                                     \
+            const bool v = (vma##S_ >> i) & 1u;                                                                    \
+            float4 t4 = ra##S_[i];                                                                                 \
             t4.x = v ? t4.x : 0.f; t4.y = v ? t4.y : 0.f; t4.z = v ? t4.z : 0.f; t4.w = v ? t4.w : 0.f;            \
             if (AG::kRelu) { t4.x = fmaxf(t4.x, 0.f); t4.y = fmaxf(t4.y, 0.f); t4.z = fmaxf(t4.z, 0.f); t4.w = fmaxf(t4.w, 0.f); } \
-            ra[i] = t4;                                                                                            \
+            ra##S_[i] = t4;                                                                                        \
         }                                                                                                          \
-        GRL_STORE_RUN(As, NA, 0 * A4 + ca, ma, ra, x)                                                  \
-        GRL_STORE_RUN(As, NA, 1 * A4 + ca, ma, ra, y)                                                  \
-        GRL_STORE_RUN(As, NA, 2 * A4 + ca, ma, ra, z)                                                  \
-        GRL_STORE_RUN(As, NA, 3 * A4 + ca, ma, ra, w)                                                  \
+        GRL_STORE_RUN(As, NA, 0 * A4 + ca, ma, ra##S_, x)                                              \
+        GRL_STORE_RUN(As, NA, 1 * A4 + ca, ma, ra##S_, y)                                              \
+        GRL_STORE_RUN(As, NA, 2 * A4 + ca, ma, ra##S_, z)                                              \
+        GRL_STORE_RUN(As, NA, 3 * A4 + ca, ma, ra##S_, w)                                              \
         _Pragma("unroll") for (int i = 0; i < NB; ++i) {                                                           \
-            const bool v = (vmb >> i) & 1u;                                                                        \
-            float4 t4 = rb[i];                                                                                     \
+            const bool v = (vmb##S_ >> i) & 1u;                                                                    \
+            float4 t4 = rb##S_[i];                                                                                 \
             t4.x = v ? t4.x : 0.f; t4.y = v ? t4.y : 0.f; t4.z = v ? t4.z : 0.f; t4.w = v ? t4.w : 0.f;            \
-            rb[i] = t4;                                                                                            \
+            rb##S_[i] = t4;                                                                                        \
         }                                                                                                          \
         if (NB == 1 && !F32) {       \
             const bool odd = gb & 1;                                                                               \
-            const float4 t4 = rb[0];                                                                               \
+            const float4 t4 = rb##S_[0];                                                                           \
             const float o0 = __shfl_xor(odd ? t4.x : t4.z, B4), o1 = __shfl_xor(odd ? t4.y : t4.w, B4);            \
             unsigned h0, l0, h1, l1;                                                                               \
             split2(odd ? o1 : t4.x, odd ? t4.w : o0, h0, l0);       \
@@ -1405,10 +1491,10 @@
             *reinterpret_cast<unsigned *>(&Bs[0][q1]) = h1;                                                        \
             *reinterpret_cast<unsigned *>(&Bs[1][q1]) = l1;                                                        \
         } else {                                                                                                   \
-        GRL_STORE_RUN(Bs, NB, 0 * B4 + cb, mb, rb, x)                                                  \
-        GRL_STORE_RUN(Bs, NB, 1 * B4 + cb, mb, rb, y)                                                  \
-        GRL_STORE_RUN(Bs, NB, 2 * B4 + cb, mb, rb, z)                                                  \
-        GRL_STORE_RUN(Bs, NB, 3 * B4 + cb, mb, rb, w)                                                  \
+        GRL_STORE_RUN(Bs, NB, 0 * B4 + cb, mb, rb##S_, x)                                              \
+        GRL_STORE_RUN(Bs, NB, 1 * B4 + cb, mb, rb##S_, y)                                              \
+        GRL_STORE_RUN(Bs, NB, 2 * B4 + cb, mb, rb##S_, z)                                              \
+        GRL_STORE_RUN(Bs, NB, 3 * B4 + cb, mb, rb##S_, w)                                              \
         }                                                                                                          \
     }
     f32x4 acc[TM][TN], acl[TM][TN];
@@ -1422,52 +1508,69 @@
     const int ro = (kg ^ swz(l16)) << 3;
     const int aro = (wm * WM + l16) * LDH + ro;
     const int bro = (wn * WN + l16) * LDH + ro;
+#define GRL_TN_MFMA() \
+        { \
+            if constexpr (F32) { \
+                mfma_f32_step<TM, TN>(reinterpret_cast<const float *>(&As[0][0]), reinterpret_cast<const float *>(&Bs[0][0]), \
+                                      wm * WM + l16, wn * WN + l16, kg, acc); \
+            } else if constexpr (TM < TN) { \
+                f16x8 af[TM][2]; \
+                _Pragma("unroll") for (int a = 0; a < TM; ++a) \
+                    _Pragma("unroll") for (int p = 0; p < 2; ++p) af[a][p] = *reinterpret_cast<const f16x8 *>(&As[p][aro + a * 16 * LDH]); \
+                _Pragma("unroll") for (int b = 0; b < TN; ++b) { \
+                    f16x8 bf[2]; \
+                    _Pragma("unroll") for (int p = 0; p < 2; ++p) bf[p] = *reinterpret_cast<const f16x8 *>(&Bs[p][bro + b * 16 * LDH]); \
+                    _Pragma("unroll") for (int a = 0; a < TM; ++a) mfma_x3(acc[a][b], acl[a][b], af[a], bf); \
+                } \
+            } else { \
+                f16x8 bf[TN][2]; \
+                _Pragma("unroll") for (int b = 0; b < TN; ++b) \
+                    _Pragma("unroll") for (int p = 0; p < 2; ++p) bf[b][p] = *reinterpret_cast<const f16x8 *>(&Bs[p][bro + b * 16 * LDH]); \
+                _Pragma("unroll") for (int a = 0; a < TM; ++a) { \
+                    f16x8 af[2]; \
+                    _Pragma("unroll") for (int p = 0; p < 2; ++p) af[p] = *reinterpret_cast<const f16x8 *>(&As[p][aro + a * 16 * LDH]); \
+                    _Pragma("unroll") for (int b = 0; b < TN; ++b) mfma_x3(acc[a][b], acl[a][b], af, bf[b]); \
+                } \
+            } \
+        }
     if (mbeg < mend) {
-        GRL_LOAD_IDX(mbeg)
-        GRL_LOAD_TILE()
-        GRL_LOAD_IDX(mbeg + BK)
+        if constexpr (PF == 2) {
+            GRL_LOAD_IDX(mbeg, _a)
+            GRL_LOAD_IDX(mbeg + BK, _b)
+            GRL_LOAD_TILE(_a)
+            GRL_LOAD_TILE(_b)
+            GRL_LOAD_IDX(mbeg + 2 * BK, _a)
+            GRL_LOAD_IDX(mbeg + 3 * BK, _b)
+            for (int mt = mbeg; mt < mend; mt += 2 * BK) {
+                GRL_STORE_TILE(_a)
+                __syncthreads();
+                GRL_LOAD_TILE(_a)
+                GRL_LOAD_IDX(mt + 4 * BK, _a)
+                GRL_TN_MFMA()
+                __syncthreads();
+                if (mt + BK >= mend) break;
+                GRL_STORE_TILE(_b)
+                __syncthreads();
+                GRL_LOAD_TILE(_b)
+                GRL_LOAD_IDX(mt + 5 * BK, _b)
+                GRL_TN_MFMA()
+                __syncthreads();
+            }
+        } else {
+        GRL_LOAD_IDX(mbeg, _a)
+        GRL_LOAD_TILE(_a)
+        GRL_LOAD_IDX(mbeg + BK, _a)
         for (int mt = mbeg; mt < mend; mt += BK) {
-            GRL_STORE_TILE()
+            GRL_STORE_TILE(_a)
             __syncthreads();
-            GRL_LOAD_TILE()
-            GRL_LOAD_IDX(mt + 2 * BK)
-            {
-                if constexpr (F32) {
-                    mfma_f32_step<TM, TN>(reinterpret_cast<const float *>(&As[0][0]), reinterpret_cast<const float *>(&Bs[0][0]),
-                                          wm * WM + l16, wn * WN + l16, kg, acc);
-                } else if constexpr (TM < TN) {
-                    f16x8 af[TM][2];
-#pragma unroll
-                    for (int a = 0; a < TM; ++a)
-#pragma unroll
-                        for (int p = 0; p < 2; ++p) af[a][p] = *reinterpret_cast<const f16x8 *>(&As[p][aro + a * 16 * LDH]);
-#pragma unroll
-                    for (int b = 0; b < TN; ++b) {
-                        f16x8 bf[2];
-#pragma unroll
-                        for (int p = 0; p < 2; ++p) bf[p] = *reinterpret_cast<const f16x8 *>(&Bs[p][bro + b * 16 * LDH]);
-#pragma unroll
-                        for (int a = 0; a < TM; ++a) mfma_x3(acc[a][b], acl[a][b], af[a], bf);
-                    }
-                } else {
-                    f16x8 bf[TN][2];
-#pragma unroll
-                    for (int b = 0; b < TN; ++b)
-#pragma unroll
-                        for (int p = 0; p < 2; ++p) bf[b][p] = *reinterpret_cast<const f16x8 *>(&Bs[p][bro + b * 16 * LDH]);
-#pragma unroll
-                    for (int a = 0; a < TM; ++a) {
-                        f16x8 af[2];
-#pragma unroll
-                        for (int p = 0; p < 2; ++p) af[p] = *reinterpret_cast<const f16x8 *>(&As[p][aro + a * 16 * LDH]);
-#pragma unroll
-                        for (int b = 0; b < TN; ++b) mfma_x3(acc[a][b], acl[a][b], af, bf[b]);
-                    }
-                }
-            }
+            GRL_LOAD_TILE(_a)
+            GRL_LOAD_IDX(mt + 2 * BK, _a)
+            GRL_TN_MFMA()
             __syncthreads();
         }
-    }
+        }
+    }
+#undef GRL_TN_MFMA
     if constexpr (!F32) {
 #pragma unroll
         for (int a = 0; a < TM; ++a)
diff --git a/golds-rl-gym_amd/csrc/net_patch.inc b/golds-rl-gym_amd/csrc/net_patch.inc
--- a/golds-rl-gym_amd/csrc/net_patch.inc
+++ b/golds-rl-gym_amd/csrc/net_patch.inc
@@ -579,9 +579,9 @@
         net->prof_tag_cur = PT_SLOT_FWD;
         GemmTimer t(net, 2.0 * live_pairs * 64 * 64);
         if (net->slots_xcd)
-            launch_rowk<128, 64, 4, 1, SlotsToPatch, EpiPatchExpand, 2, true, 1, true>(net, dim3(1, tiles + 8), st, g, PT + ConvOffsets::c3w, 576, 64, e);
+            launch_rowk<128, 64, 4, 1, SlotsToPatch, EpiPatchExpand, 2, true, 1, true, PF_SLOTS_TO_PATCH>(net, dim3(1, tiles + 8), st, g, PT + ConvOffsets::c3w, 576, 64, e);
         else
-            launch_rowk<128, 64, 4, 1, SlotsToPatch, EpiPatchExpand, 1, true, 1, true>(net, dim3(1, tiles), st, g, PT + ConvOffsets::c3w, 576, 64, e);
+            launch_rowk<128, 64, 4, 1, SlotsToPatch, EpiPatchExpand, 1, true, 1, true, PF_SLOTS_TO_PATCH>(net, dim3(1, tiles), st, g, PT + ConvOffsets::c3w, 576, 64, e);
     } else {
     {
         SlotRowsP g{net->d2s, net->sperm, n * 9, 64, 64, net->sbase + n, net->patch_skip ? net->stmask : nullptr};
@@ -602,7 +602,7 @@
         EpiBiasAct e{net->ysh, 512, net->tubias, ACT_NONE};
         net->prof_tag_cur = PT_ENV_FWD;
         GemmTimer t(net, 2.0 * nenv * 64.0 * trunk_union_pixels(net) * 512);
-        launch_rowk<128, 64, 4, 1, DenseRowsKU, EpiBiasAct, true, true, 2>(net, dim3(512 / 64, (nenv + 127) / 128), st, g, PT + ConvOffsets::d1w, 3136, 512, e);
+        launch_rowk<128, 64, 4, 1, DenseRowsKU, EpiBiasAct, true, true, 2, false, PF_DENSE_KU>(net, dim3(512 / 64, (nenv + 127) / 128), st, g, PT + ConvOffsets::d1w, 3136, 512, e);
     } else {
         DenseRows g{net->a3sh, nenv, 3136, 3136};
         EpiBiasAct e{net->ysh, 512, P + ConvOffsets::d1b, ACT_NONE};
diff --git a/golds-rl-gym_amd/csrc/net_shared.inc b/golds-rl-gym_amd/csrc/net_shared.inc
--- a/golds-rl-gym_amd/csrc/net_shared.inc
+++ b/golds-rl-gym_amd/csrc/net_shared.inc
@@ -1062,7 +1062,7 @@
         net->prof_tag_cur = PT_ENV_FWD;
         {
             GemmTimer t(net, 2.0 * trunk_live(net, 0, (double)nenv * 81) * 512 * 64);
-            launch_rowk<128, 64, 4, 1, GatherConv2ReluRows, EpiBiasDualRows>(net, dim3(1, (nenv * 81 + 127) / 128), st, gr,
+            launch_rowk<128, 64, 4, 1, GatherConv2ReluRows, EpiBiasDualRows, 1, true, 1, false, PF_CONV2_ROWS>(net, dim3(1, (nenv * 81 + 127) / 128), st, gr,
                                                                                       PT + ConvOffsets::c2w, 512, 64, e);
         }
         hipLaunchKernelGGL(trunk_fill_kernel, dim3((nenv * 81 * 16 + 255) / 256), dim3(256), 0, st, (const unsigned *)net->tamask, 3, 81,
@@ -1121,7 +1121,7 @@
         EpiConv2Corr e{net->d2s, net->m2s, net->cperm, net->cslot, net->expand3_gather && net->chunk <= (1u << 17) ? net->a2 : nullptr};
         net->prof_tag_cur = PT_CLASS_CORR;
         GemmTimer t(net, 2.0 * n * 128 * 576 * (6.25 / 9.0));
-        launch_rowk<128, 64, 4, 1, CorrRows, EpiConv2Corr, true, true, 1, true>(net, dim3(576 / 64, net->ctiles * 2), st, g, net->w2corr, 128, 576, e);
+        launch_rowk<128, 64, 4, 1, CorrRows, EpiConv2Corr, true, true, 1, true, PF_CORR_ROWS>(net, dim3(576 / 64, net->ctiles * 2), st, g, net->w2corr, 128, 576, e);
     } else {
         hipLaunchKernelGGL(expand_conv2_kernel, dim3(nenv < 256 ? nenv : 256), dim3(1024), EXP2_LDS_BYTES, st, net->sraw, net->z2sh, pos,
                            P + ConvOffsets::c1w, P + ConvOffsets::c2w, nenv, net->a2sh, net->d2s, net->m2s, net->ulist, net->sbase);
diff --git a/golds-rl-gym_amd/csrc/net_train.inc b/golds-rl-gym_amd/csrc/net_train.inc
--- a/golds-rl-gym_amd/csrc/net_train.inc
+++ b/golds-rl-gym_amd/csrc/net_train.inc
@@ -705,9 +705,9 @@
         GemmTimer t(net, 2.0 * flop_rows * (double)I * J * net->sfrac);
         if (net->swgrad_pair) {
             SlotGatherT3PPair gp{ag};
-            launch_tn<128, BN, 2, 2, SlotGatherT3PPair>(net, dim3(5, J / BN, chunks), st, gp, net->d2s, J, mc, slab);
+            launch_tn<128, BN, 2, 2, SlotGatherT3PPair, 1, PF_TN_SLOT_T3P_PAIR>(net, dim3(5, J / BN, chunks), st, gp, net->d2s, J, mc, slab);
         } else
-            launch_tn<BM, BN, 2, 2, SlotGatherT3P>(net, dim3(I / BM, J / BN, chunks), st, ag, net->d2s, J, mc, slab);
+            launch_tn<BM, BN, 2, 2, SlotGatherT3P, 1, PF_TN_SLOT_T3P>(net, dim3(I / BM, J / BN, chunks), st, ag, net->d2s, J, mc, slab);
     }
     RJob j{};
     j.kind = RJ_TAPS_C3; j.blocks = I * J / 32; j.i0 = chunks; j.p0 = slab; j.p1 = skip ? net->szmask : nullptr; j.d0 = gw3;
@@ -739,10 +739,10 @@
     rq_push(net, rd, j);
 }
 
-template <int BM, int BN, int WGM, int WGN, bool FENCE = true, int NBUF = 1, bool ACC1 = false, class AG, class Epi>
+template <int BM, int BN, int WGM, int WGN, bool FENCE = true, int NBUF = 1, bool ACC1 = false, int PFI = PF_NONE, class AG, class Epi>
 static void rowk_launch(grl_net *net, AG ag, const float *W, int ldb, int N, Epi epi, double flops) {
     GemmTimer t(net, flops);
-    launch_rowk<BM, BN, WGM, WGN, AG, Epi, true, FENCE, NBUF, ACC1>(net, dim3(N / BN, (ag.rows + BM - 1) / BM), net->h->stream, ag, W, ldb, N, epi);
+    launch_rowk<BM, BN, WGM, WGN, AG, Epi, true, FENCE, NBUF, ACC1, PFI>(net, dim3(N / BN, (ag.rows + BM - 1) / BM), net->h->stream, ag, W, ldb, N, epi);
 }
 
 static int resident_grid(const void *kernel, int cap) {
@@ -878,7 +878,7 @@
         if (trunk3) {
             float *cs4 = slabb_take(net, ((size_t)nenv * 81 / 128 + 2) * 4 * 64);
             if (!cs4) return nfail(net, GRL_E_INVALID, "backward_chunk: column-sum buffer too small");
-            rowk_launch<128, 64, 4, 1, false, 1, true>(net, GatherT3Rows{net->dz3sh, net->trowlist, net->trows_n, nenv * 81}, net->w3t, 576, 64,
+            rowk_launch<128, 64, 4, 1, false, 1, true, PF_T3_ROWS>(net, GatherT3Rows{net->dz3sh, net->trowlist, net->trows_n, nenv * 81}, net->w3t, 576, 64,
                                        EpiGradRowsSum{net->dz2, 64, net->a2sh, cs4, net->trowlist, net->trows_n},
                                        2.0 * trunk_live(net, 0, (double)nenv * 81) * 576 * 64);
             hipLaunchKernelGGL(colsum_live_kernel, dim3(kLiveParts), dim3(256), 0, st, (const float *)cs4, (const int *)net->trows_n, 128, 4, 64,
@@ -895,7 +895,7 @@
         {
             SlotGatherT3P g3{net->dz3p, net->rowdesc, n * 9, net->sbase + n, net->sperm, net->patch_skip ? net->stmask : nullptr, nullptr};
             GemmTimer t(net, 2.0 * slot_rows_for_flops(net, n) * 576 * 64 * net->sfrac);
-            launch_rowk<128, 64, 4, 1, SlotGatherT3P, EpiPermStore, true, true, 1, true>(net, dim3(1, (n * 9 + 127) / 128), st, g3, net->w3t, 576, 64,
+            launch_rowk<128, 64, 4, 1, SlotGatherT3P, EpiPermStore, true, true, 1, true, PF_SLOT_T3P>(net, dim3(1, (n * 9 + 127) / 128), st, g3, net->w3t, 576, 64,
                                                                                          EpiPermStore{net->gsl, net->sperm, 64});
         }
         static const int hg2 = resident_grid((const void *)agent_dz2_kernel, 2048);
@@ -963,7 +963,7 @@
             if (!slab) return nfail(net, GRL_E_INVALID, "dense1 per-env weight gradient: slab too small");
             {
                 GemmTimer t(net, 2.0 * nenv * 64.0 * trunk_union_pixels(net) * J);
-                launch_tn<64, 128, 2, 2, DenseRowsIU>(net, dim3(I / 64, J / 128, chunks), st, DenseRowsIU{{net->a3sh, nenv, 3136, 3136}, net->tumask},
+                launch_tn<64, 128, 2, 2, DenseRowsIU, 1, PF_TN_DENSE_IU>(net, dim3(I / 64, J / 128, chunks), st, DenseRowsIU{{net->a3sh, nenv, 3136, 3136}, net->tumask},
                                                       net->gd1sh, J, mc, slab);
             }
             RJob j{};
@@ -1012,7 +1012,7 @@
             GatherConv3Rows ag{net->a2sh, net->tc3list, net->trows_n + 2, net->tbgimg3, nenv * 49, chunks};
             {
                 GemmTimer t(net, 2.0 * trunk_live(net, 2, (double)nenv * 49) * I * J);
-                launch_tn<64, 64, 2, 2, GatherConv3Rows>(net, dim3(I / 64, J / 64, chunks), st, ag, net->dz3sh, J, 0, slab);
+                launch_tn<64, 64, 2, 2, GatherConv3Rows, 1, PF_TN_CONV3_ROWS>(net, dim3(I / 64, J / 64, chunks), st, ag, net->dz3sh, J, 0, slab);
             }
             RJob j{};
             j.kind = RJ_SLAB; j.blocks = (I * J + 255) / 256; j.i0 = chunks; j.i1 = 1; j.n = (long)I * J; j.p0 = slab; j.d0 = Gr + ConvOffsets::c3w;
@@ -1034,7 +1034,7 @@
             GatherConv2ReluRows ag{net->sraw, net->trowlist, net->trows_n, net->tbgimg, nenv * 81, chunks};
             {
                 GemmTimer t(net, 2.0 * trunk_live(net, 0, (double)nenv * 81) * I * J);
-                launch_tn<128, 64, 2, 2, GatherConv2ReluRows>(net, dim3(I / 128, J / 64, chunks), st, ag, net->dz2, J, 0, slab);
+                launch_tn<128, 64, 2, 2, GatherConv2ReluRows, 1, PF_TN_CONV2_ROWS>(net, dim3(I / 128, J / 64, chunks), st, ag, net->dz2, J, 0, slab);
             }
             RJob j{};
             j.kind = RJ_SLAB; j.blocks = (I * J + 255) / 256; j.i0 = chunks; j.i1 = 1; j.n = (long)I * J; j.p0 = slab; j.d0 = Gr + ConvOffsets::c2w;
@@ -1069,13 +1069,13 @@
             T2SlotGather g{net->dza, net->t2desc, 4 * npad, npad, n, 32, cpc};
             {
                 GemmTimer t(net, 4 * 2.0 * n * 256 * 32);
-                launch_rowk<128, 32, 4, 1, T2SlotGather, EpiStore>(net, dim3(1, 4 * npad / 128), st, g, net->w2t, 256, 32, EpiStore{net->tt2, 32});
+                launch_rowk<128, 32, 4, 1, T2SlotGather, EpiStore, 1, true, 1, false, PF_T2_SLOT>(net, dim3(1, 4 * npad / 128), st, g, net->w2t, 256, 32, EpiStore{net->tt2, 32});
             }
             float *cslab = slab_take(net, (size_t)4 * cpc * 8192);
             if (!cslab) return nfail(net, GRL_E_INVALID, "class corrections: slab too small");
             {
                 GemmTimer t(net, 4 * 2.0 * n * 256 * 32);
-                launch_tn<64, 32, 4, 1, T2SlotGather>(net, dim3(256 / 64, 1, 4 * cpc), st, g, net->dl2, 32, mc, cslab);
+                launch_tn<64, 32, 4, 1, T2SlotGather, 1, PF_TN_T2_SLOT>(net, dim3(256 / 64, 1, 4 * cpc), st, g, net->dl2, 32, mc, cslab);
             }
             RJob j{};
             j.kind = RJ_GROUPS_C2; j.blocks = 4 * 8192 / 256; j.i0 = cpc; j.p0 = cslab; j.d0 = Gr + ConvOffsets::c2w;
```

Measured after the change: 2.305 million env-steps/s (median of 5 runs). 1.8% higher.
